# santiagolmedo/gnn_qot_estimation

Hardware: AMD Instinct MI355X
Metric: graphs/sec (train step) on 100-node/400-edge synthetic topologies, batch=1024 (higher is better)
Workload: dtype f32; 1 GPU; configs[1]: 2-layer TopologicalGNN (TransformerConv+NNConv) hidden=64, 100-node/400-directed-edge topologies, batch=1024 graphs per GPU, dropout 0.5, SGD momentum 0.9, SmoothL1; CSR build included in every step; graphs_per_gpu=1024, global_batch=1024, distinct_graphs_per_gpu=1024, launch=hip-graph replay, 4 whole steps (fwd+bwd+optimizer each) per graph, steps_per_graph=4, collective_in_graph=False, parallelism=dp1, prime_steps=45, collective_world_size=1, all_reduce_floats=68715

## Files before the change

### gnn_qot_estimation_amd/_lib.py

```python
from __future__ import annotations

import ctypes as C
import os
import subprocess

import torch

_HERE = os.path.dirname(os.path.abspath(__file__))
LIB_PATH = os.environ.get("QOT_LIB_PATH") or os.path.join(_HERE, "libqot_gnn.so")
CSRC_DIR = os.path.join(_HERE, "csrc")

_p = C.c_void_p
_i64 = C.c_int64
_int = C.c_int
_f = C.c_float
_u64 = C.c_uint64
_sz = C.c_size_t

ABI_VERSION = 13

_INFER_COMMON = ([_p] * 5 + [_i64] * 3 + [_int, _int, _p, _int, _p, _int, _p, _int] + [_p] * 9
                 + [_f, _f, _p, _int, _int, _int, _p])
_LP_COMMON = ([_p] * 6 + [_i64] * 4 + [_p] * 4 + [_f] + [_p] * 4 + [_f] + [_p] * 4 + [_f, _p, _p] + [_int] * 5 + [_p])

SIGNATURES = {
    "qot_abi_version": (_int, []),
    "qot_error_string": (C.c_char_p, [_int]),
    "qot_csr_workspace_bytes": (_sz, [_i64, _i64, _int]),
    "qot_csr_build": (_int, [_p, _i64, _i64, _int, _p, _p, _p, _p, _p, _p, _p, _p, _p, _p, _sz, _p]),
    "qot_csr_gat_by_graph_supported": (_int, [_i64, _i64]),
    "qot_csr_build_gat_by_graph": (_int, [_p, _i64, _i64, _p, _p, _i64, _i64, _i64, _p, _p, _p, _p, _p, _p, _p, _p, _p, _p, _p,
                                          _p]),
    "qot_csr_build_by_graph": (_int, [_p, _i64, _i64, _p, _p, _i64, _i64, _i64, _p, _p, _p, _p, _p, _p, _p, _p, _p,
                                      _p, _p, _p, _p, _p, _p, _p]),
    "qot_i32_gather": (_int, [_p, _p, _p, _i64, _p]),
    "qot_i64_to_i32": (_int, [_p, _p, _i64, _p]),
    "qot_batch_ptr": (_int, [_p, _i64, _i64, _p, _p]),
    "qot_embed_fwd": (_int, [_p, _p, _p, _i64, _int, _int, _p]),
    "qot_embed_bwd": (_int, [_p, _p, _p, _i64, _int, _int, _p]),
    "qot_tconv_fwd_scores": (_int, [_p, _p, _p, _int, _p, _int, _p, _p, _p, _p, _p, _p, _p, _p, _i64, _int, _int,
                                    _int, _f, _f, _u64, _p, _p]),
    "qot_tconv_rows_supported": (_int, [_int, _int, _int]),
    "qot_tconv_rows_npad": (_int, [_int]),
    "qot_tconv_rows_ld": (_int, [_int, _int, _int]),
    "qot_tconv_bwd_dst_rows": (_int, [_p, _p, _p, _int, _p, _p, _p, _p, _p, _p, _p, _int, _p, _p, _p, _p, _f, _f, _u64, _p,
                                      _int, _i64, _int, _p, _p, _int, _int, _p]),
    "qot_tconv_fwd_rows": (_int, [_p, _p, _p, _int, _p, _int, _p, _p, _p, _p, _p, _p, _p, _int, _i64, _int, _int, _int,
                                  _int, _f, _f, _u64, _p, _p]),
    "qot_tconv_bwd_src_rows": (_int, [_p, _p, _p, _p, _p, _int, _i64, _int, _p, _int, _p]),
    "qot_tconv_fwd": (_int, [_p, _p, _p, _p, _int, _p, _p, _p, _p, _p, _p, _p, _p, _i64, _int, _int,
                             _int, _f, _f, _u64, _p, _p]),
    "qot_tconv_fwd_tile": (_int, [_p, _p, _p, _p, _int, _p, _p, _p, _p, _p, _p, _p, _p, _i64, _int, _int, _int, _i64,
                                  _int, _f, _f, _u64, _p, _p]),
    "qot_tconv_bwd_dst_workspace_floats": (_sz, [_i64, _int, _int]),
    "qot_tconv_rows_per_block": (_int, [_int]),
    "qot_tconv_bwd_dst_blocks": (_i64, [_i64, _int, _int, _i64]),
    "qot_tconv_bwd_dst": (_int, [_p, _p, _p, _p, _int, _p, _p, _p, _p, _p, _p, _p, _p, _p, _int, _p, _p, _p, _p,
                                 _p, _f, _f, _u64, _p, _p, _p, _int, _i64, _p, _i64, _int, _int, _p]),
    "qot_tconv_bwd_src": (_int, [_p, _int, _p, _int, _p, _p, _p, _p, _p, _p, _p, _p, _int, _int, _i64, _p, _i64, _int,
                                 _p]),
    "qot_tconv_graph_supported": (_int, [_int, _int, _int, _int]),
    "qot_tconv_graph_ldm": (_int, [_int]),
    "qot_tconv_graph_row_floats": (_sz, [_int, _int, _int]),
    "qot_tconv_bwd_graph_blocks": (_int, [_i64]),
    "qot_table_scores": (_int, [_p, _p, _p, _p, _p, _p, _p, _p, _int, _int, _int, _p]),
    "qot_tconv_fwd_graph": (_int, [_p, _int, _p, _p, _p, _p, _p, _p, _p, _p, _p, _p, _p, _p, _int, _i64, _int, _int, _int,
                                   _int, _f, _f, _u64, _p, _p]),
    "qot_tconv_bwd_graph": (_int, [_p, _p, _f, _f, _u64, _p, _p, _int, _p, _p, _p, _p, _p, _p, _p, _p, _p, _p, _p, _int,
                                   _i64, _int, _int, _int, _p]),
    "qot_table_project_bwd_scores": (_int, [_p, _p, _p, _p, _p, _p, _p, _p, _p, _p, _p, _p, _int, _int, _int, _int, _p]),
    "qot_nnconv_agg": (_int, [_p, _int, _p, _p, _p, _p, _p, _p, _p, _p, _int, _p, _i64, _int, _int, _p]),
    "qot_nnconv_fused": (_int, [_p, _int, _p, _p, _p, _p, _p, _p, _p, _int, _p, _p, _p, _i64, _int, _int,
                                _int, _f, _f, _u64, _p, _p]),
    "qot_nnconv_fused_split": (_int, [_p, _int, _p, _p, _p, _p, _p, _p, _p, _p, _i64, _p, _p, _i64, _int, _int,
                                      _int, _f, _f, _u64, _p, _p]),
    "qot_nnconv_gradh_split": (_int, [_p, _int, _p, _int, _p, _p, _p, _p, _p, _p, _p, _p, _i64, _p, _p, _p, _i64, _int,
                                      _int, _p]),
    "qot_nnconv_bwd_finalize": (_int, [_p, _p, _p, _p, _p, _i64, _int, _int, _p]),
    "qot_nnconv_dw_workspace_floats": (_sz, [_i64, _int, _int]),
    "qot_nnconv_dw": (_int, [_p, _int, _p, _int, _p, _p, _p, _p, _p, _p, _p, _p, _p, _i64, _int, _int, _p]),
    "qot_gemm_tn_workspace_floats": (_sz, [_int]),
    "qot_gemm_tn": (_int, [_p, _int, _p, _int, _i64, _int, _p, _p, _p]),
    "qot_nnconv_adjoint_dw_workspace_floats": (_sz, [_int]),
    "qot_nnconv_adjoint_dw": (_int, [_p, _int, _p, _int, _p, _p, _p, _p, _p, _p, _p, _p, _p, _p, _int, _p, _i64,
                                     _int, _int, _p]),
    "qot_nnconv_gradh_workspace_floats": (_sz, [_int]),
    "qot_nnconv_gradh_fused": (_int, [_p, _int, _p, _int, _p, _p, _p, _p, _p, _p, _p, _p, _p, _p, _p, _i64, _int,
                                      _int, _p]),
    "qot_nnconv_bwd_edge": (_int, [_p, _int, _p, _int, _p, _p, _p, _p, _p, _p, _p, _p, _p, _i64, _int,
                                   _int, _p]),
    "qot_tconv_edge_attr_grad": (_int, [_p, _p, _f, _f, _u64, _p, _p, _int, _p, _p, _p, _p, _p, _p, _p, _i64, _int, _int,
                                        _p]),
    "qot_nnconv_edge_attr_grad": (_int, [_p, _int, _p, _int, _p, _p, _p, _p, _p, _p, _p, _p, _i64, _int, _int, _p]),
    "qot_tconv_attention": (_int, [_p, _int, _p, _p, _p, _p, _p, _p, _p, _i64, _int, _int, _p]),
    "qot_gat_attention": (_int, [_p, _p, _p, _p, _p, _p, _i64, _p, _i64, _int, _f, _p]),
    "qot_act_fwd": (_int, [_p, _p, _i64, _f, _f, _u64, _p, _p]),
    "qot_act_bwd": (_int, [_p, _p, _p, _i64, _f, _f, _u64, _p, _p]),
    "qot_pool_fwd": (_int, [_p, _p, _p, _i64, _int, _p]),
    "qot_pool_bwd": (_int, [_p, _p, _p, _p, _i64, _i64, _int, _p]),
    "qot_gat_blocks": (_int, [_i64, _int, _int]),
    "qot_gat_bn_partials_floats": (_sz, [_i64, _int, _int]),
    "qot_gat_logits": (_int, [_p, _p, _p, _p, _p, _i64, _int, _int, _p]),
    "qot_gat_fwd": (_int, [_p, _p, _p, _p, _p, _p, _p, _p, _i64, _int, _int, _f, _p, _p]),
    "qot_gat_att_grad": (_int, [_p, _p, _p, _p, _p, _p, _i64, _int, _int, _p]),
    "qot_gat_chunk_rows": (_i64, [_i64, _int, _int]),
    "qot_bn_stats_from_partials": (_int, [_p, _p, _int, _i64, _i64, _int, _f, _f, _p, _p, _p, _p, _p]),
    "qot_gat_thin_supported": (_int, [_int, _int, _int]),
    "qot_gat_fwd_thin": (_int, [_p, _int, _p, _p, _p, _p, _p, _p, _p, _p, _i64, _int, _int, _f, _p, _p]),
    "qot_gat_bwd_dst_thin": (_int, [_p, _p, _int, _p, _p, _p, _p, _p, _p, _p, _p, _p, _i64, _int, _int, _f, _p, _p, _p]),
    "qot_gat_bwd_dst": (_int, [_p, _p, _p, _p, _p, _p, _p, _p, _p, _p, _i64, _int, _int, _f, _p, _p, _p]),
    "qot_gat_bwd_src": (_int, [_p, _p, _p, _p, _p, _p, _p, _p, _p, _p, _i64, _int, _int, _f, _p, _p, _p, _p]),
    "qot_bn_partials_floats": (_sz, [_i64, _int]),
    "qot_bn_stats": (_int, [_p, _i64, _int, _f, _f, _p, _p, _p, _p, _p, _p]),
    "qot_bn_apply": (_int, [_p, _p, _p, _p, _p, _p, _i64, _int, _int, _p]),
    "qot_bn_bwd_reduce": (_int, [_p, _p, _p, _p, _p, _p, _p, _i64, _int, _int, _p, _p, _p, _p]),
    "qot_bn_bwd_apply": (_int, [_p, _p, _p, _p, _p, _p, _p, _p, _p, _i64, _int, _int, _int, _p, _p]),
    "qot_bn_apply_rows": (_int, [_p, _p, _i64, _p, _p, _p, _p, _p, _int, _int, _p]),
    "qot_bn_bwd_reduce_rows": (_int, [_p, _p, _i64, _p, _p, _p, _p, _p, _int, _int, _p, _p, _p, _p]),
    "qot_bn_bwd_apply_rows": (_int, [_p, _p, _i64, _p, _p, _p, _p, _p, _p, _p, _i64, _int, _int, _p, _p]),
    "qot_sgd_momentum": (_int, [_p, _p, _p, _i64, _f, _f, _int, _p]),
    "qot_sgd_momentum_multi": (_int, [_p, _p, _p, _int, _p, _p, _i64, _f, _p, _f, _int, _p]),
    "qot_sgd_momentum_dev": (_int, [_p, _p, _p, _i64, _p, _f, _int, _p]),
    "qot_small_gemm": (_int, [_p, _i64, _i64, _p, _i64, _i64, _p, _p, _int, _int, _int, _int, _int, _p]),
    "qot_colsum_workspace_floats": (_sz, [_int]),
    "qot_colsum": (_int, [_p, _int, _i64, _int, _p, _p, _p]),
    "qot_rowsum_wide_workspace_floats": (_sz, [_i64]),
    "qot_rowsum_wide": (_int, [_p, _i64, _i64, _p, _p, _p]),
    "qot_head_fwd": (_int, [_p, _p, _p, _p, _p, _p, _p, _p, _p, _i64, _int, _int, _f, _f, _u64, _p, _p]),
    "qot_head_fwd_loss": (_int, [_p, _p, _p, _p, _p, _p, _p, _p, _p, _i64, _int, _int, _f, _f, _u64, _p, _p, _f, _p, _p, _p]),
    "qot_head_train": (_int, [_p, _p, _p, _p, _p, _p, _p, _f, _p, _p, _p, _p, _p, _i64, _int, _int, _f, _f, _u64, _p, _int,
                              _f, _f, _u64, _p, _p]),
    "qot_head_train_blocks": (_int, [_i64, _int]),
    "qot_head_bwd_workspace_floats": (_sz, [_int, _int]),
    "qot_head_bwd_blocks": (_int, [_i64]),
    "qot_head_bwd": (_int, [_p, _p, _p, _p, _p, _p, _p, _p, _p, _i64, _int, _int, _f, _f, _u64, _p,
                            _p, _f, _f, _u64, _p, _p]),
    "qot_act_bwd_colsum": (_int, [_p, _p, _p, _i64, _int, _f, _f, _u64, _p, _p, _p, _p]),
    "qot_smooth_l1_workspace_floats": (_sz, []),
    "qot_smooth_l1": (_int, [_p, _p, _i64, _f, _p, _p, _p, _p]),
    "qot_table_project_fwd": (_int, [_p, _p, _p, _p, _p, _p, _p, _p, _p, _p, _int, _int, _p, _p, _p]),
    "qot_table_project_bwd": (_int, [_p, _p, _p, _p, _p, _p, _p, _p, _p, _int, _int, _p]),
    "qot_table_maps": (_int, [_p, _p, _p, _p, _p, _p, _i64, _i64, _p]),
    "qot_step_advance": (_int, [_p, _p, _p]),
    "qot_shard_stage": (_int, [_p, _i64, _p, _p, _p, _p, _i64, _i64, _i64, _p, _p, _int, _p, _p, _int, _p, _int, _i64, _i64,
                               _i64, _i64, _i64, _i64, _p, _p, _p, _p, _p, _p, _p, _p, _p]),
    "qot_shard_stage_padded": (_int, [_p, _i64, _p, _p, _p, _p, _i64, _i64, _i64, _p, _p, _int, _p, _p, _int, _p, _int, _i64,
                                      _i64, _i64, _i64, _i64, _i64, _p, _p, _p, _p, _p, _p, _p, _p, _p]),
    "qot_shard_stage_gather": (_int, [_p, _i64, _p, _p, _p, _p, _i64, _i64, _i64, _p, _p, _int, _p, _p, _int, _p, _int, _i64,
                                      _i64, _i64, _i64, _i64, _i64, _p, _p, _p, _p, _p, _p, _p, _p, _p]),
    "qot_gather3": (_int, [_p, _i64, _p, _i64, _p, _p, _p, _i64, _p]),
    "qot_gemm_nt": (_int, [_p, _i64, _p, _i64, _p, _i64, _i64, _int, _int, _p, _p, _p, _p]),
    "qot_gemm_nt_planes": (_int, [_p, _i64, _p, _i64, _p, _i64, _int, _int, _int, _p]),
    "qot_gemm_tn_splits": (_int, [_int, _int, _i64]),
    "qot_gemm256_takes": (_int, [_i64, _int]),
    "qot_gemm_tn_planes": (_int, [_p, _i64, _p, _i64, _p, _int, _int, _i64, _int, _p, _p, _p]),
    "qot_skinny_linear_fwd": (_int, [_p, _p, _p, _i64, _int, _int, _p]),
    "qot_skinny_linear_fwd_logits": (_int, [_p, _p, _p, _i64, _int, _int, _p, _p, _p, _p, _p]),
    "qot_gemm_nt_logits": (_int, [_p, _i64, _p, _i64, _p, _i64, _i64, _int, _int, _p, _p, _p, _p, _p, _p, _p, _p]),
    "qot_skinny_linear_dw_blocks": (_int, [_i64]),
    "qot_skinny_linear_dw": (_int, [_p, _p, _p, _i64, _int, _int, _p]),
    "qot_run_roles": (_int, [_p, _int, _p]),
    "qot_nnconv_gradh_host_roles": (_int, [_p, _int]),
    "qot_rows_gather": (_int, [_p, _p, _p, _i64, _int, _p]),
    "qot_rows_scatter": (_int, [_p, _p, _p, _i64, _int, _p]),
    **{f"qot_topological_infer{k}_supported": (_int, [_int] * 5) for k in ("", "_mc", "_grad", "_whatif")},
    **{f"qot_topological_infer{k}_max_edges": (_int, [_int] * 3) for k in ("", "_mc", "_grad", "_whatif")},
    "qot_topological_infer": (_int, _INFER_COMMON + [_p]),
    "qot_topological_infer_mc": (_int, _INFER_COMMON + [_int, _i64, _u64, _f, _f, _int, _p]),
    "qot_topological_infer_grad": (_int, _INFER_COMMON + [_p, _int, _p, _p, _p]),
    "qot_topological_infer_whatif": (_int, _INFER_COMMON + [_p, _p, _p, _i64, _p, _p, _i64, _p, _i64, _int, _p]),
    "qot_topological_infer_status": (_int, _INFER_COMMON + [_p, _p, _p, _i64, _int, _i64, _i64, _int, _int, _int, _p, _int,
                                                            _p]),
    "qot_topological_infer_place": (_int, _INFER_COMMON + [_p, _p, _p, _i64, _int, _i64, _i64, _int, _int, _int, _p, _int,
                                                           _p, _p, _p, _i64, _p]),
    "qot_lightpath_infer": (_int, _LP_COMMON + [_p]),
    "qot_lightpath_infer_grad": (_int, _LP_COMMON + [_p, _int, _p, _p, _p, _p, _p]),
    "qot_lightpath_infer_whatif": (_int, _LP_COMMON + [_p, _p, _p, _i64, _p, _p, _i64, _i64, _p]),
    "qot_lightpath_infer_status": (_int, _LP_COMMON + [_p, _p, _p, _i64, _int, _i64, _i64, _int, _int, _int, _int, _p, _int,
                                                       C.c_double, _p]),
    "qot_lightpath_infer_place": (_int, _LP_COMMON + [_p, _p, _p, _i64, _int, _i64, _i64, _int, _int, _int, _int, _p, _int,
                                                      C.c_double, _p, _p, _p, _i64, _p]),
    "qot_topological_infer_place_release": (_int, _INFER_COMMON + [_p, _p, _p, _i64, _int, _i64, _i64, _int, _int, _int, _p,
                                                                   _int, _p, _p, _p, _i64, _p, _p, _i64, _p]),
    "qot_lightpath_infer_place_release": (_int, _LP_COMMON + [_p, _p, _p, _i64, _int, _i64, _i64, _int, _int, _int, _int, _p,
                                                              _int, C.c_double, _p, _p, _p, _i64, _p, _p, _i64, _p]),
    "qot_lightpath_infer_place_impact": (_int, _LP_COMMON + [_p, _p, _p, _i64, _int, _i64, _i64, _int, _int, _int, _int, _p,
                                                             _int, C.c_double, _p, _p, _p, _i64, _p, _p, _p, _p, _int, _p]),
    "qot_status_graph_scratch_bytes": (_sz, [_i64, _i64, _i64, _int]),
    "qot_status_graph_count": (_int, [_p, _p, _p, _i64, _i64, _int, _i64, _i64, _int, _int, _int, C.c_double, _int, _p, _sz, _p,
                                      _p]),
    "qot_status_graph_fill": (_int, [_p, _p, _p, _i64, _i64, _int, _i64, _i64, _int, _int, _int, _int, _p, _int, _p, _int, _p,
                                     _p, _p, _p, _i64, _i64, _p, _p, _p, _p, _p]),
}

MAX_ROLES = 12
(ROLE_CSR_BY_GRAPH, ROLE_TABLE_PROJECT_FWD, ROLE_GATHER3, ROLE_SUM_ROWS, ROLE_NNCONV_FINALIZE64, ROLE_TABLE_PROJECT_BWD,
 ROLE_TABLE_SCORES, ROLE_TABLE_PROJECT_BWD_SCORES, ROLE_NNCONV_SLAB_SUM64, ROLE_NNCONV_GRADH_SUM64) = range(1, 11)
HOSTABLE_ROLES = (ROLE_SUM_ROWS, ROLE_NNCONV_SLAB_SUM64)


class Role(C.Structure):
    _fields_ = [("kind", C.c_int32), ("reserved", C.c_int32), ("p", C.c_void_p * 18), ("i", C.c_int64 * 8)]


def make_role(kind: int, ptrs, ints) -> Role:
    r = Role()
    r.kind = kind
    for k, t in enumerate(ptrs):
        r.p[k] = None if t is None else (t.data_ptr() if isinstance(t, torch.Tensor) else int(t))
    for k, v in enumerate(ints):
        r.i[k] = int(v)
    return r


def run_roles(roles, stream_handle=None):
    if not roles:
        return
    if len(roles) > MAX_ROLES:
        for k in range(0, len(roles), MAX_ROLES):
            run_roles(roles[k:k + MAX_ROLES], stream_handle)
        return
    arr = (Role * len(roles))(*roles)
    code = (_lib or load()).qot_run_roles(C.addressof(arr), len(roles), stream() if stream_handle is None else stream_handle)
    if code != 0:
        check(code, "qot_run_roles")


def host_roles(roles):
    arr = (Role * max(len(roles), 1))(*roles)
    code = (_lib or load()).qot_nnconv_gradh_host_roles(C.addressof(arr), len(roles))
    if code != 0:
        check(code, "qot_nnconv_gradh_host_roles")


_lib = None


class QotError(RuntimeError):
    """A libqot_gnn entry point returned a non-zero status."""


def build_library(verbose: bool = False) -> str:
    cmd = ["make", "-C", CSRC_DIR, "-j", str(min(8, os.cpu_count() or 1))]
    res = subprocess.run(cmd, capture_output=True, text=True)
    if res.returncode != 0:
        raise RuntimeError("building libqot_gnn.so failed:\n" + res.stdout[-4000:] + res.stderr[-8000:])
    if verbose:
        print(res.stdout[-2000:])
    return LIB_PATH


def load():
    global _lib
    if _lib is not None:
        return _lib
    if not os.path.exists(LIB_PATH):
        raise QotError(
            f"{LIB_PATH} not found: build it with `python -c 'import __graft_entry__ as g; g.build()'` "
            "or `make -C gnn_qot_estimation_amd/csrc` -- there is no CPU fallback for the HIP path"
        )
    lib = C.CDLL(LIB_PATH)
    for name, (res, args) in SIGNATURES.items():
        fn = getattr(lib, name)
        fn.restype = res
        fn.argtypes = args
    if lib.qot_abi_version() != ABI_VERSION:
        raise QotError(f"libqot_gnn ABI version {lib.qot_abi_version()} != {ABI_VERSION} expected by this package: "
                       "rebuild with `make -C gnn_qot_estimation_amd/csrc`")
    _lib = lib
    return lib


def ptr(t):
    return None if t is None else t.data_ptr()


_raw_stream = getattr(torch._C, "_cuda_getCurrentRawStream", None)
_raw_device = getattr(torch._C, "_cuda_getDevice", None)


def stream():
    if _pinned_stream is not None:
        return _pinned_stream
    if _raw_stream is not None and _raw_device is not None:
# ... 36 lines not shown
```

### gnn_qot_estimation_amd/csrc/head.hip

```cpp
#include "common.hpp"

namespace qot {

constexpr int kHeadBwdBlocks = 512;

template <int H>
__global__ __launch_bounds__(256) void head_fwd_kernel(
    const float* __restrict__ x, const int32_t* __restrict__ ptr, const float* __restrict__ w0,
    const float* __restrict__ b0, const float* __restrict__ w3, const float* __restrict__ b3,
    float* __restrict__ pooled, float* __restrict__ hidden, float* __restrict__ out, int O, ActParams act,
    const float* __restrict__ target, float beta, float inv_n, float* __restrict__ grad_out, float* __restrict__ loss_rows) {
    __shared__ float4 red[256];
    __shared__ float lrow[8];
    __shared__ float p[H];
    __shared__ float h[H];
    constexpr int TPR = H / 4, RPB = 256 / TPR;
    const int sub = threadIdx.x % TPR, slot = threadIdx.x / TPR;
    const int64_t b = blockIdx.x;
    const int beg = ptr[b], end = ptr[b + 1];
    float4 acc = f4zero();
    if (slot < RPB)
        for (int64_t r = beg + slot; r < end; r += RPB) acc = add4(acc, ld4(x + r * H + 4 * sub));
    red[threadIdx.x] = acc;
    __syncthreads();
    if (threadIdx.x < TPR) {
        float4 s = red[threadIdx.x];
        for (int k = 1; k < RPB; ++k) s = add4(s, red[k * TPR + threadIdx.x]);
        const int cnt = end - beg;
        s = scale4(1.0f / (float)(cnt > 1 ? cnt : 1), s);
        p[4 * threadIdx.x] = s.x; p[4 * threadIdx.x + 1] = s.y; p[4 * threadIdx.x + 2] = s.z; p[4 * threadIdx.x + 3] = s.w;
        st4(pooled + b * H + 4 * threadIdx.x, s);
    }
    __syncthreads();
    if (threadIdx.x < H) {
        const int o = threadIdx.x;
        float v = b0[o];
#pragma unroll 8
        for (int a = 0; a < H; ++a) v = fmaf(w0[o * H + a], p[a], v);
        v = act_apply1(v, act, (uint64_t)(b * H + o));
        h[o] = v;
        hidden[b * H + o] = v;
    }
    __syncthreads();
    if (threadIdx.x < O) {
        const int o = threadIdx.x;
        float v = b3[o];
        for (int a = 0; a < H; ++a) v = fmaf(w3[o * H + a], h[a], v);
        out[b * O + o] = v;
        if (target) {
            const float d = v - target[b * O + o];
            const float ad = fabsf(d);
            float l, g;
            if (ad < beta) { l = 0.5f * d * d / beta; g = d / beta; }
            else           { l = ad - 0.5f * beta;    g = d > 0.f ? 1.f : -1.f; }
            grad_out[b * O + o] = g * inv_n;
            lrow[o] = l * inv_n;
        }
    }
    if (target) {
        __syncthreads();
        if (threadIdx.x == 0) {
            float s = lrow[0];
            for (int o = 1; o < O; ++o) s += lrow[o];
            loss_rows[b] = s;
        }
    }
}

template <int H>
__global__ __launch_bounds__(256) void head_bwd_kernel(
    const float* __restrict__ gout, const float* __restrict__ pooled, const float* __restrict__ hidden,
    const int32_t* __restrict__ ptr, const float* __restrict__ w0, const float* __restrict__ w3,
    float* __restrict__ gx, float* __restrict__ partials, int64_t B, int O, ActParams act,
    const float* __restrict__ x_in, ActParams in_act) {
    constexpr int PER = H * H / 256;
    __shared__ float4 cred[256];
    float4 acs = f4zero();
    __shared__ float gh[H];
    __shared__ float gp[H];
    __shared__ float pp[H];
    __shared__ float go[8];
    float aw0[PER];
#pragma unroll
    for (int e = 0; e < PER; ++e) aw0[e] = 0.f;
    float ab0 = 0.f, aw3[8], ab3 = 0.f;
#pragma unroll
    for (int e = 0; e < 8; ++e) aw3[e] = 0.f;
    const int t = threadIdx.x;
    __shared__ float w0s[H * H];
    __shared__ float w3s[8 * H];
    {
        float wv[PER];
#pragma unroll
        for (int e = 0; e < PER; ++e) wv[e] = w0[t + 256 * e];
#pragma unroll
        for (int e = 0; e < PER; ++e) w0s[t + 256 * e] = wv[e];
    }
    for (int e = t; e < O * H; e += 256) w3s[e] = w3[e];
    for (int64_t b = blockIdx.x; b < B; b += gridDim.x) {
        if (t < O) go[t] = gout[b * O + t];
        if (t < H) pp[t] = pooled[b * H + t];
        const int beg = ptr[b], end = ptr[b + 1];
        const float hv_pre = (t < H) ? hidden[b * H + t] : 0.f;
        __syncthreads();
        if (t < H) {
            float v = 0.f;
            for (int o = 0; o < O; ++o) v = fmaf(w3s[o * H + t], go[o], v);
            const float hv = hv_pre;
            float d = 0.f;
            if (act.thr16) {
                const uint64_t z = act_hash64(act.seed, (uint64_t)act.step[0], (uint64_t)(b * H + t) >> 2);
                const bool keep = ((uint32_t)(z >> (16 * ((b * H + t) & 3))) & 0xFFFFu) >= act.thr16;
                d = keep ? act.keep_scale : 0.f;
            } else {
                d = 1.0f;
            }
            d *= (hv > 0.f) ? 1.0f : act.slope;
            gh[t] = v * d;
            ab0 += v * d;
#pragma unroll
            for (int o = 0; o < 8; ++o) if (o < O) aw3[o] = fmaf(go[o], hv, aw3[o]);
        }
        if (t < O) ab3 += go[t];
        __syncthreads();
        if (t < H) {
            float v = 0.f;
#pragma unroll 8
            for (int o = 0; o < H; ++o) v = fmaf(w0s[o * H + t], gh[o], v);
            gp[t] = v;
        }
#pragma unroll
        for (int e = 0; e < PER; ++e) {
            const int idx = t * PER + e;
            aw0[e] = fmaf(gh[idx / H], pp[idx % H], aw0[e]);
        }
        __syncthreads();
        const float inv = 1.0f / (float)((end - beg) > 1 ? (end - beg) : 1);
        constexpr int TPR = H / 4, RPB = 256 / TPR;
        const int sub = t % TPR, slot = t / TPR;
        float4 cs = f4zero();
        if (slot < RPB) {
            const float4 v = make_float4(gp[4 * sub] * inv, gp[4 * sub + 1] * inv, gp[4 * sub + 2] * inv, gp[4 * sub + 3] * inv);
            if (!x_in) {
                for (int64_t r = beg + slot; r < end; r += RPB) st4(gx + r * H + 4 * sub, v);
            } else {
                constexpr int UR = 4;
                for (int64_t r0 = beg + slot; r0 < end; r0 += (int64_t)UR * RPB) {
                    float4 yy[UR];
#pragma unroll
                    for (int u = 0; u < UR; ++u) {
                        const int64_t r = r0 + (int64_t)u * RPB;
                        yy[u] = ld4(x_in + (r < end ? r : r0) * H + 4 * sub);
                    }
// ... 126 lines not shown
                }
                if (t < O) ptgt = target[bn * O + t];
            }
        }
        float4 acc = f4zero();
        if (slot < RPB) {
#pragma unroll
            for (int u = 0; u < 8; ++u) {
                const int r = slot + u * RPB;
                if (r < cnt) {
                    if (in_lds) *reinterpret_cast<float4*>(&xs[r * H + 4 * sub]) = v0[u];
                    acc = add4(acc, v0[u]);
                }
            }
            for (int r0 = slot + 8 * RPB; r0 < cnt; r0 += 8 * RPB) {
                float4 v[8];
#pragma unroll
                for (int u = 0; u < 8; ++u) {
                    const int r = r0 + u * RPB;
                    v[u] = ld4(x + (int64_t)(beg + (r < cnt ? r : r0)) * H + 4 * sub);
                }
#pragma unroll
                for (int u = 0; u < 8; ++u) {
                    const int r = r0 + u * RPB;
                    if (r < cnt) {
                        if (in_lds) *reinterpret_cast<float4*>(&xs[r * H + 4 * sub]) = v[u];
                        acc = add4(acc, v[u]);
                    }
                }
            }
        }
        cred[t] = acc;
        __syncthreads();
        if (t < TPR) {
            float4 s4 = cred[t];
            for (int k2 = 1; k2 < RPB; ++k2) s4 = add4(s4, cred[k2 * TPR + t]);
            s4 = scale4(1.0f / (float)(cnt > 1 ? cnt : 1), s4);
            pp[4 * t] = s4.x; pp[4 * t + 1] = s4.y; pp[4 * t + 2] = s4.z; pp[4 * t + 3] = s4.w;
        }
        __syncthreads();
        float hv = 0.f, dact = 0.f;
        if (t < H) {
            float v = b0t;
#pragma unroll 8
            for (int a = 0; a < H; ++a) v = fmaf(w0s[t * HP + a], pp[a], v);
            float d = 1.0f;
            if (act.thr16) {
                const uint64_t flat = (uint64_t)(b * H + t);
                const uint64_t z = act_hash64(act.seed, stepv, flat >> 2);
                const bool keep = ((uint32_t)(z >> (16 * (flat & 3))) & 0xFFFFu) >= act.thr16;
                d = keep ? act.keep_scale : 0.f;
            }
            d *= (v > 0.f) ? 1.0f : act.slope;
            hv = v * d;
            dact = d;
            hh[t] = hv;
        }
        __syncthreads();
        if (t < O) {
            float v = b3t;
            for (int a = 0; a < H; ++a) v = fmaf(w3s[t * H + a], hh[a], v);
            out[b * O + t] = v;
            const float df = v - tgt;
            const float ad = fabsf(df);
            float l, g;
            if (ad < beta) { l = 0.5f * df * df / beta; g = df / beta; }
            else           { l = ad - 0.5f * beta;      g = df > 0.f ? 1.f : -1.f; }
            g *= inv_n;
            grad_out[b * O + t] = g;
            go[t] = g;
            lrow[t] = l * inv_n;
            ab3 += g;
        }
        __syncthreads();
        if (t == 0) {
            float sl = lrow[0];
            for (int o = 1; o < O; ++o) sl += lrow[o];
            loss_rows[b] = sl;
        }
        if (t < H) {
            float v = 0.f;
            for (int o = 0; o < O; ++o) v = fmaf(w3s[o * H + t], go[o], v);
            const float g1 = v * dact;
            gh[t] = g1;
            ab0 += g1;
#pragma unroll
            for (int o = 0; o < 8; ++o) if (o < O) aw3[o] = fmaf(go[o], hv, aw3[o]);
        }
        __syncthreads();
        if (t < H) {
            float v = 0.f;
#pragma unroll 8
            for (int o = 0; o < H; ++o) v = fmaf(w0s[o * HP + t], gh[o], v);
            gp[t] = v;
        }
#pragma unroll
        for (int e = 0; e < PER; ++e) {
            const int idx = t * PER + e;
            aw0[e] = fmaf(gh[idx / H], pp[idx % H], aw0[e]);
        }
        __syncthreads();
        const float inv = 1.0f / (float)(cnt > 1 ? cnt : 1);
        float4 cs = f4zero();
        if (slot < RPB) {
            const float4 v = make_float4(gp[4 * sub] * inv, gp[4 * sub + 1] * inv, gp[4 * sub + 2] * inv, gp[4 * sub + 3] * inv);
            if (!fold) {
                for (int r = slot; r < cnt; r += RPB) st4(gx + (int64_t)(beg + r) * H + 4 * sub, v);
            } else {
                for (int r = slot; r < cnt; r += RPB) {
                    const int64_t flat = (int64_t)(beg + r) * H + 4 * sub;
                    const float4 yy = in_lds ? *reinterpret_cast<const float4*>(&xs[r * H + 4 * sub]) : ld4(x + flat);
                    uint64_t z = 0;
                    if (in_act.thr16) z = act_hash64(in_act.seed, in_stepv, (uint64_t)flat >> 2);
                    float vi[4] = {v.x, v.y, v.z, v.w};
                    const float vr[4] = {yy.x, yy.y, yy.z, yy.w};
#pragma unroll
                    for (int c = 0; c < 4; ++c) {
                        const bool keep = in_act.thr16 ? (((uint32_t)(z >> (16 * c)) & 0xFFFFu) >= in_act.thr16) : true;
                        vi[c] = vi[c] * (keep ? in_act.keep_scale : 0.f) * (vr[c] > 0.f ? 1.0f : in_act.slope);
                    }
                    const float4 o4 = make_float4(vi[0], vi[1], vi[2], vi[3]);
                    st4(gx + flat, o4);
                    cs = add4(cs, o4);
                }
            }
        }
        if (fold) {
            cred[t] = cs;
            __syncthreads();
            if (t < TPR) {
                float4 s4 = cred[t];
                for (int k2 = 1; k2 < RPB; ++k2) s4 = add4(s4, cred[k2 * TPR + t]);
                acs = add4(acs, s4);
            }
        }
        __syncthreads();
    }
    float* part = partials + (int64_t)blockIdx.x * (H * H + H + O * H + O + (fold ? H : 0));
    if (fold && t < H / 4) st4(part + H * H + H + O * H + O + 4 * t, acs);
#pragma unroll
    for (int e = 0; e < PER; ++e) part[t * PER + e] = aw0[e];
    if (t < H) {
        part[H * H + t] = ab0;
        for (int o = 0; o < O; ++o) part[H * H + H + o * H + t] = aw3[o];
    }
    if (t < O) part[H * H + H + O * H + t] = ab3;
}

constexpr int kHeadKeep = 32;
#ifndef QOT_HEAD_THREADS
#define QOT_HEAD_THREADS 512
#endif
constexpr int kHeadThreads = QOT_HEAD_THREADS;

template <int H, int NT>
__global__ __launch_bounds__(NT) void head_train_batched_kernel(
    const float* __restrict__ x, const int32_t* __restrict__ ptr, const float* __restrict__ w0,
    const float* __restrict__ b0, const float* __restrict__ w3, const float* __restrict__ b3,
    const float* __restrict__ target, float beta, float inv_n, float* __restrict__ out, float* __restrict__ grad_out,
    float* __restrict__ loss_rows, float* __restrict__ gx, float* __restrict__ partials, int64_t B, int O, ActParams act,
    int fold, ActParams in_act) {
    constexpr int TPR = H / 4, RPB = NT / TPR;
    constexpr int GB = 256 / H;
    constexpr int SPG = RPB / GB;
    constexpr int KS = NT / 256;
    constexpr int KR = kHeadKeep * 4 / SPG;
    constexpr int PER = H * H / NT;
    constexpr int HP = H + 1;
    static_assert(KS == 1 || KS == 2 || KS == 4, "dense outputs are summed inside a quad");
    static_assert(H % (4 * KS) == 0 && PER >= 1, "width");
    extern __shared__ __attribute__((aligned(16))) float dyn[];
    float* w0s = dyn;
    float* w3s = w0s + H * HP;
    __shared__ float4 cred[NT > 640 ? NT : 640];
    __shared__ __attribute__((aligned(16))) float pp[GB][H];
    __shared__ __attribute__((aligned(16))) float hh[GB][H];
    __shared__ __attribute__((aligned(16))) float gh[GB][H];
    __shared__ __attribute__((aligned(16))) float gp[GB][H];
    __shared__ float go[GB][8];
    __shared__ float lrow[GB][8];
    __shared__ int pb[GB + 1];
    const int t = threadIdx.x;
    const int sub = t % TPR, slot = t / TPR;
    const int gs = slot / SPG, sr = slot % SPG;
    const int part = t % KS, od = t / KS;
    const int g = od / H, o = od % H;
    const int64_t npass = (B + GB - 1) / GB;
    int pb_first = 0;
    if (t <= GB && (int64_t)blockIdx.x < npass) {
        const int64_t bb = (int64_t)blockIdx.x * GB + t;
        pb_first = ptr[bb < B ? bb : B];
    }
    for (int e = t; e < H * H; e += NT) w0s[(e / H) * HP + e % H] = w0[e];
    for (int e = t; e < O * H; e += NT) w3s[e] = w3[e];
    const uint64_t stepv = act.thr16 ? (uint64_t)act.step[0] : 0;
    const uint64_t in_stepv = (fold && in_act.thr16) ? (uint64_t)in_act.step[0] : 0;
    const float b0o = b0[o];
    float aw0[PER];
#pragma unroll
    for (int e = 0; e < PER; ++e) aw0[e] = 0.f;
    float ab0p = 0.f, aw3p[8], ab3p = 0.f;
#pragma unroll
    for (int e = 0; e < 8; ++e) aw3p[e] = 0.f;
    float4 acs = f4zero();
    for (int64_t ps = blockIdx.x; ps < npass; ps += gridDim.x) {
        const int64_t b0g = ps * GB;
        __syncthreads();
        if (t <= GB) {
            const int64_t bb = b0g + t;
            pb[t] = ps == (int64_t)blockIdx.x ? pb_first : ptr[bb < B ? bb : B];
        }
        __syncthreads();
        const bool live = b0g + gs < B;
        const int beg = pb[gs], cnt = live ? pb[gs + 1] - beg : 0;
        float4 v[KR];
        float4 acc = f4zero();
#pragma unroll
        for (int k = 0; k < KR; ++k) {
            const int r = sr + SPG * k;
            v[k] = (r < cnt) ? ld4(x + (int64_t)(beg + r) * H + 4 * sub) : f4zero();
        }
#pragma unroll
        for (int k = 0; k < KR; ++k) acc = add4(acc, v[k]);
        for (int r = sr + SPG * KR; r < cnt; r += SPG) acc = add4(acc, ld4(x + (int64_t)(beg + r) * H + 4 * sub));
        cred[t] = acc;
        __syncthreads();
        if (t < GB * TPR) {
            const int gg = t / TPR, sb = t % TPR;
            float4 s4 = cred[(gg * SPG) * TPR + sb];
            for (int q = 1; q < SPG; ++q) s4 = add4(s4, cred[(gg * SPG + q) * TPR + sb]);
            const int c2 = pb[gg + 1] - pb[gg];
            s4 = scale4(1.0f / (float)(c2 > 1 ? c2 : 1), s4);
            pp[gg][4 * sb] = s4.x; pp[gg][4 * sb + 1] = s4.y; pp[gg][4 * sb + 2] = s4.z; pp[gg][4 * sb + 3] = s4.w;
        }
        __syncthreads();
        const int64_t bg = b0g + g;
        float hv = 0.f, dact = 0.f;
        {
            float a0 = 0.f;
#pragma unroll
            for (int a = part * (H / KS); a < (part + 1) * (H / KS); ++a) a0 = fmaf(w0s[o * HP + a], pp[g][a], a0);
            if (KS >= 2) a0 += dpp_move<0xB1>(a0);
            if (KS >= 4) a0 += dpp_move<0x4E>(a0);
            const float vv = a0 + b0o;
            float d = 1.0f;
            if (act.thr16) {
                const uint64_t flat = (uint64_t)(bg * H + o);
                const uint64_t z = act_hash64(act.seed, stepv, flat >> 2);
                const bool keep = ((uint32_t)(z >> (16 * (flat & 3))) & 0xFFFFu) >= act.thr16;
                d = keep ? act.keep_scale : 0.f;
            }
            d *= (vv > 0.f) ? 1.0f : act.slope;
            hv = vv * d;
            dact = d;
            if (part == 0) hh[g][o] = hv;
        }
        __syncthreads();
        for (int q = t / 16; q < GB * O; q += NT / 16) {
            const int gg = q / O, o3 = q % O, l16 = t % 16;
            const int64_t bb = b0g + gg;
            float pv = 0.f;
#pragma unroll
            for (int a = l16 * (H / 16); a < (l16 + 1) * (H / 16); ++a) pv = fmaf(w3s[o3 * H + a], hh[gg][a], pv);
            pv = group_sum<16>(pv);
            if (l16 == 0) {
                if (bb < B) {
                    const float vv = pv + b3[o3];
                    out[bb * O + o3] = vv;
                    const float df = vv - target[bb * O + o3];
                    const float ad = fabsf(df);
                    float l, gq;
                    if (ad < beta) { l = 0.5f * df * df / beta; gq = df / beta; }
                    else           { l = ad - 0.5f * beta;      gq = df > 0.f ? 1.f : -1.f; }
                    gq *= inv_n;
                    grad_out[bb * O + o3] = gq;
                    go[gg][o3] = gq;
                    lrow[gg][o3] = l * inv_n;
                } else {
                    go[gg][o3] = 0.f;
                    lrow[gg][o3] = 0.f;
                }
            }
        }
        __syncthreads();
        if (t < GB && b0g + t < B) {
            float sl = lrow[t][0];
            for (int o3 = 1; o3 < O; ++o3) sl += lrow[t][o3];
            loss_rows[b0g + t] = sl;
        }
        if (t < GB * O) ab3p += go[t / O][t % O];
        {
            float vv = 0.f;
            for (int o3 = 0; o3 < O; ++o3) vv = fmaf(w3s[o3 * H + o], go[g][o3], vv);
            const float g1 = bg < B ? vv * dact : 0.f;
            if (part == 0) {
                gh[g][o] = g1;
                ab0p += g1;
#pragma unroll
                for (int o3 = 0; o3 < 8; ++o3) if (o3 < O) aw3p[o3] = fmaf(go[g][o3], hv, aw3p[o3]);
            }
        }
        __syncthreads();
        {
            float a0 = 0.f;
#pragma unroll
            for (int oo = part * (H / KS); oo < (part + 1) * (H / KS); ++oo) a0 = fmaf(w0s[oo * HP + o], gh[g][oo], a0);
            if (KS >= 2) a0 += dpp_move<0xB1>(a0);
            if (KS >= 4) a0 += dpp_move<0x4E>(a0);
            if (part == 0) gp[g][o] = a0;
        }
#pragma unroll
        for (int gg = 0; gg < GB; ++gg)
#pragma unroll
            for (int e = 0; e < PER; ++e) {
                const int idx = t * PER + e;
                aw0[e] = fmaf(gh[gg][idx / H], pp[gg][idx % H], aw0[e]);
            }
        __syncthreads();
        if (cnt > 0) {
            const float inv = 1.0f / (float)(cnt > 1 ? cnt : 1);
            const float4 gv = make_float4(gp[gs][4 * sub] * inv, gp[gs][4 * sub + 1] * inv, gp[gs][4 * sub + 2] * inv,
                                          gp[gs][4 * sub + 3] * inv);
            auto back = [&](int r, float4 yy) {
                const int64_t flat = (int64_t)(beg + r) * H + 4 * sub;
                if (!fold) { st4(gx + flat, gv); return; }
                uint64_t z = 0;
                if (in_act.thr16) z = act_hash64(in_act.seed, in_stepv, (uint64_t)flat >> 2);
                float vi[4] = {gv.x, gv.y, gv.z, gv.w};
                const float vr[4] = {yy.x, yy.y, yy.z, yy.w};
#pragma unroll
                for (int c = 0; c < 4; ++c) {
                    const bool keep = in_act.thr16 ? (((uint32_t)(z >> (16 * c)) & 0xFFFFu) >= in_act.thr16) : true;
                    vi[c] = vi[c] * (keep ? in_act.keep_scale : 0.f) * (vr[c] > 0.f ? 1.0f : in_act.slope);
                }
                const float4 o4 = make_float4(vi[0], vi[1], vi[2], vi[3]);
                st4(gx + flat, o4);
                acs = add4(acs, o4);
            };
#pragma unroll
            for (int k = 0; k < KR; ++k) {
                const int r = sr + SPG * k;
                if (r < cnt) back(r, v[k]);
            }
            for (int r = sr + SPG * KR; r < cnt; r += SPG) back(r, fold ? ld4(x + (int64_t)(beg + r) * H + 4 * sub) : f4zero());
        }
    }
    float* part_row = partials + (int64_t)blockIdx.x * (H * H + H + O * H + O + (fold ? H : 0));
#pragma unroll
    for (int e = 0; e < PER; ++e) part_row[t * PER + e] = aw0[e];
    __syncthreads();
    float* red = reinterpret_cast<float*>(cred);
    if (part == 0) {
        red[od] = ab0p;
#pragma unroll
        for (int o3 = 0; o3 < 8; ++o3) if (o3 < O) red[(1 + o3) * 256 + od] = aw3p[o3];
    }
    if (t < GB * O) red[9 * 256 + t] = ab3p;
    __syncthreads();
    if (t < H) {
        float s2 = red[t];
#pragma unroll
        for (int gg = 1; gg < GB; ++gg) s2 += red[gg * H + t];
        part_row[H * H + t] = s2;
        for (int o3 = 0; o3 < O; ++o3) {
            float s3 = red[(1 + o3) * 256 + t];
#pragma unroll
            for (int gg = 1; gg < GB; ++gg) s3 += red[(1 + o3) * 256 + gg * H + t];
            part_row[H * H + H + o3 * H + t] = s3;
        }
    }
    if (t < O) {
        float s2 = red[9 * 256 + t];
        for (int gg = 1; gg < GB; ++gg) s2 += red[9 * 256 + gg * O + t];
        part_row[H * H + H + O * H + t] = s2;
    }
    if (fold) {
        __syncthreads();
        cred[t] = acs;
        __syncthreads();
        if (t < TPR) {
            float4 s4 = cred[t];
            for (int k2 = 1; k2 < RPB; ++k2) s4 = add4(s4, cred[k2 * TPR + t]);
            st4(part_row + H * H + H + O * H + O + 4 * t, s4);
        }
    }
}

__global__ __launch_bounds__(1024) void head_partial_sum_kernel(const float* __restrict__ partials, int nblk, int n,
                                                                float* __restrict__ out) {
    __shared__ float red[16][64];
    const int o = threadIdx.x & 63, sg = threadIdx.x >> 6;
    const int t = blockIdx.x * 64 + o;
    float acc = 0.f;
    if (t < n) {
        const int per = (nblk + 15) / 16;
        const int p0 = sg * per, p1 = (p0 + per < nblk) ? p0 + per : nblk;
        int p = p0;
        for (; p + 8 <= p1; p += 8) {
            float v[8];
#pragma unroll
            for (int u = 0; u < 8; ++u) v[u] = partials[(int64_t)(p + u) * n + t];
#pragma unroll
            for (int u = 0; u < 8; ++u) acc += v[u];
        }
        for (; p < p1; ++p) acc += partials[(int64_t)p * n + t];
    }
    red[sg][o] = acc;
    __syncthreads();
    if (sg == 0 && t < n) {
        float s = red[0][o];
#pragma unroll
        for (int q = 1; q < 16; ++q) s += red[q][o];
        out[t] = s;
    }
}

}

using namespace qot;

#define QOT_HEAD_H(H, ...)                                            \
    switch (H) {                                                      \
        case 16:  { constexpr int kH = 16;  __VA_ARGS__; } break;     \
        case 32:  { constexpr int kH = 32;  __VA_ARGS__; } break;     \
        case 64:  { constexpr int kH = 64;  __VA_ARGS__; } break;     \
        case 128: { constexpr int kH = 128; __VA_ARGS__; } break;     \
        default: return QOT_ERR_UNSUPPORTED;                          \
    }

extern "C" int qot_head_train(const float* x, const int32_t* ptr, const float* w0, const float* b0, const float* w3,
                              const float* b3, const float* target, float beta, float* out, float* grad_out,
                              float* loss_rows, float* grad_x, float* workspace, int64_t B, int H, int O, float slope,
                              float p, uint64_t seed, const int64_t* step_counter, int fold, float in_slope, float in_p,
                              uint64_t in_seed, const int64_t* in_step, qot_stream_t stream_) {
    hipStream_t stream = (hipStream_t)stream_;
    if (B <= 0 || O <= 0 || !(beta > 0.f)) return QOT_ERR_BADARG;
    if (O > 8) return QOT_ERR_UNSUPPORTED;
    if (!x || !ptr || !w0 || !b0 || !w3 || !b3 || !target || !out || !grad_out || !loss_rows || !grad_x || !workspace)
        return QOT_ERR_BADARG;
    const ActParams ap = make_act(1, slope, p, seed, step_counter);
    const ActParams in_ap = make_act(fold ? 1 : 0, in_slope, in_p, in_seed, in_step);
    int blocks = kHeadBwdBlocks;
    if (B < blocks) blocks = (int)B;
    const float inv_n = 1.0f / ((float)B * (float)O);
    if (H <= 64) {
        const int gbn = 256 / H;
        int64_t nb = (B + gbn - 1) / gbn;
        if (nb > kHeadBwdBlocks) nb = kHeadBwdBlocks;
        blocks = (int)nb;
        QOT_HEAD_H(H, {
            if constexpr (kH <= 64) {
                const size_t lds = (size_t)(kH * (kH + 1) + 8 * kH) * sizeof(float);
                constexpr int NT = kH * kH < kHeadThreads ? 256 : kHeadThreads;
                head_train_batched_kernel<kH, NT><<<blocks, NT, lds, stream>>>(
                    x, ptr, w0, b0, w3, b3, target, beta, inv_n, out, grad_out, loss_rows, grad_x, workspace, B, O, ap, fold,
                    in_ap);
            }
        });
        QOT_LAUNCH_CHECK();
        return QOT_OK;
    }
    QOT_HEAD_H(H, {
        const size_t lds = (size_t)(kHeadRowsCap * kH + kH * (kH + 1) + 8 * kH) * sizeof(float);
        static size_t allowed[kMaxDevices];
        const int lrc = ensure_dyn_lds(reinterpret_cast<const void*>(head_train_kernel<kH>), lds, allowed);
        if (lrc != QOT_OK) return lrc;
        head_train_kernel<kH><<<blocks, 256, lds, stream>>>(x, ptr, w0, b0, w3, b3, target, beta, inv_n, out, grad_out,
                                                            loss_rows, grad_x, workspace, B, O, ap, fold, in_ap);
    });
    QOT_LAUNCH_CHECK();
    return QOT_OK;
}

extern "C" int qot_head_train_blocks(int64_t B, int H) {
    if (B <= 0) return 0;
    if (H <= 64 && H >= 16) {
        const int gbn = 256 / H;
        const int64_t nb = (B + gbn - 1) / gbn;
        return nb > kHeadBwdBlocks ? kHeadBwdBlocks : (int)nb;
    }
    return B < kHeadBwdBlocks ? (int)B : kHeadBwdBlocks;
}


extern "C" int qot_head_fwd_loss(const float* x, const int32_t* ptr, const float* w0, const float* b0,
                                 const float* w3, const float* b3, float* pooled, float* hidden, float* out,
                                 int64_t B, int H, int O, float slope, float p, uint64_t seed,
                                 const int64_t* step_counter, const float* target, float beta, float* grad_out,
                                 float* loss_rows, qot_stream_t stream) {
    if (B < 0 || O <= 0 || O > 8) return (O > 8) ? QOT_ERR_UNSUPPORTED : QOT_ERR_BADARG;
    if (B == 0) return QOT_OK;
    if (!x || !ptr || !w0 || !b0 || !w3 || !b3 || !pooled || !hidden || !out) return QOT_ERR_BADARG;
    if (target && (!grad_out || !loss_rows || !(beta > 0.f))) return QOT_ERR_BADARG;
    const ActParams ap = make_act(1, slope, p, seed, step_counter);
    const float inv_n = 1.0f / ((float)B * (float)O);
    QOT_HEAD_H(H, head_fwd_kernel<kH><<<(int)B, 256, 0, (hipStream_t)stream>>>(x, ptr, w0, b0, w3, b3, pooled, hidden,
                                                                              out, O, ap, target, beta, inv_n, grad_out,
                                                                              loss_rows));
    QOT_LAUNCH_CHECK();
    return QOT_OK;
}

extern "C" int qot_head_fwd(const float* x, const int32_t* ptr, const float* w0, const float* b0,
                            const float* w3, const float* b3, float* pooled, float* hidden, float* out,
                            int64_t B, int H, int O, float slope, float p, uint64_t seed,
                            const int64_t* step_counter, qot_stream_t stream) {
    return qot_head_fwd_loss(x, ptr, w0, b0, w3, b3, pooled, hidden, out, B, H, O, slope, p, seed, step_counter, nullptr,
                             1.0f, nullptr, nullptr, stream);
}

extern "C" int qot_head_bwd_blocks(int64_t B) { return B < kHeadBwdBlocks ? (int)(B > 0 ? B : 0) : kHeadBwdBlocks; }

extern "C" size_t qot_head_bwd_workspace_floats(int H, int O) {
    return (size_t)kHeadBwdBlocks * (size_t)(H * H + 2 * H + O * H + O);
}

extern "C" int qot_head_bwd(const float* grad_out, const float* pooled, const float* hidden, const int32_t* ptr,
                            const float* w0, const float* w3, float* grad_x, float* grads, float* workspace,
                            int64_t B, int H, int O, float slope, float p, uint64_t seed,
                            const int64_t* step_counter, const float* x_in, float in_slope, float in_p,
                            uint64_t in_seed, const int64_t* in_step, qot_stream_t stream_) {
    hipStream_t stream = (hipStream_t)stream_;
    if (B <= 0 || O <= 0) return QOT_ERR_BADARG;
    if (O > 8) return QOT_ERR_UNSUPPORTED;
    if (!grad_out || !pooled || !hidden || !ptr || !w0 || !w3 || !grad_x || !workspace) return QOT_ERR_BADARG;
    const ActParams ap = make_act(1, slope, p, seed, step_counter);
    int blocks = kHeadBwdBlocks;
    if (B < blocks) blocks = (int)B;
    const ActParams in_ap = make_act(x_in ? 1 : 0, in_slope, in_p, in_seed, in_step);
    QOT_HEAD_H(H, head_bwd_kernel<kH><<<blocks, 256, 0, stream>>>(grad_out, pooled, hidden, ptr, w0, w3, grad_x,
                                                                  workspace, B, O, ap, x_in, in_ap));
    QOT_LAUNCH_CHECK();
    if (!grads) return QOT_OK;
    const int n = H * H + H + O * H + O + (x_in ? H : 0);
    head_partial_sum_kernel<<<grid_for(n, 64), 1024, 0, stream>>>(workspace, blocks, n, grads);
    QOT_LAUNCH_CHECK();
    return QOT_OK;
}
```

### gnn_qot_estimation_amd/csrc/mfma_tile.hpp

```cpp
#pragma once
#include "common.hpp"

namespace qot {

typedef float f32x16 __attribute__((ext_vector_type(16)));

__device__ __forceinline__ int at4_slot(int g, int hi, int i) { return (2 * g + hi) * 32 + (i ^ (g & 7)); }

__device__ __forceinline__ void store_fragment_grouped(float4* At4, int g, int i, float4 v0, float4 v1) {
    const float4 even = make_float4(v0.x, v0.z, v1.x, v1.z), odd = make_float4(v0.y, v0.w, v1.y, v1.w);
    At4[at4_slot(g, 0, i)] = even;
    At4[at4_slot(g, 1, i)] = odd;
}

__host__ __device__ constexpr int acc_row(int r, int hi) { return (r & 3) + 8 * (r >> 2) + 4 * hi; }

__device__ __forceinline__ f32x16 mfma4(float4 a, float4 b, f32x16 c) {
    c = __builtin_amdgcn_mfma_f32_32x32x2f32(a.x, b.x, c, 0, 0, 0);
    c = __builtin_amdgcn_mfma_f32_32x32x2f32(a.y, b.y, c, 0, 0, 0);
    c = __builtin_amdgcn_mfma_f32_32x32x2f32(a.z, b.z, c, 0, 0, 0);
    c = __builtin_amdgcn_mfma_f32_32x32x2f32(a.w, b.w, c, 0, 0, 0);
    return c;
}

__device__ __forceinline__ f32x16 mfma_group(const float4* __restrict__ At4, int g, int hi, int r31, float4 b,
                                             f32x16 c) {
    return mfma4(At4[at4_slot(g, hi, r31)], b, c);
}

template <int D>
__device__ __forceinline__ void edge_hidden(const float* __restrict__ w1, const float* __restrict__ b1,
                                            const float* __restrict__ ea, int64_t e, float scale, float* __restrict__ hid) {
    float ee[D];
#pragma unroll
    for (int d = 0; d < D; ++d) ee[d] = ea[e * D + d];
#pragma unroll
    for (int kk = 0; kk < 2 * D; ++kk) {
        float h = b1[kk];
#pragma unroll
        for (int d = 0; d < D; ++d) h = fmaf(w1[kk * D + d], ee[d], h);
        hid[kk] = fmaxf(h, 0.f) * scale;
    }
}

template <int S, int NH, int SS, int ST>
__device__ __forceinline__ void quad_share_from(const uint32_t (&mylo)[NH], const uint32_t (&myhi)[NH], uint32_t (&zlo)[4 * NH],
                                                uint32_t (&zhi)[4 * NH]) {
#pragma unroll
    for (int t = 0; t < NH; ++t) {
        zlo[S * SS + t * ST] = __builtin_amdgcn_update_dpp(0, mylo[t], S * 0x55, 0xF, 0xF, true);
        zhi[S * SS + t * ST] = __builtin_amdgcn_update_dpp(0, myhi[t], S * 0x55, 0xF, 0xF, true);
    }
}
template <int NH, int SS, int ST>
__device__ __forceinline__ void quad_share_draws(const uint32_t (&mylo)[NH], const uint32_t (&myhi)[NH], uint32_t (&zlo)[4 * NH],
                                                 uint32_t (&zhi)[4 * NH]) {
    quad_share_from<0, NH, SS, ST>(mylo, myhi, zlo, zhi);
    quad_share_from<1, NH, SS, ST>(mylo, myhi, zlo, zhi);
    quad_share_from<2, NH, SS, ST>(mylo, myhi, zlo, zhi);
    quad_share_from<3, NH, SS, ST>(mylo, myhi, zlo, zhi);
}

__device__ __forceinline__ void mfma_acc_in_agprs() {
#ifndef QOT_NO_AGPR_HINT
    float az = 0.f;
    asm volatile("; accumulators in AGPRs" : "+a"(az));
#endif
}

template <bool AFFINE>
__device__ __forceinline__ float4 affine_relu4(float4 v, float4 s, float4 t) {
    if (!AFFINE) return v;
    return make_float4(fmaxf(fmaf(v.x, s.x, t.x), 0.f), fmaxf(fmaf(v.y, s.y, t.y), 0.f),
                       fmaxf(fmaf(v.z, s.z, t.z), 0.f), fmaxf(fmaf(v.w, s.w, t.w), 0.f));
}

__device__ __forceinline__ void lds_barrier() {
    asm volatile("s_waitcnt lgkmcnt(0)" ::: "memory");
    __builtin_amdgcn_s_barrier();
    asm volatile("" ::: "memory");
}

__device__ __forceinline__ int64_t xcd_tile(int64_t it, int64_t ntiles, unsigned grid) {
    const int nx = 8;
    if ((int)grid % nx != 0) {
        const int64_t t = (int64_t)blockIdx.x + it * grid;
        return t < ntiles ? t : -1;
    }
    const int xcd = blockIdx.x % nx, slot = blockIdx.x / nx, per_x = grid / nx;
    const int64_t chunk = (ntiles + nx - 1) / nx;
    const int64_t local = slot + it * per_x;
    const int64_t t = xcd * chunk + local;
    return (local < chunk && t < ntiles) ? t : -1;
}
__device__ __forceinline__ int64_t xcd_tile(int64_t it, int64_t ntiles) {
    const int nx = 8;
    if ((int)gridDim.x % nx != 0) {
        const int64_t t = (int64_t)blockIdx.x + it * gridDim.x;
        return t < ntiles ? t : -1;
    }
    const int xcd = blockIdx.x % nx, slot = blockIdx.x / nx, per_x = gridDim.x / nx;
    const int64_t chunk = (ntiles + nx - 1) / nx;
    const int64_t local = slot + it * per_x;
    const int64_t t = xcd * chunk + local;
    return (local < chunk && t < ntiles) ? t : -1;
}

}

static inline int num_cus() {
    static int n = 0;
    if (!n) {
        int dev = 0;
        hipDeviceProp_t prop;
        if (hipGetDevice(&dev) == hipSuccess && hipGetDeviceProperties(&prop, dev) == hipSuccess) n = prop.multiProcessorCount;
        if (n <= 0) n = 256;
    }
    return n;
}
```

### gnn_qot_estimation_amd/csrc/nnconv_mfma.hip

```cpp
#include "common.hpp"
#include "mfma_tile.hpp"
#include "nnconv_finalize_dev.hpp"
#include "split_bf16.hpp"

namespace qot {

template <int D, bool TRANSPOSE, bool PRESPLIT = false>
__device__ __forceinline__ void nnconv_gather_tile(
    float* __restrict__ At, const float* __restrict__ x, int ldx, const float* __restrict__ ea,
    const float* __restrict__ w1, const float* __restrict__ b1, const int32_t* __restrict__ rowptr,
    const int32_t* __restrict__ col, const int32_t* __restrict__ eidx, const float* __restrict__ invdeg,
    int64_t tile0, int64_t N, float4& root0, float4& root1, float4* park0 = nullptr, float4* park1 = nullptr) {
    constexpr int K = 2 * D;
    const int sub = threadIdx.x & 7, il = threadIdx.x >> 3;
    const int c0 = 8 * sub;
    const int64_t i = tile0 + il;
    float4 acc0[K + 1], acc1[K + 1];
    root0 = f4zero(); root1 = f4zero();
    int beg = 0, end = 0;
    float srow = 0.f;
    if (i < N) {
        beg = rowptr[i]; end = rowptr[i + 1];
        if (!TRANSPOSE) srow = invdeg[i];
        root0 = ld4(x + i * ldx + c0);
        root1 = ld4(x + i * ldx + c0 + 4);
    }
    const int own = (i < N) ? (int)i : 0;
#define QOT_ACC(FIRSTSLOT, H, X, A) ((FIRSTSLOT) ? scale4((H), (X)) : fma4((H), (X), (A)))
#define QOT_EDGE4(U0, FIRST)                                                                            \
        {                                                                                               \
            float4 xa[4], xb[4];                                                                        \
            float sc[4];                                                                                \
            int jj[4];                                                                                  \
            jj[0] = group8_bcast<U0 + 0>(myj); jj[1] = group8_bcast<U0 + 1>(myj);                       \
            jj[2] = group8_bcast<U0 + 2>(myj); jj[3] = group8_bcast<U0 + 3>(myj);                       \
            sc[0] = group8_bcast<U0 + 0>(mysc); sc[1] = group8_bcast<U0 + 1>(mysc);                     \
            sc[2] = group8_bcast<U0 + 2>(mysc); sc[3] = group8_bcast<U0 + 3>(mysc);                     \
            _Pragma("unroll") for (int u = 0; u < 4; ++u) {                                             \
                const float* xr = x + (int64_t)jj[u] * ldx + c0;                                        \
                xa[u] = ld4(xr);                                                                        \
                xb[u] = ld4(xr + 4);                                                                    \
            }                                                                                           \
            _Pragma("unroll") for (int kk = 0; kk < K; ++kk) {                                          \
                const float h0 = group8_bcast<U0 + 0>(myh[kk]), h1 = group8_bcast<U0 + 1>(myh[kk]);     \
                acc0[kk] = QOT_ACC(FIRST, h0, xa[0], acc0[kk]); acc1[kk] = QOT_ACC(FIRST, h0, xb[0], acc1[kk]); \
                acc0[kk] = fma4(h1, xa[1], acc0[kk]); acc1[kk] = fma4(h1, xb[1], acc1[kk]);             \
            }                                                                                           \
            acc0[K] = QOT_ACC(FIRST, sc[0], xa[0], acc0[K]); acc1[K] = QOT_ACC(FIRST, sc[0], xb[0], acc1[K]); \
            acc0[K] = fma4(sc[1], xa[1], acc0[K]); acc1[K] = fma4(sc[1], xb[1], acc1[K]);               \
             \
             \
            if (cnt > U0 + 2) {                                                                         \
                _Pragma("unroll") for (int kk = 0; kk < K; ++kk) {                                      \
                    const float h2 = group8_bcast<U0 + 2>(myh[kk]), h3 = group8_bcast<U0 + 3>(myh[kk]); \
                    acc0[kk] = fma4(h2, xa[2], acc0[kk]); acc1[kk] = fma4(h2, xb[2], acc1[kk]);         \
                    acc0[kk] = fma4(h3, xa[3], acc0[kk]); acc1[kk] = fma4(h3, xb[3], acc1[kk]);         \
                }                                                                                       \
                _Pragma("unroll") for (int u = 2; u < 4; ++u) {                                         \
                    acc0[K] = fma4(sc[u], xa[u], acc0[K]);                                              \
                    acc1[K] = fma4(sc[u], xb[u], acc1[K]);                                              \
                }                                                                                       \
            }                                                                                           \
        }
#define QOT_FWD_BATCH(FIRST)                                                                            \
    {                                                                                                   \
        const int p = base + sub;                                                                       \
        int myj = own;                                                                                  \
        float myh[K], mysc = 0.f;                                                                       \
        _Pragma("unroll") for (int kk = 0; kk < K; ++kk) myh[kk] = 0.f;                                 \
        if (p < end) {                                                                                  \
            myj = col[p];                                                                               \
            mysc = TRANSPOSE ? invdeg[myj] : srow;                                                      \
            edge_hidden<D>(w1, b1, ea, (int64_t)eidx[p], mysc, myh);                                    \
        }                                                                                               \
        const int cnt = (end - base < 8) ? end - base : 8;                                              \
        QOT_EDGE4(0, FIRST)                                                                             \
        if (cnt > 4) QOT_EDGE4(4, false)                                                                \
    }
    int base = beg;
    QOT_FWD_BATCH(true)
    for (base = beg + 8; base < end; base += 8) QOT_FWD_BATCH(false)
#undef QOT_FWD_BATCH
#undef QOT_EDGE4
#undef QOT_ACC
    if constexpr (PRESPLIT) {
        constexpr int HB = (K + 2) / 2;
#pragma unroll
        for (int kk = 0; kk < HB; ++kk)
            store_split_planes(reinterpret_cast<u32x4*>(At) + kk * 3 * kGhPlLd, sub, il, acc0[kk], acc1[kk]);
#pragma unroll
        for (int kk = HB; kk <= K; ++kk) { park0[kk - HB] = acc0[kk]; park1[kk - HB] = acc1[kk]; }
    } else {
#pragma unroll
        for (int kk = 0; kk <= K; ++kk)
            store_fragment_grouped(reinterpret_cast<float4*>(At), kk * 8 + sub, il, acc0[kk], acc1[kk]);
    }
}

__device__ __forceinline__ void root_restage(float* At, float4 root0, float4 root1) {
    lds_barrier();
    store_fragment_grouped(reinterpret_cast<float4*>(At), threadIdx.x & 7, threadIdx.x >> 3, root0, root1);
    __syncthreads();
}

__host__ __device__ constexpr int fwd_plane_off(int p) { return (p / 4) * 3 * kGhPlLd + (p % 4) * kGhPlStep; }

template <int D, bool TRANSPOSE, bool SPLIT = false, bool PRESPLIT = false>
__global__ __launch_bounds__(256, 2) void nnconv_mfma64_kernel(
    const float* __restrict__ x, int ldx, const float* __restrict__ ea, const float* __restrict__ w1,
    const float* __restrict__ b1, const int32_t* __restrict__ rowptr, const int32_t* __restrict__ col,
    const int32_t* __restrict__ eidx, const float* __restrict__ invdeg, const float* __restrict__ Wp,
    const float* __restrict__ bias, float* __restrict__ out, int64_t N, ActParams act,
    const u32x4* __restrict__ Ws = nullptr, int64_t ws_planes = 0) {
    static_assert(!SPLIT || !TRANSPOSE, "split form: forward only");
    static_assert(!PRESPLIT || SPLIT, "the planes are the split form's");
    constexpr int K = 2 * D;
    constexpr int KM = (K + 1) * 64;
    constexpr int GM = KM / 16;
    constexpr int CH = 4;
    constexpr int HB = (K + 2) / 2;
    constexpr int PLF = HB * 3 * kGhPlLd * 4;
    __shared__ __attribute__((aligned(16))) float At[PRESPLIT ? PLF + 4 * 8 * 64 : KM * 32];
    const int64_t ntiles = (N + 31) / 32;
    const float bz = bias ? bias[((threadIdx.x >> 6) & 1) * 32 + (threadIdx.x & 31)] : 0.f;
    const uint64_t drop_step = (act.enabled && act.thr16) ? (uint64_t)act.step[0] : 0;
#pragma unroll 1
    for (int64_t it = 0;; ++it) {
    const int64_t tile = xcd_tile(it, ntiles);
    if (tile < 0) break;
    const int64_t tile0 = tile * 32;
    float4 root0, root1;
    float4 park0[PRESPLIT ? HB : 1], park1[PRESPLIT ? HB : 1];
    if constexpr (PRESPLIT) {
        nnconv_gather_tile<D, false, true>(At, x, ldx, ea, w1, b1, rowptr, col, eidx, invdeg, tile0, N, park0[HB - 1],
                                           park1[HB - 1], park0, park1);
    } else {
        nnconv_gather_tile<D, TRANSPOSE>(At, x, ldx, ea, w1, b1, rowptr, col, eidx, invdeg, tile0, N, root0, root1);
    }
    const float4* At4 = reinterpret_cast<const float4*>(At);
    const int lane = threadIdx.x & 63, wave = threadIdx.x >> 6;
    const int nh = wave & 1, kh = wave >> 1;
    const int r31 = lane & 31, hi = lane >> 5;
    f32x16 c;
#pragma unroll
    for (int r = 0; r < 16; ++r) c[r] = 0.f;
    if constexpr (PRESPLIT) {
        constexpr int SP = K + 2;
        constexpr int ST = 4 * SP;
        constexpr int SC = 2;
        constexpr int NCS = SP / SC;
        constexpr int NBS = 3;
        const int wv = __builtin_amdgcn_readfirstlane(wave);
        const u32x4* wsp = Ws + ((int64_t)(wv & 1) * ST + (wv >> 1) * SP) * 64;
        const unsigned lane_u = lane;
        const u32x4* plane = reinterpret_cast<const u32x4*>(At) + lane;
        const u32x4* pl_e = plane + kh * (fwd_plane_off(SP) - fwd_plane_off(0));
        const u32x4* pl_o = plane + kh * (fwd_plane_off(SP + 2) - fwd_plane_off(2));
        Bf3 sb[NBS][SC];
#define QOT_FWD_BLOAD(J)                                                                                \
        _Pragma("unroll") for (int u = 0; u < SC; ++u)                                                  \
            sb[(J) % NBS][u] = load_split_b(wsp + (((J) / NCS) * 2 * SP + ((J) % NCS) * SC + u) * 64, lane_u, ws_planes);
#define QOT_FWD_ALOAD(J)                                                                                \
        _Pragma("unroll") for (int u = 0; u < SC; ++u) {                                                \
            const int t = ((J) % NCS) * SC + u;                                                         \
            af[(J) & 1][u] = load_split_b(((t & 2) ? pl_o : pl_e) + fwd_plane_off(t), kGhPlLd);         \
        }
#define QOT_FWD_CHUNK(J)                                                                                \
        {                                                                                               \
            if ((J) + NBS - 1 < 2 * NCS) { QOT_FWD_BLOAD((J) + NBS - 1) }                               \
            if (((J) + 1) % NCS != 0) { QOT_FWD_ALOAD((J) + 1) }                                        \
            __builtin_amdgcn_sched_barrier(0);                                                          \
            _Pragma("unroll") for (int u = 0; u < SC; ++u) c = mfma_split6(af[(J) & 1][u], sb[(J) % NBS][u], c); \
            __builtin_amdgcn_sched_barrier(0);                                                          \
        }
        Bf3 af[2][SC];
#pragma unroll
        for (int j = 0; j < NBS - 1; ++j) QOT_FWD_BLOAD(j)
        lds_barrier();
        QOT_FWD_ALOAD(0)
#pragma unroll
        for (int j = 0; j < NCS; ++j) QOT_FWD_CHUNK(j)
        lds_barrier();
        {
            const int sub = threadIdx.x & 7, il = threadIdx.x >> 3;
#pragma unroll
            for (int kk = 0; kk < HB; ++kk)
                store_split_planes(reinterpret_cast<u32x4*>(At) + kk * 3 * kGhPlLd, sub, il, park0[kk], park1[kk]);
        }
        lds_barrier();
        QOT_FWD_ALOAD(NCS)
#pragma unroll
        for (int j = NCS; j < 2 * NCS; ++j) QOT_FWD_CHUNK(j)
#undef QOT_FWD_ALOAD
#undef QOT_FWD_CHUNK
#undef QOT_FWD_BLOAD
    } else if constexpr (SPLIT) {
        constexpr int ST = (K + 2) * 64 / 16;
        constexpr int SM = GM / 2;
        constexpr int SC = 2;
        constexpr int NCS = SM / SC;
        constexpr int NBS = 3;
        static_assert(GM % 4 == 0, "chunking");
        const u32x4* wsn = Ws + (int64_t)nh * ST * 64 + lane;
        const u32x4* wsp = wsn + (int64_t)kh * SM * 64;
        const u32x4* rsp = wsn + (int64_t)(2 * SM + 2 * kh) * 64;
        asm volatile("" : "+v"(rsp));
        Bf3 rbs[2];
#pragma unroll
        for (int u = 0; u < 2; ++u) rbs[u] = load_split_b(rsp + u * 64, ws_planes);
        Bf3 sb[NBS][SC];
#pragma unroll
        for (int q = 0; q < NBS - 1; ++q)
#pragma unroll
            for (int u = 0; u < SC; ++u) sb[q][u] = load_split_b(wsp + (q * SC + u) * 64, ws_planes);
        lds_barrier();
        int ch = 0;
#pragma unroll 1
        for (; ch + NBS <= NCS; ch += NBS) {
#pragma unroll
            for (int q = 0; q < NBS; ++q) {
                if (ch + q + NBS - 1 < NCS) {
#pragma unroll
                    for (int u = 0; u < SC; ++u)
                        sb[(q + NBS - 1) % NBS][u] = load_split_b(wsp + ((ch + q + NBS - 1) * SC + u) * 64, ws_planes);
                }
#pragma unroll
                for (int u = 0; u < SC; ++u) c = mfma_split_step(At4, kh * GM + 2 * ((ch + q) * SC + u), hi, r31, sb[q][u], c);
            }
        }
#pragma unroll
        for (int q = 0; q < NBS - 1; ++q) {
            if (ch + q < NCS) {
#pragma unroll
                for (int u = 0; u < SC; ++u) c = mfma_split_step(At4, kh * GM + 2 * ((ch + q) * SC + u), hi, r31, sb[q][u], c);
            }
        }
        root_restage(At, root0, root1);
#pragma unroll
        for (int u = 0; u < 2; ++u) c = mfma_split_step(At4, kh * 4 + 2 * u, hi, r31, rbs[u], c);
    } else {
    const float4* wpn = reinterpret_cast<const float4*>(Wp) + (int64_t)nh * (2 * GM + 8) * 64 + lane;
    const float4* wp = wpn + (int64_t)kh * GM * 64;
    const float4* rbp = wpn + (int64_t)(2 * GM + kh * 4) * 64;
    asm volatile("" : "+v"(rbp));
    float4 rb[4];
#pragma unroll
    for (int u = 0; u < 4; ++u) rb[u] = rbp[u * 64];
    constexpr int NCH = GM / CH;
    constexpr int NB = 4;
    float4 bb[NB][CH];
#pragma unroll
    for (int q = 0; q < NB - 1; ++q)
#pragma unroll
        for (int u = 0; u < CH; ++u) bb[q][u] = wp[(q * CH + u) * 64];
    lds_barrier();
    int ch = 0;
#pragma unroll 1
    for (; ch + NB <= NCH; ch += NB) {
#pragma unroll
        for (int q = 0; q < NB; ++q) {
            if (ch + q + NB - 1 < NCH) {
#pragma unroll
                for (int u = 0; u < CH; ++u) bb[(q + NB - 1) % NB][u] = wp[((ch + q + NB - 1) * CH + u) * 64];
            }
#pragma unroll
            for (int u = 0; u < CH; ++u) c = mfma_group(At4, kh * GM + (ch + q) * CH + u, hi, r31, bb[q][u], c);
        }
    }
#pragma unroll
    for (int q = 0; q < NB - 1; ++q) {
        if (ch + q < NCH) {
#pragma unroll
            for (int u = 0; u < CH; ++u) c = mfma_group(At4, kh * GM + (ch + q) * CH + u, hi, r31, bb[q][u], c);
        }
    }
    root_restage(At, root0, root1);
#pragma unroll
    for (int u = 0; u < 4; ++u) c = mfma_group(At4, kh * 4 + u, hi, r31, rb[u], c);
    }
    float* red = At + (PRESPLIT ? PLF : 64 * 32);
    if (kh) {
#pragma unroll
        for (int r = 0; r < 8; ++r) red[((2 + nh) * 8 + r) * 64 + lane] = c[r];
    } else {
#pragma unroll
        for (int r = 0; r < 8; ++r) red[(nh * 8 + r) * 64 + lane] = c[8 + r];
    }
    lds_barrier();
    {
        const int colg = nh * 32 + r31;
        float v[8];
        if (kh) {
#pragma unroll
            for (int r = 0; r < 8; ++r) v[r] = c[8 + r] + red[(nh * 8 + r) * 64 + lane] + bz;
        } else {
#pragma unroll
            for (int r = 0; r < 8; ++r) v[r] = c[r] + red[((2 + nh) * 8 + r) * 64 + lane] + bz;
        }
        uint32_t zlo[8], zhi[8];
        const bool drop = act.enabled && act.thr16;
        if (drop) {
            const int jq = r31 & 3;
            uint32_t mylo[2], myhi[2];
#pragma unroll
            for (int t = 0; t < 2; ++t) {
                const int rr = kh * 8 + 2 * jq + t;
                const int row = acc_row(rr, hi);
                const uint64_t flat = (uint64_t)((tile0 + row) * 64 + colg);
                const uint64_t z = act_hash64(act.seed, drop_step, flat >> 2);
                mylo[t] = (uint32_t)z; myhi[t] = (uint32_t)(z >> 32);
            }
            quad_share_draws<2, 2, 1>(mylo, myhi, zlo, zhi);
        }
#pragma unroll
        for (int r = 0; r < 8; ++r) {
            const int rr = kh * 8 + r;
            const int row = acc_row(rr, hi);
            const int64_t i = tile0 + row;
            float y = v[r];
            if (act.enabled) {
                y = y > 0.f ? y : act.slope * y;
                if (drop) {
                    const uint64_t z = ((uint64_t)zhi[r] << 32) | zlo[r];
                    const bool keep = ((uint32_t)(z >> (16 * (colg & 3))) & 0xFFFFu) >= act.thr16;
                    y = keep ? y * act.keep_scale : 0.f;
                }
            }
            if (i < N) out[i * 64 + colg] = y;
        }
    }
    if constexpr (!PRESPLIT) lds_barrier();
    }
}


template <int D, bool SPLIT>
__global__ __launch_bounds__(512, 2) void nnconv_adjoint_dw64_kernel(
    const float* __restrict__ g, int ldg, const float* __restrict__ xf, int ldx, const float* __restrict__ ea,
    const float* __restrict__ w1, const float* __restrict__ b1, const int32_t* __restrict__ rowptr_t,
    const int32_t* __restrict__ col_t, const int32_t* __restrict__ eid_t, const float* __restrict__ invdeg,
    const float* __restrict__ Wp, float* __restrict__ gx, float* __restrict__ slabs, int64_t N) {
    constexpr int K = 2 * D;
    constexpr int KT = (K + 2) * 64;
    constexpr int GQ = KT / 8 / 4;
    constexpr int MB = KT / 32;
    constexpr int TPW = MB * 2 / 8;
    static_assert(GQ % 4 == 0 || GQ % 5 == 0, "chunking");
    constexpr int CH = (GQ % 4 == 0) ? 4 : 5;
    __shared__ __attribute__((aligned(16))) float Ut[KT * 32];
    __shared__ __attribute__((aligned(16))) float red[8 * 3 * 4 * 64];
    __shared__ __attribute__((aligned(16))) float xs[32 * 64];
    float4* Ut4 = reinterpret_cast<float4*>(Ut);
    const int lane = threadIdx.x & 63, wave = threadIdx.x >> 6;
    const int r31 = lane & 31, hi = lane >> 5;
    const int nh = wave & 1, kq = wave >> 1;
    const int ah = wave & 1, mb0 = wave >> 1;
    const int64_t ntiles = (N + 31) / 32;

    f32x16 dw[TPW];
#pragma unroll
    for (int t = 0; t < TPW; ++t)
#pragma unroll
        for (int r = 0; r < 16; ++r) dw[t][r] = 0.f;
    int dwoff[4];
    {
        const int kcol = mb0 * 32 + r31;
        const int gg = kcol >> 3, within = kcol & 7;
        const int base0 = ((2 * gg + (within & 1)) * 32) * 4 + (within >> 1);
        const int m = gg & 7;
#pragma unroll
        for (int b = 0; b < 4; ++b) dwoff[b] = base0 + ((((b ^ (m >> 1)) << 1) | (hi ^ (m & 1))) << 2);
    }
    const float4* wp = reinterpret_cast<const float4*>(Wp) + ((int64_t)nh * (KT / 8) + kq * GQ) * 64 + lane;

#pragma unroll 1
    for (int64_t it = 0;; ++it) {
        const int64_t tile = xcd_tile(it, ntiles);
        if (tile < 0) break;
        const int64_t tile0 = tile * 32;
        float4 xown;
        {
            const int64_t j = tile0 + (threadIdx.x >> 4);
            xown = (j < N) ? ld4(xf + j * ldx + 4 * (threadIdx.x & 15)) : f4zero();
        }
        {
            const int sub = threadIdx.x & 15, il = threadIdx.x >> 4;
            const int c0 = 4 * sub;
            const int64_t j = tile0 + il;
            float4 acc[K + 2];
            acc[K + 1] = f4zero();
            int beg = 0, end = 0;
            if (j < N) { beg = rowptr_t[j]; end = rowptr_t[j + 1]; acc[K + 1] = ld4(g + j * ldg + c0); }
            const int own = (j < N) ? (int)j : 0;
#define QOT_ADJ_EDGE(U)                                                                                  \
                {                                                                                        \
                    const int64_t i = (int64_t)row16_bcast<U>(myi);                                      \
                    gr[(U) & 3] = ld4(g + i * ldg + c0);                                                 \
                    sc[(U) & 3] = row16_bcast<U>(mysc);                                                  \
                }
#define QOT_ADJ_FMA(U, FIRSTSLOT)                                                                        \
                {                                                                                        \
                    _Pragma("unroll") for (int kk = 0; kk < K; ++kk)                                     \
                        acc[kk] = (FIRSTSLOT) ? scale4(row16_bcast<U>(myh[kk]), gr[(U) & 3])             \
                                              : fma4(row16_bcast<U>(myh[kk]), gr[(U) & 3], acc[kk]);     \
                    acc[K] = (FIRSTSLOT) ? scale4(sc[(U) & 3], gr[(U) & 3]) : fma4(sc[(U) & 3], gr[(U) & 3], acc[K]); \
                }
#define QOT_ADJ_EDGE4(U0, FIRST)                                                                         \
                {                                                                                        \
                    float4 gr[4];                                                                        \
                    float sc[4];                                                                         \
                    QOT_ADJ_EDGE(U0) QOT_ADJ_EDGE(U0 + 1) QOT_ADJ_EDGE(U0 + 2) QOT_ADJ_EDGE(U0 + 3)      \
                    QOT_ADJ_FMA(U0, FIRST) QOT_ADJ_FMA(U0 + 1, false)                                    \
                     \
                     \
                    if (cnt > U0 + 2) { QOT_ADJ_FMA(U0 + 2, false) QOT_ADJ_FMA(U0 + 3, false) }          \
                }
#define QOT_ADJ_BATCH(FIRST)                                                                             \
            {                                                                                            \
                const int p = base + sub;                                                                \
                int myi = own;                                                                           \
                float myh[K], mysc = 0.f;                                                                \
                _Pragma("unroll") for (int kk = 0; kk < K; ++kk) myh[kk] = 0.f;                          \
                if (p < end) {                                                                           \
                    myi = col_t[p];                                                                      \
                    mysc = invdeg[myi];                                                                  \
                    edge_hidden<D>(w1, b1, ea, (int64_t)eid_t[p], mysc, myh);                            \
                }                                                                                        \
                const int cnt = (end - base < 16) ? end - base : 16;                                     \
                QOT_ADJ_EDGE4(0, FIRST)                                                                  \
                if (cnt > 4) QOT_ADJ_EDGE4(4, false)                                                     \
                if (cnt > 8) QOT_ADJ_EDGE4(8, false)                                                     \
                if (cnt > 12) QOT_ADJ_EDGE4(12, false)                                                   \
            }
            int base = beg;
            QOT_ADJ_BATCH(true)
            for (base = beg + 16; base < end; base += 16) QOT_ADJ_BATCH(false)
#undef QOT_ADJ_BATCH
#undef QOT_ADJ_EDGE4
#undef QOT_ADJ_FMA
#undef QOT_ADJ_EDGE
#pragma unroll
            for (int kk = 0; kk < K + 2; ++kk) {
                const int gg = kk * 8 + (sub >> 1);
                float2* s0 = reinterpret_cast<float2*>(&Ut4[at4_slot(gg, 0, il)]) + (sub & 1);
                float2* s1 = reinterpret_cast<float2*>(&Ut4[at4_slot(gg, 1, il)]) + (sub & 1);
                *s0 = make_float2(acc[kk].x, acc[kk].z);
                *s1 = make_float2(acc[kk].y, acc[kk].w);
            }
        }
        {
            const int sub = threadIdx.x & 15, il = threadIdx.x >> 4;
            *reinterpret_cast<float4*>(&xs[il * 64 + 4 * sub]) = xown;
        }
        constexpr int NCH = GQ / CH;
        float4 bc[CH], bn[CH];
#pragma unroll
        for (int u = 0; u < CH; ++u) bc[u] = wp[u * 64];
        lds_barrier();
        f32x16 c;
#pragma unroll
        for (int r = 0; r < 16; ++r) c[r] = 0.f;
        {
            int ch = 0;
#pragma unroll 1
            for (; ch + 1 < NCH; ch += 2) {
#pragma unroll
                for (int u = 0; u < CH; ++u) bn[u] = wp[((ch + 1) * CH + u) * 64];
#pragma unroll
                for (int u = 0; u < CH; ++u) c = mfma_group(Ut4, kq * GQ + ch * CH + u, hi, r31, bc[u], c);
                if (ch + 2 < NCH) {
#pragma unroll
                    for (int u = 0; u < CH; ++u) bc[u] = wp[((ch + 2) * CH + u) * 64];
                }
#pragma unroll
                for (int u = 0; u < CH; ++u) c = mfma_group(Ut4, kq * GQ + (ch + 1) * CH + u, hi, r31, bn[u], c);
            }
            if (NCH & 1) {
#pragma unroll
                for (int u = 0; u < CH; ++u) c = mfma_group(Ut4, kq * GQ + (NCH - 1) * CH + u, hi, r31, bc[u], c);
            }
        }
// ... 50 lines not shown
            float v[4];
            if (kq == 0) { v[0] = c[0]; v[1] = c[1]; v[2] = c[2]; v[3] = c[3]; }
            else if (kq == 1) { v[0] = c[4]; v[1] = c[5]; v[2] = c[6]; v[3] = c[7]; }
            else if (kq == 2) { v[0] = c[8]; v[1] = c[9]; v[2] = c[10]; v[3] = c[11]; }
            else { v[0] = c[12]; v[1] = c[13]; v[2] = c[14]; v[3] = c[15]; }
            const int colg = nh * 32 + r31;
#pragma unroll
            for (int rr = 0; rr < 4; ++rr) {
#pragma unroll
                for (int slot = 0; slot < 3; ++slot) v[rr] += red[(((kq * 2 + nh) * 3 + slot) * 4 + rr) * 64 + lane];
                const int reg = 4 * kq + rr;
                const int row = acc_row(reg, hi);
                const int64_t j = tile0 + row;
                if (j < N) gx[j * 64 + colg] = v[rr];
            }
        }
        lds_barrier();
    }
    float* slab = slabs + (int64_t)blockIdx.x * KT * 64;
#pragma unroll
    for (int t = 0; t < TPW; ++t)
#pragma unroll
        for (int r = 0; r < 16; ++r) {
            const int row = acc_row(r, hi);
            slab[((mb0 + 4 * t) * 32 + row) * 64 + ah * 32 + r31] = dw[t][r];
        }
}

__global__ void adj_slab_reduce_kernel(const float* __restrict__ slabs, int nslabs, int per_group, int64_t elems,
                                       int64_t slab_stride, float* __restrict__ dst, int64_t dst_stride) {
    int64_t t = blockIdx.x * (int64_t)blockDim.x + threadIdx.x;
    if (t * 4 >= elems) return;
    const int s0 = blockIdx.y * per_group;
    int s1 = s0 + per_group;
    if (s1 > nslabs) s1 = nslabs;
    float4 acc = f4zero();
    int sidx = s0;
    for (; sidx + 8 <= s1; sidx += 8) {
        float4 v[8];
#pragma unroll
        for (int u = 0; u < 8; ++u) v[u] = ld4(slabs + (int64_t)(sidx + u) * slab_stride + 4 * t);
#pragma unroll
        for (int u = 0; u < 8; ++u) acc = add4(acc, v[u]);
    }
    for (; sidx < s1; ++sidx) acc = add4(acc, ld4(slabs + (int64_t)sidx * slab_stride + 4 * t));
    st4(dst + blockIdx.y * dst_stride + 4 * t, acc);
}

__global__ void adj_slab_final_params_kernel(const float* __restrict__ slabs, int nslabs, int64_t elems,
                                             int64_t slab_stride, float* __restrict__ dst, int K) {
    int64_t t = blockIdx.x * (int64_t)blockDim.x + threadIdx.x;
    if (t * 4 >= elems) return;
    float4 acc = f4zero();
    for (int sidx = 0; sidx < nslabs; ++sidx) acc = add4(acc, ld4(slabs + (int64_t)sidx * slab_stride + 4 * t));
    const int64_t e = 4 * t;
    const int a0 = (int)(e & 63), o = (int)((e >> 6) & 63), kb = (int)(e >> 12);
    const float v[4] = {acc.x, acc.y, acc.z, acc.w};
#pragma unroll
    for (int c = 0; c < 4; ++c) {
        const int a = a0 + c;
        int64_t idx;
        if (kb < K) idx = ((int64_t)a * 64 + o) * K + kb;
        else if (kb == K) idx = (int64_t)4096 * K + a * 64 + o;
        else idx = (int64_t)4096 * (K + 1) + o * 64 + a;
        dst[idx] = v[c];
    }
}

__global__ void gradh_partial_sum_kernel(const float* __restrict__ partials, int nblk, int n, int KD,
                                         float* __restrict__ gw1, float* __restrict__ gb1) {
    const int t = blockIdx.x * (blockDim.x >> 6) + (threadIdx.x >> 6);
    if (t >= n) return;
    const float s = wave_sum_partials(partials, nblk, n, t);
    if ((threadIdx.x & 63) == 0) { if (t < KD) gw1[t] = s; else gb1[t - KD] = s; }
}

}

using namespace qot;

int qot_nnconv_gen_launch(const float* x, int ld_x, const float* edge_attr, const float* w1, const float* b1,
                          const int32_t* rowptr, const int32_t* col, const int32_t* edge_ids, const float* invdeg,
                          int transpose, const float* w_perm, const float* bias, float* out, int64_t N, int H, int D,
                          const ActParams& ap, hipStream_t stream);
int qot_nnconv_gradh_gen_launch(const float* grad_out, int ld_g, const float* x, int ld_x, const float* edge_attr,
                                const float* w1, const float* b1, const int32_t* rowptr, const int32_t* col,
                                const int32_t* eid, const float* invdeg, const float* b_perm, float* gw1, float* gb1,
                                float* workspace, int64_t N, int H, int D, hipStream_t stream);

extern "C" int qot_nnconv_fused(const float* x, int ld_x, const float* edge_attr, const float* w1,
                                const float* b1, const int32_t* rowptr, const int32_t* col,
                                const int32_t* edge_ids, const float* invdeg, int transpose,
                                const float* w_perm, const float* bias, float* out, int64_t N, int H, int D,
                                int act, float act_slope, float act_p, uint64_t act_seed,
                                const int64_t* act_step, qot_stream_t stream) {
    if (N < 0 || !rowptr) return QOT_ERR_BADARG;
    if (H != 16 && H != 32 && H != 64 && H != 128 && H != 256) return QOT_ERR_UNSUPPORTED;
    if (N == 0) return QOT_OK;
    if (!x || !w1 || !b1 || !invdeg || !w_perm || !out || (ld_x & 3)) return QOT_ERR_BADARG;
    if (H != 64 || transpose == 2 || transpose == 3) {
        if (D > 4) return QOT_ERR_UNSUPPORTED;
        return qot_nnconv_gen_launch(x, ld_x, edge_attr, w1, b1, rowptr, col, edge_ids, invdeg, transpose & 1, w_perm,
                                     bias, out, N, H, D, make_act(act, act_slope, act_p, act_seed, act_step),
                                     (hipStream_t)stream);
    }
    int grid = grid_for(N, 32);
    if (grid > 2 * num_cus()) grid = 2 * num_cus();
    const ActParams ap = make_act(act, act_slope, act_p, act_seed, act_step);
    QOT_DISPATCH_D(D, {
        if (transpose)
            nnconv_mfma64_kernel<kD, true><<<grid, 256, 0, (hipStream_t)stream>>>(
                x, ld_x, edge_attr, w1, b1, rowptr, col, edge_ids, invdeg, w_perm, bias, out, N, ap);
        else
            nnconv_mfma64_kernel<kD, false><<<grid, 256, 0, (hipStream_t)stream>>>(
                x, ld_x, edge_attr, w1, b1, rowptr, col, edge_ids, invdeg, w_perm, bias, out, N, ap);
    });
    QOT_LAUNCH_CHECK();
    return QOT_OK;
}

extern "C" int qot_nnconv_fused_split(const float* x, int ld_x, const float* edge_attr, const float* w1,
                                      const float* b1, const int32_t* rowptr, const int32_t* col,
                                      const int32_t* edge_ids, const float* invdeg, const void* w_split,
                                      int64_t split_stride, const float* bias, float* out, int64_t N, int H, int D,
                                      int act, float act_slope, float act_p, uint64_t act_seed,
                                      const int64_t* act_step, qot_stream_t stream) {
    if (N < 0 || !rowptr) return QOT_ERR_BADARG;
    if (H != 64 || D > 4) return QOT_ERR_UNSUPPORTED;
    if (N == 0) return QOT_OK;
    if (!x || !w1 || !b1 || !invdeg || !w_split || !out || (ld_x & 3) || ((uintptr_t)w_split & 15) || (split_stride & 7) ||
        split_stride < (int64_t)(2 * D + 2) * 4096)
        return QOT_ERR_BADARG;
    int grid = grid_for(N, 32);
    if (grid > 2 * num_cus()) grid = 2 * num_cus();
    const ActParams ap = make_act(act, act_slope, act_p, act_seed, act_step);
    const char* sar_env = getenv("QOT_NNCONV_FWD_SPLIT_AFTER_READ");
    const bool presplit = !(sar_env && sar_env[0] == '1' && sar_env[1] == '\0');
    QOT_DISPATCH_D(D, {
        if (kD <= 4) {
            if (presplit)
                nnconv_mfma64_kernel<(kD <= 4 ? kD : 4), false, true, true><<<grid, 256, 0, (hipStream_t)stream>>>(
                    x, ld_x, edge_attr, w1, b1, rowptr, col, edge_ids, invdeg, nullptr, bias, out, N, ap,
                    static_cast<const u32x4*>(w_split), split_stride / 8);
            else
                nnconv_mfma64_kernel<(kD <= 4 ? kD : 4), false, true><<<grid, 256, 0, (hipStream_t)stream>>>(
                    x, ld_x, edge_attr, w1, b1, rowptr, col, edge_ids, invdeg, nullptr, bias, out, N, ap,
                    static_cast<const u32x4*>(w_split), split_stride / 8);
        }
    });
    QOT_LAUNCH_CHECK();
    return QOT_OK;
}

int qot_nnconv_gradh64_launch(const float* grad_out, int ld_g, const float* x, int ld_x, const float* edge_attr, const float* w1,
                              const float* b1, const int32_t* rowptr, const int32_t* col, const int32_t* eid, const float* invdeg,
                              const float* b_perm, const void* b_split, int64_t split_stride, float* workspace, int64_t N, int D,
                              int grid, const qot::HostedTable& hosted, hipStream_t stream);
int qot_hosted_take(qot::HostedTable* t, qot_role_t* planned);
extern "C" size_t qot_nnconv_gradh_workspace_floats(int D) {
    return (size_t)2 * 256 * 2 * (size_t)(2 * D * (D + 1));
}

static int nnconv_gradh_impl(const float* grad_out, int ld_g, const float* x, int ld_x,
                             const float* edge_attr, const float* w1, const float* b1,
                             const int32_t* rowptr, const int32_t* col, const int32_t* eid,
                             const float* invdeg, const float* b_perm, const void* b_split, int64_t split_stride,
                             float* gw1, float* gb1,
                             float* workspace, int64_t N, int H, int D, qot_stream_t stream_) {
    hipStream_t stream = (hipStream_t)stream_;
    HostedTable hosted;
    qot_role_t hosted_roles[QOT_MAX_ROLES];
    const int n_hosted = qot_hosted_take(&hosted, hosted_roles);
    if (N < 0 || !rowptr) return QOT_ERR_BADARG;
    if ((H != 16 && H != 32 && H != 64 && H != 128 && H != 256) || D > 4) return QOT_ERR_UNSUPPORTED;
    if (!grad_out || !x || !w1 || !b1 || !invdeg || !(b_perm || b_split) || (!gw1 != !gb1) || !workspace || (ld_g & 3) ||
        (ld_x & 3) || ((uintptr_t)b_split & 15) || (b_split && ((split_stride & 7) || split_stride < (int64_t)2 * D * 64 * 64)))
        return QOT_ERR_BADARG;
    if (b_split && H != 64) return QOT_ERR_UNSUPPORTED;
    if (!gw1 && H != 64) return QOT_ERR_UNSUPPORTED;
    for (int r = 0; r < n_hosted; ++r) {
        const uintptr_t src = (uintptr_t)hosted.job[r].src, w0 = (uintptr_t)workspace;
        if (src >= w0 && src < w0 + qot_nnconv_gradh_workspace_floats(D) * sizeof(float)) return QOT_ERR_BADARG;
    }
    if (H != 64) {
        const int rc = qot_nnconv_gradh_gen_launch(grad_out, ld_g, x, ld_x, edge_attr, w1, b1, rowptr, col, eid, invdeg, b_perm,
                                                   gw1, gb1, workspace, N, H, D, stream);
        if (rc != QOT_OK || n_hosted == 0) return rc;
        return qot_run_roles(hosted_roles, n_hosted, stream_);
    }
    int grid = grid_for(N > 0 ? N : 1, 32);
    if (grid > 2 * num_cus()) grid = 2 * num_cus();
    const int K = 2 * D;
    const int rc = qot_nnconv_gradh64_launch(grad_out, ld_g, x, ld_x, edge_attr, w1, b1, rowptr, col, eid, invdeg, b_perm,
                                             b_split, split_stride, workspace, N, D, grid, hosted, stream);
    if (rc != QOT_OK) return rc;
    QOT_LAUNCH_CHECK();
    if (!gw1) return QOT_OK;
    const int n = K * (D + 1);
    gradh_partial_sum_kernel<<<grid_for(n, 4), 256, 0, stream>>>(workspace, grid, n, K * D, gw1, gb1);
    QOT_LAUNCH_CHECK();
    return QOT_OK;
}

extern "C" int qot_nnconv_gradh_fused(const float* grad_out, int ld_g, const float* x, int ld_x,
                                      const float* edge_attr, const float* w1, const float* b1,
                                      const int32_t* rowptr, const int32_t* col, const int32_t* eid,
                                      const float* invdeg, const float* b_perm, float* gw1, float* gb1,
                                      float* workspace, int64_t N, int H, int D, qot_stream_t stream) {
    return nnconv_gradh_impl(grad_out, ld_g, x, ld_x, edge_attr, w1, b1, rowptr, col, eid, invdeg, b_perm, nullptr, 0, gw1, gb1,
                             workspace, N, H, D, stream);
}

extern "C" int qot_nnconv_gradh_split(const float* grad_out, int ld_g, const float* x, int ld_x,
                                      const float* edge_attr, const float* w1, const float* b1,
                                      const int32_t* rowptr, const int32_t* col, const int32_t* eid,
                                      const float* invdeg, const void* b_split, int64_t split_stride, float* gw1, float* gb1,
                                      float* workspace, int64_t N, int H, int D, qot_stream_t stream) {
    if (!b_split) return QOT_ERR_BADARG;
    return nnconv_gradh_impl(grad_out, ld_g, x, ld_x, edge_attr, w1, b1, rowptr, col, eid, invdeg, nullptr, b_split, split_stride,
                             gw1, gb1,
                             workspace, N, H, D, stream);
}

extern "C" int qot_nnconv_bwd_finalize(const float* adj_workspace, const float* gradh_workspace, float* grad_params,
                                       float* gw1, float* gb1, int64_t N, int H, int D, qot_stream_t stream_) {
    if (N <= 0 || H != 64 || D < 1 || D > 4) return (H != 64 || D > 4) ? QOT_ERR_UNSUPPORTED : QOT_ERR_BADARG;
    qot_role_t r{};
    r.kind = QOT_ROLE_NNCONV_FINALIZE64;
    r.p[0] = adj_workspace; r.p[1] = gradh_workspace; r.p[2] = grad_params; r.p[3] = gw1; r.p[4] = gb1;
    r.i[0] = N; r.i[1] = D;
    return qot_run_roles(&r, 1, stream_);
}

extern "C" size_t qot_nnconv_adjoint_dw_workspace_floats(int D) {
    return (size_t)(num_cus() > 256 ? num_cus() : 256) * kAdjBlocksPerCu * (size_t)((2 * D + 2) * 64) * 64;
}

extern "C" int qot_nnconv_adjoint_dw(const float* grad_out, int ld_g, const float* x, int ld_x,
                                     const float* edge_attr, const float* w1, const float* b1,
                                     const int32_t* rowptr_t, const int32_t* col_t, const int32_t* eid_t,
                                     const float* invdeg, const float* w_perm, float* grad_x, float* gwcat_t,
                                     int param_layout, float* workspace, int64_t N, int H, int D,
                                     qot_stream_t stream_) {
    hipStream_t stream = (hipStream_t)stream_;
    if (N <= 0 || !rowptr_t) return QOT_ERR_BADARG;
    if (H != 64 || D > 4) return QOT_ERR_UNSUPPORTED;
    if (!grad_out || !x || !w1 || !b1 || !invdeg || !w_perm || !grad_x || !gwcat_t || !workspace || (ld_g & 3))
        return QOT_ERR_BADARG;
    int grid = grid_for(N, 32);
    const int cap = num_cus() * kAdjBlocksPerCu;
    if (grid > cap) grid = cap;
    const char* f32_env = getenv("QOT_NNCONV_F32_MFMA");
    const bool f32_mfma = f32_env && f32_env[0] == '1' && f32_env[1] == '\0';
    QOT_DISPATCH_D(D, {
        if (kD <= 4) {
            constexpr int kD4 = kD <= 4 ? kD : 4;
            if (f32_mfma)
                nnconv_adjoint_dw64_kernel<kD4, false><<<grid, 512, 0, stream>>>(
                    grad_out, ld_g, x, ld_x, edge_attr, w1, b1, rowptr_t, col_t, eid_t, invdeg, w_perm, grad_x,
                    workspace, N);
            else
                nnconv_adjoint_dw64_kernel<kD4, true><<<grid, 512, 0, stream>>>(
                    grad_out, ld_g, x, ld_x, edge_attr, w1, b1, rowptr_t, col_t, eid_t, invdeg, w_perm, grad_x,
                    workspace, N);
        }
    });
    QOT_LAUNCH_CHECK();
    if (param_layout == 2) return QOT_OK;
    const int64_t elems = (int64_t)(2 * D + 2) * 64 * 64;
    const int per_group = 16;
    const int groups = (grid + per_group - 1) / per_group;
    adj_slab_reduce_kernel<<<dim3(grid_for(elems / 4, 256), groups), 256, 0, stream>>>(
        workspace, grid, per_group, elems, elems, workspace, (int64_t)per_group * elems);
    QOT_LAUNCH_CHECK();
    if (param_layout)
        adj_slab_final_params_kernel<<<grid_for(elems / 4, 256), 256, 0, stream>>>(
            workspace, groups, elems, (int64_t)per_group * elems, gwcat_t, 2 * D);
    else
        adj_slab_reduce_kernel<<<dim3(grid_for(elems / 4, 256), 1), 256, 0, stream>>>(
            workspace, groups, groups, elems, (int64_t)per_group * elems, gwcat_t, 0);
    QOT_LAUNCH_CHECK();
    return QOT_OK;
}
```

### gnn_qot_estimation_amd/functional.py

```python
from __future__ import annotations

import os
from typing import Optional

import torch

from . import _lib, launch_group as LG
from .graph import GraphIndex, require_cuda

P = _lib.ptr


def _f32c(t: torch.Tensor) -> torch.Tensor:
    if t.dtype != torch.float32:
        raise TypeError("the HIP path computes in fp32; got %s" % t.dtype)
    return t.contiguous()


def _off(t: torch.Tensor, floats: int) -> int:
    return t.data_ptr() + 4 * floats


class EmbedFn(torch.autograd.Function):

# ... 532 lines not shown

class TConvGraphFn(torch.autograd.Function):

    @staticmethod
    def forward(ctx, table, wq, bq, wk, bk, wv, bv, ws, bs, w_edge, edge_attr, pre, graph: GraphIndex, maps, plan, act=None):
        t4, M, Pm = pre
        n, B, max_e = plan
        edge_attr, w_edge_c = _f32c(edge_attr), _f32c(w_edge.detach())
        require_cuda(edge_attr, t4, M, Pm)
        H, D = table.shape[1], w_edge.shape[1]
        N = graph.num_nodes
        if edge_attr.shape != (graph.num_edges_in, D):
            raise ValueError(f"edge_attr must be [{graph.num_edges_in}, {D}], got {tuple(edge_attr.shape)}")
        dev = t4.device
        out = torch.empty(N, H, dtype=torch.float32, device=dev)
        E = max(graph.num_edges_in, 1)
        alpha = torch.empty(E, dtype=torch.float32, device=dev)
        ea_csr = torch.empty(E, D, dtype=torch.float32, device=dev)
        aa = torch.empty(max(N, 1), D, dtype=torch.float32, device=dev)
        _lib.call("qot_tconv_fwd_graph", t4, 4 * H, M, Pm, w_edge_c, edge_attr, graph.rowptr, maps[1], graph.eid, graph.row,
                  out, alpha, ea_csr, aa, n, B, max_e, H, D, *_act_args(act))
        ctx.save_for_backward(table, wq, wk, wv, ws, w_edge_c, t4, alpha, ea_csr, aa, out if act is not None else None,
                              act[3] if act is not None else None, edge_attr if ctx.needs_input_grad[10] else None)
        ctx.graph, ctx.maps, ctx.plan = graph, maps, plan
        ctx.act = None if act is None else (act[0], act[1], act[2])
        return out

    @staticmethod
    def backward(ctx, g):
        table, wq, wk, wv, ws, w_edge, t4, alpha, ea_csr, aa, y, act_step, edge_attr = ctx.saved_tensors
        graph, maps = ctx.graph, ctx.maps
        n, B, max_e = ctx.plan
        g = _f32c(g)
        gea = tconv_edge_attr_grad(g, y, ctx.act, act_step, t4, edge_attr, w_edge, graph, maps) \
            if ctx.needs_input_grad[10] else None
        V, H = table.shape
        D = w_edge.shape[1]
        dev = g.device
        lib = _lib.load()
        blocks, rowlen = int(lib.qot_tconv_bwd_graph_blocks(B)), int(lib.qot_tconv_graph_row_floats(n, H, D))
        partials = torch.empty(blocks, rowlen, dtype=torch.float32, device=dev)
        if ctx.act is not None:
            slope, p, seed = ctx.act
            act_args = (y, float(slope), float(p if act_step is not None else 0.0), int(seed), act_step)
        else:
            act_args = (None, 0.0, 0.0, 0, None)
        _lib.call("qot_tconv_bwd_graph", g, *act_args, t4, 4 * H, w_edge, ea_csr, alpha, aa, graph.rowptr, maps[1],
                  graph.row, graph.rowptr_t, graph.col_t, graph.pos_t, partials, n, B, max_e, H, D)
        S = partials[0] if blocks == 1 else torch.empty(rowlen, dtype=torch.float32, device=dev)
        gt = torch.empty(V * H, dtype=torch.float32, device=dev)
        gw = torch.empty(4 * H * H, dtype=torch.float32, device=dev)
        gb = torch.empty(4 * H, dtype=torch.float32, device=dev)
        gwe = torch.empty(H, D, dtype=torch.float32, device=dev)
        wq_, wk_, wv_, ws_ = (_f32c(t.detach()) for t in (wq, wk, wv, ws))
        tab = _f32c(table.detach())
        if LG.enabled():
            if blocks > 1:
                LG.defer(_lib.ROLE_SUM_ROWS, (partials, S), (blocks, rowlen, 0), stage=1)
            LG.defer(_lib.ROLE_TABLE_PROJECT_BWD_SCORES, (S, t4, w_edge, tab, wq_, wk_, wv_, ws_, gt, gw, gb, gwe),
                     (V, n, H, D), stage=2)
            LG.flush()
        else:
            if blocks > 1:
                wsr = torch.empty(lib.qot_rowsum_wide_workspace_floats(rowlen), dtype=torch.float32, device=dev)
                _lib.call("qot_rowsum_wide", partials, blocks, rowlen, S, wsr)
            _lib.call("qot_table_project_bwd_scores", S, t4, w_edge, tab, wq_, wk_, wv_, ws_, gt, gw, gb, gwe, V, n, H, D)
        gw2 = gw.view(4 * H, H)
        return (gt.view(V, H), gw2[:H], gb[:H], gw2[H:2 * H], gb[H:2 * H], gw2[2 * H:3 * H], gb[2 * H:3 * H], gw2[3 * H:],
                gb[3 * H:], gwe, gea, None, None, None, None, None)


def nnconv_wcat(w2, b2, wroot, hin, hout, k):
    return torch.cat([
        w2.view(hin, hout, k).permute(2, 0, 1).reshape(k * hin, hout),
        b2.view(hin, hout),
        wroot.t(),
    ], dim=0)


def nnconv_wcat_t(w2, b2, wroot, hin, hout, k):
    return torch.cat([
        w2.view(hin, hout, k).permute(2, 1, 0).reshape(k * hout, hin),
        b2.view(hin, hout).t(),
        wroot,
    ], dim=0)


def gemm_tn(a: torch.Tensor, g: torch.Tensor) -> torch.Tensor:
    n, kt = a.shape
    if g.shape[1] != 64 or kt % 128 != 0 or kt > 1280 or n == 0 or os.environ.get("QOT_DISABLE_GEMM_TN"):
        return a.t() @ g
    a, g = a.contiguous(), g.contiguous()
    out = torch.empty(kt, 64, dtype=torch.float32, device=a.device)
    ws = torch.empty(_lib.load().qot_gemm_tn_workspace_floats(kt), dtype=torch.float32, device=a.device)
    _lib.call("qot_gemm_tn", P(a), kt, P(g), 64, n, kt, P(out), P(ws))
    return out


_PERM_CACHE = {}


def nnconv_perm_index(kt: int, device) -> torch.Tensor:
    key = (kt, str(device))
    if key not in _PERM_CACHE:
        nh, g, l, r = torch.meshgrid(torch.arange(2), torch.arange(kt // 8), torch.arange(64), torch.arange(4),
                                     indexing="ij")
        k = 8 * g + 2 * r + (l >> 5)
        n = nh * 32 + (l & 31)
        _PERM_CACHE[key] = (k * 64 + n).reshape(-1).to(device)
    return _PERM_CACHE[key]


def nnconv_gradh_perm_index(k: int, device) -> torch.Tensor:
    key = ("gradh", k, str(device))
    if key not in _PERM_CACHE:
        nb, gq, l, r = torch.meshgrid(torch.arange(2 * k), torch.arange(8), torch.arange(64), torch.arange(4),
                                      indexing="ij")
        o = 8 * gq + 2 * r + (l >> 5)
        n = nb * 32 + (l & 31)
        _PERM_CACHE[key] = (n * 64 + o).reshape(-1).to(device)
    return _PERM_CACHE[key]


def nnconv_fused_indices(k: int, device):
    key = ("fusedidx", k, str(device))
    if key not in _PERM_CACHE:
        h = 64
        kk, a, o = torch.meshgrid(torch.arange(k), torch.arange(h), torch.arange(h), indexing="ij")
        w2_off = (a * h + o) * k + kk
        a2, o2 = torch.meshgrid(torch.arange(h), torch.arange(h), indexing="ij")
        b2_off = h * h * k + a2 * h + o2
        root_off = h * h * k + h * h + o2 * h + a2
        wcat_idx = torch.cat([w2_off.reshape(k * h, h), b2_off, root_off], 0)
        wcat_t_idx = wcat_idx.view(k + 2, h, h).transpose(1, 2).reshape((k + 2) * h, h)
        fwd = wcat_idx.reshape(-1)[nnconv_perm_index((k + 2) * h, "cpu")]
        adj = wcat_t_idx.reshape(-1)[nnconv_perm_index((k + 2) * h, "cpu")]
        gh = wcat_idx[:k * h].reshape(-1)[nnconv_gradh_perm_index(k, "cpu")]
        allidx = torch.cat([fwd, adj, gh]).to(torch.int32).contiguous().to(device)
        _PERM_CACHE[key] = (allidx, fwd.numel(), adj.numel(), gh.numel())
    return _PERM_CACHE[key]


def nnconv_pack_operands(w2, b2, wroot, k: int):
    allidx, n_f, n_a, n_g = nnconv_fused_indices(k, w2.device)
    packed = torch.empty(allidx.numel(), dtype=torch.float32, device=w2.device)
    _lib.call("qot_gather3", P(w2), w2.numel(), P(b2), b2.numel(), P(wroot), P(allidx), P(packed), allidx.numel())
    return packed[:n_f], packed[n_f:n_f + n_a], packed[n_f + n_a:]


def nnconv_split_bf16() -> bool:
    return os.environ.get("QOT_NNCONV_F32_MFMA", "0") != "1"


def nnconv_split_index(k: int, device) -> torch.Tensor:
    key = ("splitidx", k, str(device))
    if key not in _PERM_CACHE:
        allidx, n_f, n_a, n_g = nnconv_fused_indices(k, "cpu")
        fwd = allidx[:n_f].view(2, -1, 2, 64, 4).permute(0, 1, 3, 2, 4)
        gh = allidx[n_f + n_a:].view(2 * k, 4, 2, 64, 4).permute(0, 1, 3, 2, 4)
        _PERM_CACHE[key] = torch.cat([fwd.reshape(-1), gh.reshape(-1)]).contiguous().to(device)
    return _PERM_CACHE[key]


def nnconv_pack(w2, b2, wroot, h: int, k: int, group=None):
    allidx, n_f, n_a, n_g = nnconv_fused_indices(k, w2.device) if h == 64 else nnconv_gen_indices(h, k, w2.device)
    packed = torch.empty(allidx.numel(), dtype=torch.float32, device=w2.device)
    ptrs, ints = [w2, b2, wroot, allidx, packed], [w2.numel(), b2.numel(), allidx.numel()]
    split = None
    if h == 64 and nnconv_split_bf16():
        sidx = nnconv_split_index(k, w2.device)
        split = torch.empty(3 * sidx.numel(), dtype=torch.int16, device=w2.device)
        ptrs, ints = ptrs + [sidx, split], ints + [sidx.numel()]
    if group is not None:
        group.add(_lib.ROLE_GATHER3, tuple(ptrs), tuple(ints))
    else:
        _lib.run_roles([_lib.make_role(_lib.ROLE_GATHER3, ptrs, ints)])
    return packed[:n_f], packed[n_f:n_f + n_a], packed[n_f + n_a:], split


GEN_WIDTHS = (16, 32, 128, 256)


def nnconv_gen_indices(h: int, k: int, device, cw: int = 0):
    key = ("genidx", h, k, str(device), cw)
    if key not in _PERM_CACHE:
        cw = cw or min(h, 64)
        n_pass, ncb, gall = h // cw, (h + 31) // 32, (k + 2) * cw // 8
        P_, CB, G_, L_, R_ = torch.meshgrid(torch.arange(n_pass), torch.arange(ncb), torch.arange(gall), torch.arange(64),
                                            torch.arange(4), indexing="ij")
        kl = 8 * G_ + 2 * R_ + (L_ >> 5)
        kk, a = kl // cw, P_ * cw + kl % cw
        col = CB * 32 + (L_ & 31)

        def wcat_off(kk, a, o):
            return torch.where(kk < k, (a * h + o) * k + kk,
                               torch.where(kk == k, h * h * k + a * h + o, h * h * (k + 1) + o * h + a))
        pad = col >= h
        colc = col.clamp(max=h - 1)
        fwd = torch.where(pad, torch.full_like(col, -1), wcat_off(kk, a, colc))
        adj = torch.where(pad, torch.full_like(col, -1), wcat_off(kk, colc, a))
        cwg = min(h, 32)
        npg, nbg, gh_ = h // cwg, k * cwg // 32, h // 8
        P2, NB, GQ, L2, R2 = torch.meshgrid(torch.arange(npg), torch.arange(nbg), torch.arange(gh_), torch.arange(64),
                                            torch.arange(4), indexing="ij")
        o = 8 * GQ + 2 * R2 + (L2 >> 5)
        n = NB * 32 + (L2 & 31)
        kq, al = n // cwg, n % cwg
        gh = ((P2 * cwg + al) * h + o) * k + kq
        allidx = torch.cat([fwd.reshape(-1), adj.reshape(-1), gh.reshape(-1)]).to(torch.int32).contiguous().to(device)
        _PERM_CACHE[key] = (allidx, fwd.numel(), adj.numel(), gh.numel())
    return _PERM_CACHE[key]


def nnconv_pack_operands_gen(w2, b2, wroot, h: int, k: int):
    allidx, n_f, n_a, n_g = nnconv_gen_indices(h, k, w2.device)
    packed = torch.empty(allidx.numel(), dtype=torch.float32, device=w2.device)
    _lib.call("qot_gather3", P(w2), w2.numel(), P(b2), b2.numel(), P(wroot), P(allidx), P(packed), allidx.numel())
    return packed[:n_f], packed[n_f:n_f + n_a], packed[n_f + n_a:]


def nnconv_edge_attr_grad(GA, x, edge_attr, w1, b1, graph: GraphIndex):
    N, hin = x.shape
    E, D = edge_attr.shape
    GA = GA.contiguous()
    gea = torch.empty(E, D, dtype=torch.float32, device=x.device)
    _lib.call("qot_nnconv_edge_attr_grad", GA, GA.shape[1], x, hin, edge_attr, w1, b1, graph.rowptr, graph.col, graph.eid,
              graph.invdeg, gea, N, hin, D)
    return gea


class NNConvFn(torch.autograd.Function):

    @staticmethod
    def forward(ctx, x, edge_attr, w1, b1, w2, b2, wroot, bias, graph: GraphIndex, act=None, side=None, packed=None):
        require_cuda(x, edge_attr, w1, b1, w2, b2, wroot, bias)
        ctx.receivers = (w1, b1, w2, b2, wroot)
        if side is not None and act is not None:
            side["bias_param"] = bias
        x, edge_attr = _f32c(x), _f32c(edge_attr)
        w1, b1, w2, b2, wroot, bias = (_f32c(t) for t in (w1, b1, w2, b2, wroot, bias))
        N, hin = x.shape
        hout = wroot.shape[0]
        K, D = w1.shape
        if K != 2 * D:
            raise _lib.QotError("NNConv edge MLP must be Linear(D, 2D) -> ReLU -> Linear(2D, Hin*Hout)")
        if edge_attr.shape != (graph.num_edges_in, D):
            raise ValueError(f"edge_attr must be [{graph.num_edges_in}, {D}], got {tuple(edge_attr.shape)}")
        if hin != hout:
            raise _lib.QotError("NNConv HIP path needs in_channels == out_channels")
        if hin != 64 and hin not in GEN_WIDTHS:
            raise _lib.QotError(f"NNConv HIP path: hidden width {hin} not in (16, 32, 64, 128, 256)")
        if D > 8:
            raise _lib.QotError("NNConv HIP path: edge_dim <= 8 (include/qot_gnn.h)")
        if D > 4:
            return NNConvFn._forward_wide_edge(ctx, x, edge_attr, w1, b1, w2, b2, wroot, bias, graph, act, side)
        wp, wp_adj, bp, split = packed if packed is not None else nnconv_pack(w2, b2, wroot, hin, K)
        out = torch.empty(N, hout, dtype=torch.float32, device=x.device)
        if split is not None:
            _lib.call("qot_nnconv_fused_split", P(x), hin, P(edge_attr), P(w1), P(b1), P(graph.rowptr), P(graph.col),
                      P(graph.eid), P(graph.invdeg), P(split), split.numel() // 3, P(bias), P(out), N, hin, D,
                      *_act_args(act))
        else:
            _lib.call("qot_nnconv_fused", P(x), hin, P(edge_attr), P(w1), P(b1), P(graph.rowptr), P(graph.col),
                      P(graph.eid), P(graph.invdeg), 0, P(wp), P(bias), P(out), N, hin, D, *_act_args(act))
        ctx.save_for_backward(x, edge_attr, w1, b1, w2, b2, wroot, None, wp_adj, bp, out if act is not None else None,
                              act[3] if act is not None else None, split)
        ctx.n_wcat = wp.numel()
        ctx.graph = graph
        ctx.act = None if act is None else (act[0], act[1], act[2])
        ctx.side = side if act is not None else None
        return out

    @staticmethod
    def _forward_wide_edge(ctx, x, edge_attr, w1, b1, w2, b2, wroot, bias, graph, act, side):
        N, hin = x.shape
        hout = wroot.shape[0]
        K, D = w1.shape
        A = torch.empty(N, (K + 2) * hin, dtype=torch.float32, device=x.device)
        _lib.call("qot_nnconv_agg", P(x), hin, P(edge_attr), P(w1), P(b1), P(graph.rowptr), P(graph.col),
                  P(graph.eid), None, P(graph.invdeg), 0, P(A), N, hin, D)
        out = torch.addmm(bias, A, nnconv_wcat(w2, b2, wroot, hin, hout, K))
        if act is not None:
            pre = out
            out = torch.empty_like(pre)
            _lib.call("qot_act_fwd", P(pre), P(out), pre.numel(), *_act_args(act)[1:])
        ctx.save_for_backward(x, edge_attr, w1, b1, w2, b2, wroot, A, None, None, out if act is not None else None,
                              act[3] if act is not None else None, None)
        ctx.graph = graph
        ctx.act = None if act is None else (act[0], act[1], act[2])
        ctx.side = side if act is not None else None
        return out

    @staticmethod
    def _backward_wide_edge(ctx, g, gbias):
        x, edge_attr, w1, b1, w2, b2, wroot, A, _, _, _, _, _ = ctx.saved_tensors
        graph = ctx.graph
        N, hin = x.shape
        hout = wroot.shape[0]
        K, D = w1.shape
        dev = x.device
        gwcat = gemm_tn(A, g)
        gx = None
        if ctx.needs_input_grad[0]:
            U = torch.empty(N, (K + 2) * hout, dtype=torch.float32, device=dev)
            _lib.call("qot_nnconv_agg", P(g), hout, P(edge_attr), P(w1), P(b1), P(graph.rowptr_t), P(graph.col_t),
                      P(graph.pos_t), P(graph.eid), P(graph.invdeg), 1, P(U), N, hout, D)
            gx = U @ nnconv_wcat_t(w2, b2, wroot, hin, hout, K)
        gw2 = gwcat[:K * hin].view(K, hin, hout).permute(1, 2, 0).reshape(hin * hout, K)
        gb2 = gwcat[K * hin:(K + 1) * hin].reshape(hin * hout)
        gwroot = gwcat[(K + 1) * hin:].t()
        wk = w2.view(hin, hout, K).permute(2, 0, 1).reshape(K * hin, hout)
        GA = (g @ wk.t()).contiguous()
        gw1 = torch.zeros(K, D, dtype=torch.float32, device=dev)
        gb1 = torch.zeros(K, dtype=torch.float32, device=dev)
        _lib.call("qot_nnconv_bwd_edge", P(GA), K * hin, P(x), hin, P(edge_attr), P(w1), P(b1),
                  P(graph.rowptr), P(graph.col), P(graph.eid), P(graph.invdeg), P(gw1), P(gb1), N, hin, D)
        gea = nnconv_edge_attr_grad(GA, x, edge_attr, w1, b1, graph) if ctx.needs_input_grad[1] else None
        return gx, gea, gw1, gb1, gw2, gb2, gwroot, gbias, None, None, None, None

    @staticmethod
    def backward(ctx, g):
        x, edge_attr, w1, b1, w2, b2, wroot, A, wp_adj, bp, y, act_step, split = ctx.saved_tensors
        graph = ctx.graph
        g = _f32c(g)
        if ctx.side is not None:
            if "gbias" not in ctx.side:
                raise RuntimeError("NNConv output was folded into the fused read-out, but the read-out's backward "
                                   "has not run: the conv output must feed only the read-out head "
                                   "(set model._qot_fold_head = False for other graphs)")
            gbias = ctx.side.pop("gbias")
        elif ctx.act is not None:
            g, gbias = act_backward_colsum(g, y, ctx.act + (act_step,))
        else:
            gbias = colsum(g)
        if A is not None:
            return NNConvFn._backward_wide_edge(ctx, g, gbias)
        N, hin = x.shape
        hout = wroot.shape[0]
        K, D = w1.shape
        dev = x.device
        hh = hin * hout
        gea = None
        if ctx.needs_input_grad[1]:
            wk = w2.view(hin, hout, K).permute(2, 0, 1).reshape(K * hin, hout)
            gea = nnconv_edge_attr_grad(g @ wk.t(), x, edge_attr, w1, b1, graph)
        gw1f = torch.empty(K * D, dtype=torch.float32, device=dev)
        gb1f = torch.empty(K, dtype=torch.float32, device=dev)
        gw1, gb1 = gw1f.view(K, D), gb1f.view(K)
        wsh = torch.empty(_lib.load().qot_nnconv_gradh_workspace_floats(D), dtype=torch.float32, device=dev)
        gpar = torch.empty((K + 2) * hh, dtype=torch.float32, device=dev)
        gradh_args = (P(g), hout, P(x), hin, P(edge_attr), P(w1), P(b1), P(graph.rowptr), P(graph.col), P(graph.eid),
                      P(graph.invdeg))
        if split is not None:
            gradh_fn, gradh_args = "qot_nnconv_gradh_split", gradh_args + (P(split[ctx.n_wcat:]), split.numel() // 3)
        else:
            gradh_fn, gradh_args = "qot_nnconv_gradh_fused", gradh_args + (P(bp),)
        if hin == 64 and not os.environ.get("QOT_SPLIT_NNCONV_BWD"):
            gx = torch.empty(N, hin, dtype=torch.float32, device=dev)
            ws = torch.empty(_lib.load().qot_nnconv_adjoint_dw_workspace_floats(D), dtype=torch.float32, device=dev)
            deferred = LG.can_defer(*ctx.receivers)
            _lib.call("qot_nnconv_adjoint_dw", P(g), hout, P(x), hin, P(edge_attr), P(w1), P(b1), P(graph.rowptr_t),
                      P(graph.col_t), P(graph.eid_t), P(graph.invdeg), P(wp_adj), P(gx), P(gpar), 2, P(ws), N, hin, D)
            if deferred and LG.hosted_sums():
                LG.defer(_lib.ROLE_NNCONV_SLAB_SUM64, (ws, None, gpar), (N, D), stage=1)
                LG.defer_gradh(gradh_fn, gradh_args + (None, None, P(wsh), N, hin, D),
                               (_lib.ROLE_NNCONV_GRADH_SUM64, (None, wsh, None, gw1f, gb1f), (N, D)),
                               keep=(g, x, edge_attr, w1, b1, graph, split, bp))
            else:
                _lib.call(gradh_fn, *gradh_args, None, None, P(wsh), N, hin, D)
                if deferred:
                    LG.defer(_lib.ROLE_NNCONV_FINALIZE64, (ws, wsh, gpar, gw1f, gb1f), (N, D), stage=1)
                else:
                    _lib.call("qot_nnconv_bwd_finalize", P(ws), P(wsh), P(gpar), P(gw1f), P(gb1f), N, hin, D)
        else:
            gx = None
            if ctx.needs_input_grad[0]:
                gx = torch.empty(N, hin, dtype=torch.float32, device=dev)
                _lib.call("qot_nnconv_fused", P(g), hout, P(edge_attr), P(w1), P(b1), P(graph.rowptr_t),
                          P(graph.col_t), P(graph.eid_t), P(graph.invdeg), 1, P(wp_adj), None, P(gx), N, hout, D,
                          0, 0.0, 0.0, 0, None)
            ws = torch.empty(_lib.load().qot_nnconv_dw_workspace_floats(N, hin, D), dtype=torch.float32, device=dev)
            _lib.call("qot_nnconv_dw", P(x), hin, P(g), hout, P(edge_attr), P(w1), P(b1), P(graph.rowptr), P(graph.col),
                      P(graph.eid), P(graph.invdeg), P(gpar), P(ws), N, hin, D)
            _lib.call(gradh_fn, *gradh_args, P(gw1), P(gb1), P(wsh), N, hin, D)
        gw2, gb2, gwroot = gpar[:hh * K].view(hh, K), gpar[hh * K:hh * (K + 1)], gpar[hh * (K + 1):].view(hout, hin)
        return gx, gea, gw1, gb1, gw2, gb2, gwroot, gbias, None, None, None, None


class ActFn(torch.autograd.Function):

    @staticmethod
    def forward(ctx, x, slope, p, seed, step_counter):
        require_cuda(x)
        x = _f32c(x)
        y = torch.empty_like(x)
        _lib.call("qot_act_fwd", P(x), P(y), x.numel(), float(slope), float(p), int(seed), P(step_counter))
        ctx.save_for_backward(y, step_counter if step_counter is not None else torch.empty(0))
        ctx.cfg = (float(slope), float(p), int(seed), step_counter is not None)
        return y

    @staticmethod
    def backward(ctx, g):
        y, counter = ctx.saved_tensors
        slope, p, seed, has_counter = ctx.cfg
        g = _f32c(g)
        gx = torch.empty_like(g)
        _lib.call("qot_act_bwd", P(g), P(y), P(gx), g.numel(), slope, p, seed, P(counter) if has_counter else None)
        return gx, None, None, None, None


class PoolFn(torch.autograd.Function):
    @staticmethod
    def forward(ctx, x, batch32, ptr32, B):
        require_cuda(x)
        x = _f32c(x)
        N, H = x.shape
        out = torch.empty(B, H, dtype=torch.float32, device=x.device)
        _lib.call("qot_pool_fwd", P(x), P(ptr32), P(out), B, H)
        ctx.save_for_backward(batch32, ptr32)
        ctx.dims = (N, H, B)
        return out

    @staticmethod
    def backward(ctx, g):
        batch32, ptr32 = ctx.saved_tensors
        N, H, B = ctx.dims
        g = _f32c(g)
        gx = torch.empty(N, H, dtype=torch.float32, device=g.device)
        _lib.call("qot_pool_bwd", P(g), P(ptr32), P(batch32), P(gx), N, B, H)
        return gx, None, None, None


class HeadFn(torch.autograd.Function):

    @staticmethod
    def forward(ctx, x, ptr32, w0, b0, w3, b3, B, act, in_act=None, side=None, loss=None):
        require_cuda(x, w0, b0, w3, b3)
        ctx.receivers = (w0, b0, w3, b3)
        x, w0, b0, w3, b3 = (_f32c(t) for t in (x, w0, b0, w3, b3))
        N, H = x.shape
        O = w3.shape[0]
        slope, p, seed, step = act
        dev = x.device
        pooled = torch.empty(B, H, dtype=torch.float32, device=dev)
        hidden = torch.empty(B, H, dtype=torch.float32, device=dev)
        out = torch.empty(B, O, dtype=torch.float32, device=dev)
        gout = loss_rows = None
        fold = in_act is not None and side is not None
        ctx.train_fused = None
        if loss is not None:
            target, beta, loss_out = loss[:3]
            target = _f32c(target.detach())
            if target.shape != (B, O):
                raise ValueError(f"target must be [{B}, {O}], got {tuple(target.shape)}")
            gout = torch.empty(B, O, dtype=torch.float32, device=dev)
            loss_rows = torch.empty(B, dtype=torch.float32, device=dev)
            ctx.loss = (loss_rows, loss_out)
            if len(loss) > 3 and loss[3] and not os.environ.get("QOT_NO_HEAD_TRAIN"):
                nb = H * H + H + O * H + O
                gx = torch.empty(N, H, dtype=torch.float32, device=dev)
                ws = torch.empty(_lib.load().qot_head_bwd_workspace_floats(H, O), dtype=torch.float32, device=dev)
                fa = (1, float(in_act[0]), float(in_act[1] if in_act[3] is not None else 0.0), int(in_act[2]), P(in_act[3])) \
                    if fold else (0, 0.0, 0.0, 0, None)
                _lib.call("qot_head_train", P(x), P(ptr32), P(w0), P(b0), P(w3), P(b3), P(target), float(beta), P(out), P(gout),
                          P(loss_rows), P(gx), P(ws), B, H, O, float(slope), float(p if step is not None else 0.0), int(seed),
                          P(step), *fa)
                ctx.train_fused = (gx, ws, gout, nb + (H if fold else 0))
                ctx.cfg = (N, H, O, B, float(slope), float(p if step is not None else 0.0), int(seed))
                ctx.fold = fold
                ctx.side = side if fold else None
                ctx.mark_non_differentiable(gout)
                ctx.set_materialize_grads(False)
                return out, gout
            _lib.call("qot_head_fwd_loss", P(x), P(ptr32), P(w0), P(b0), P(w3), P(b3), P(pooled), P(hidden), P(out), B, H,
                      O, float(slope), float(p if step is not None else 0.0), int(seed), P(step), P(target), float(beta),
                      P(gout), P(loss_rows))
        else:
            _lib.call("qot_head_fwd", P(x), P(ptr32), P(w0), P(b0), P(w3), P(b3), P(pooled), P(hidden), P(out), B, H, O,
                      float(slope), float(p if step is not None else 0.0), int(seed), P(step))
            ctx.loss = None
        ctx.save_for_backward(ptr32, w0, w3, pooled, hidden, step, x if fold else None,
                              in_act[3] if fold else None)
        ctx.cfg = (N, H, O, B, float(slope), float(p if step is not None else 0.0), int(seed))
        ctx.fold = (float(in_act[0]), float(in_act[1] if in_act[3] is not None else 0.0), int(in_act[2])) if fold else None
        ctx.side = side if fold else None
        if loss is not None:
            ctx.mark_non_differentiable(gout)
            ctx.set_materialize_grads(False)
            return out, gout
        return out

    @staticmethod
    def _backward_train_fused(ctx, g):
        gx, ws, gout, ntot = ctx.train_fused
        N, H, O, B, slope, p, seed = ctx.cfg
        if g is None or g.data_ptr() != gout.data_ptr() or g.shape != gout.shape:
            raise RuntimeError("the read-out ran its backward inside forward_loss with the criterion's own gradient: call "
                               "out.backward(g) with the g forward_loss returned (or use forward() + a criterion)")
        nb = H * H + H + O * H + O
        grads = torch.empty(ntot, dtype=torch.float32, device=gx.device)
        loss_rows, loss_out = ctx.loss
        roles = [(_lib.ROLE_SUM_ROWS, (ws, grads), (_lib.load().qot_head_train_blocks(B, H), ntot, 0)),
                 (_lib.ROLE_SUM_ROWS, (loss_rows, loss_out), (B, 1, 0))]
        if LG.can_defer(*ctx.receivers, ctx.side.get("bias_param") if ctx.fold else None):
            for r in roles:
                LG.defer(*r, stage=1)
        else:
            _lib.run_roles([_lib.make_role(*r) for r in roles])
        if ctx.fold:
            ctx.side["gbias"] = grads[nb:]
        gw0 = grads[:H * H].view(H, H)
        gb0 = grads[H * H:H * H + H]
        gw3 = grads[H * H + H:H * H + H + O * H].view(O, H)
        gb3 = grads[H * H + H + O * H:H * H + H + O * H + O]
        return gx, None, gw0, gb0, gw3, gb3, None, None, None, None, None

    @staticmethod
    def backward(ctx, g, _g_gout=None):
        if ctx.train_fused is not None:
            return HeadFn._backward_train_fused(ctx, g)
        ptr32, w0, w3, pooled, hidden, step, x_in, in_step = ctx.saved_tensors
        N, H, O, B, slope, p, seed = ctx.cfg
        if g is None:
            g = torch.zeros(B, O, dtype=torch.float32, device=pooled.device)
        g = _f32c(g)
        dev = g.device
        gx = torch.empty(N, H, dtype=torch.float32, device=dev)
        nb = H * H + H + O * H + O
        ntot = nb + (H if ctx.fold else 0)
        grads = torch.empty(ntot, dtype=torch.float32, device=dev)
        ws = torch.empty(_lib.load().qot_head_bwd_workspace_floats(H, O), dtype=torch.float32, device=dev)
        fold_args = (P(x_in), ctx.fold[0], ctx.fold[1], ctx.fold[2], P(in_step)) if ctx.fold else (None, 0.0, 0.0, 0, None)
        grouped = LG.can_defer(*ctx.receivers, ctx.side.get("bias_param") if ctx.fold else None)
        _lib.call("qot_head_bwd", P(g), P(pooled), P(hidden), P(ptr32), P(w0), P(w3), P(gx), None if grouped else P(grads),
                  P(ws), B, H, O, slope, p, seed, P(step), *fold_args)
        if grouped:
            LG.defer(_lib.ROLE_SUM_ROWS, (ws, grads), (_lib.load().qot_head_bwd_blocks(B), ntot, 0), stage=1)
        if ctx.loss is not None:
            loss_rows, loss_out = ctx.loss
            role = (_lib.ROLE_SUM_ROWS, (loss_rows, loss_out), (B, 1, 0))
            if LG.enabled():
                LG.defer(*role, stage=1)
            else:
                _lib.run_roles([_lib.make_role(*role)])
        if ctx.fold:
            ctx.side["gbias"] = grads[nb:]
        gw0 = grads[:H * H].view(H, H)
        gb0 = grads[H * H:H * H + H]
        gw3 = grads[H * H + H:H * H + H + O * H].view(O, H)
        gb3 = grads[H * H + H + O * H:H * H + H + O * H + O]
        return gx, None, gw0, gb0, gw3, gb3, None, None, None, None, None


class GatFn(torch.autograd.Function):

    @staticmethod
    def forward(ctx, z, att_src, att_dst, bias, graph: GraphIndex, neg_slope: float, bn_stats: bool = False,
                a_src=None, a_dst=None, logits_sink=None):
        require_cuda(z, att_src, att_dst, bias)
        z, bias = _f32c(z), _f32c(bias)
        heads, C = att_src.shape[-2], att_src.shape[-1]
        att_s, att_d = _f32c(att_src).reshape(-1), _f32c(att_dst).reshape(-1)
        N, HC = z.shape
        dev = z.device
        if a_src is None or a_dst is None:
            a_src = torch.empty(N, heads, dtype=torch.float32, device=dev)
            a_dst = torch.empty(N, heads, dtype=torch.float32, device=dev)
            _lib.call("qot_gat_logits", P(z), P(att_s), P(att_d), P(a_src), P(a_dst), N, heads, C)
        else:
            a_src, a_dst = _f32c(a_src), _f32c(a_dst)
        if logits_sink is not None:
            logits_sink.append((a_src, a_dst))
        out = torch.empty(N, HC, dtype=torch.float32, device=dev)
        stats = torch.empty(N, heads, 2, dtype=torch.float32, device=dev)
        partials = None
        if bn_stats and N > 0:
            partials = torch.empty(_lib.load().qot_gat_bn_partials_floats(N, heads, C), dtype=torch.float32, device=dev)
        _lib.call("qot_gat_fwd", P(z), P(a_src), P(a_dst), P(bias), P(graph.rowptr), P(graph.col), P(out),
                  P(stats), N, heads, C, float(neg_slope), P(partials))
        ctx.save_for_backward(z, a_src, a_dst, stats, att_s, att_d)
        ctx.graph, ctx.ns, ctx.att_shape = graph, float(neg_slope), tuple(att_src.shape)
        if bn_stats:
            if partials is None:
                partials = torch.empty(0, dtype=torch.float32, device=dev)
            ctx.mark_non_differentiable(partials)
            return out, partials
        return out

    @staticmethod
    def backward(ctx, g, _gp=None):
        z, a_src, a_dst, stats, att_s, att_d = ctx.saved_tensors
        graph, ns = ctx.graph, ctx.ns
        g = _f32c(g)
        N, HC = z.shape
        heads = a_src.shape[1]
        C = HC // heads
        dev = z.device
        gad = torch.empty(N, heads, dtype=torch.float32, device=dev)
        gas = torch.empty(N, heads, dtype=torch.float32, device=dev)
        gz = torch.empty(N, HC, dtype=torch.float32, device=dev)
        escr = torch.empty(max(graph.cap, 1), heads, 2, dtype=torch.float32, device=dev)
        delta = torch.empty(N, heads, dtype=torch.float32, device=dev)
        g_bias = torch.empty(HC, dtype=torch.float32, device=dev)
        ws = torch.empty(_lib.load().qot_gat_bn_partials_floats(N, heads, C), dtype=torch.float32, device=dev)
        _lib.call("qot_gat_bwd_dst", P(g), P(z), P(a_src), P(a_dst), P(stats), P(graph.rowptr), P(graph.col),
                  P(gad), P(escr), P(delta), N, heads, C, ns, P(g_bias), P(ws))
        _lib.call("qot_gat_bwd_src", P(g), P(a_src), P(a_dst), P(escr), P(delta), P(graph.rowptr_t),
                  P(graph.col_t), P(graph.pos_t), P(gz), P(gas), N, heads, C, ns, P(att_s), P(att_d), P(gad))
        g_att = torch.empty(2, HC, dtype=torch.float32, device=dev)
        _lib.call("qot_gat_att_grad", P(z), P(gas), P(gad), _off(g_att, 0), _off(g_att, HC), P(ws), N, heads, C)
        return gz, g_att[0].view(ctx.att_shape), g_att[1].view(ctx.att_shape), g_bias, None, None, None, None, None, None


def gat_thin_ok(x: torch.Tensor, heads: int, C: int) -> bool:
    if os.environ.get("QOT_NO_GAT_THIN", "0") == "1" or not x.is_cuda or x.dtype != torch.float32 or x.requires_grad:
        return False
    if x.dim() != 2 or x.shape[0] < int(os.environ.get("QOT_GAT_THIN_MIN_ROWS", "32768")) or not skinny_ok(x.shape[1], 4):
        return False
    return bool(_lib.load().qot_gat_thin_supported(heads, C, x.shape[1]))
# ... 403 lines not shown
```

### gnn_qot_estimation_amd/graph.py

```python
from __future__ import annotations

from dataclasses import dataclass
from typing import Optional

import os

import torch

from . import _lib


@dataclass
class GraphIndex:
    num_nodes: int
    num_edges_in: int
    cap: int
    rowptr: torch.Tensor
    col: torch.Tensor
    eid: torch.Tensor
    row: torch.Tensor
    rowptr_t: torch.Tensor
    col_t: torch.Tensor
    pos_t: torch.Tensor
    eid_t: torch.Tensor
# ... 69 lines not shown
        pos_t=torch.empty(max(cap, 1), **i32), eid_t=torch.empty(max(cap, 1), **i32),
        invdeg=torch.empty(max(N, 1), dtype=torch.float32, device=dev),
        gat_self_loops=gat_self_loops,
    )
    lib = _lib.load()
    if slices is not None and not gat_self_loops:
        node_ptr, edge_ptr, max_n, max_m = slices
        B = node_ptr.numel() - 1
        if (B >= 1 and edge_ptr.numel() == B + 1 and node_ptr.is_cuda and edge_ptr.is_cuda
                and node_ptr.dtype == torch.long and edge_ptr.dtype == torch.long
                and int(max_n) <= 65535 and (5 * int(max_n) + 2 + 6 * int(max_m)) * 4 <= 144 * 1024):
            g.ptr32 = torch.empty(B + 1, **i32)
            ids = None
            if node_ids is not None and node_ids.is_cuda and node_ids.dtype == torch.long and node_ids.numel() == N:
                ids = node_ids.contiguous()
                g.ids32 = torch.empty(N, **i32)
                g.colf, g.colf_t = torch.empty(max(E, 1), **i32), torch.empty(max(E, 1), **i32)
            np_c, ep_c = node_ptr.contiguous(), edge_ptr.contiguous()
            status = _index_status(dev)
            g.sizes = (int(max_n), int(max_m))
            if group is not None and B >= 1:
                group.add(_lib.ROLE_CSR_BY_GRAPH, (ei, np_c, ep_c, g.rowptr, g.col, g.eid, g.row, g.rowptr_t, g.col_t,
                                                   g.pos_t, g.eid_t, g.invdeg, status, ids, g.ids32, g.colf, g.colf_t,
                                                   g.ptr32), (E, N, B, int(max_n), int(max_m)))
                if CHECK_INDEX_STATUS:
                    group.post.append(lambda: check_index_status(dev))
                return g
            _lib.call("qot_csr_build_by_graph", ei, E, N, np_c, ep_c, B, int(max_n), int(max_m), g.rowptr, g.col,
                      g.eid, g.row, g.rowptr_t, g.col_t, g.pos_t, g.eid_t, g.invdeg, status, ids, g.ids32, g.colf,
                      g.colf_t, g.ptr32)
            if CHECK_INDEX_STATUS:
                check_index_status(dev)
            return g
    if slices is not None and gat_self_loops:
        node_ptr, edge_ptr, max_n, max_m = slices
        B = node_ptr.numel() - 1
        if (B >= 1 and edge_ptr.numel() == B + 1 and node_ptr.is_cuda and edge_ptr.is_cuda and node_ptr.dtype == torch.long
                and edge_ptr.dtype == torch.long and lib.qot_csr_gat_by_graph_supported(int(max_n), int(max_m))):
            g.ptr32 = torch.empty(B + 1, **i32)
            np_c, ep_c = node_ptr.contiguous(), edge_ptr.contiguous()
            status = _index_status(dev)
            _lib.call("qot_csr_build_gat_by_graph", ei, E, N, np_c, ep_c, B, int(max_n), int(max_m), g.rowptr, g.col, g.eid,
                      g.row, g.rowptr_t, g.col_t, g.pos_t, g.eid_t, g.invdeg, status, g.ptr32)
            if CHECK_INDEX_STATUS and check:
                check_index_status(dev)
            else:
                g.status_pending = CHECK_INDEX_STATUS
            return g
    ws_bytes = lib.qot_csr_workspace_bytes(E, N, int(gat_self_loops))
    if ws_bytes == 0:
        raise _lib.QotError("qot_csr_workspace_bytes failed")
    ws = torch.empty(ws_bytes, dtype=torch.uint8, device=dev)
    _lib.call("qot_csr_build", _lib.ptr(ei), E, N, int(gat_self_loops), _lib.ptr(g.rowptr), _lib.ptr(g.col),
              _lib.ptr(g.eid), _lib.ptr(g.row), _lib.ptr(g.rowptr_t), _lib.ptr(g.col_t), _lib.ptr(g.pos_t),
              _lib.ptr(g.eid_t), _lib.ptr(g.invdeg), _lib.ptr(ws), ws_bytes)
    return g


def _cache(data) -> Optional[dict]:
    c = getattr(data, "_qot_cache", None)
    if c is None:
        c = {}
        try:
            setattr(data, "_qot_cache", c)
        except Exception:
            return None
    return c


def graph_index_for(data, num_nodes: int, gat_self_loops: bool = False, group=None, check: bool = True) -> GraphIndex:
    ei = data.edge_index
    key = ("graph", bool(gat_self_loops))
    tag = (ei.data_ptr(), ei._version, tuple(ei.shape), int(num_nodes))
    c = _cache(data)
    if c is not None and key in c and c[key][0] == tag:
        return c[key][1]
    slices = None
    ptr, eptr, sizes = getattr(data, "ptr", None), getattr(data, "edge_ptr", None), getattr(data, "graph_sizes", None)
    if eptr is None and not gat_self_loops and ptr is not None:
        sd = getattr(data, "_slice_dict", None)
        es = sd.get("edge_index") if isinstance(sd, dict) else None
        if isinstance(es, torch.Tensor) and es.dim() == 1 and es.numel() == ptr.numel() and es.numel() >= 2:
            es = es.to(torch.long).cpu()
            pc = ptr.detach().to("cpu", torch.long) if c is None or "ptr_host" not in c else c["ptr_host"]
            eptr = es.to(ei.device)
            sizes = (int((pc[1:] - pc[:-1]).max()), int((es[1:] - es[:-1]).max()))
            if c is not None:
                c["ptr_host"] = pc
    if (ptr is not None and eptr is not None and sizes is not None and ptr.numel() == eptr.numel() and ptr.is_cuda
            and eptr.is_cuda and (not gat_self_loops or (getattr(data, "has_self_loops", None) is False
                                                         and os.environ.get("QOT_NO_GAT_BY_GRAPH", "0") != "1"))):
        slices = (ptr, eptr, sizes[0], sizes[1])
    ids = getattr(data, "node_ids", None) if (slices is not None and getattr(data, "uniform_node_ids", None)) else None
    g = build_graph_index(ei, num_nodes, gat_self_loops, slices, ids, group=group, check=check)
    if c is not None:
        def remember():
            c[key] = (tag, g)
            if g.ptr32 is not None:
                c["ptr32"] = ((ptr.data_ptr(), ptr._version, tuple(ptr.shape)), (g.ptr32, ptr.numel() - 1))
        if group is not None and group.roles:
            group.on_success.append(remember)
        else:
            remember()
    return g


def to_i32(t: torch.Tensor) -> torch.Tensor:
    require_cuda(t)
    t = t.contiguous()
    if t.dtype == torch.int32:
        return t
    if t.dtype != torch.long:
        raise ValueError("expected an int64 index tensor")
    out = torch.empty(t.shape, dtype=torch.int32, device=t.device)
    _lib.call("qot_i64_to_i32", _lib.ptr(t), _lib.ptr(out), t.numel())
    return out


def batch_index_for(data, num_nodes: int):
    batch = data.batch
    tag = (batch.data_ptr(), batch._version, tuple(batch.shape))
    c = _cache(data)
    if c is not None and "batch" in c and c["batch"][0] == tag:
        return c["batch"][1]
    B = getattr(data, "num_graphs", None)
    if B is None:
        B = int(batch.max().item()) + 1 if batch.numel() else 0
    B = int(B)
    b32 = to_i32(batch)
    ptr = torch.empty(B + 1, dtype=torch.int32, device=batch.device)
    _lib.call("qot_batch_ptr", _lib.ptr(b32), int(num_nodes), B, _lib.ptr(ptr))
    res = (b32, ptr, B)
    if c is not None:
        c["batch"] = (tag, res)
    return res


def batch_ptr_for(data, num_nodes: int):
    ptr = getattr(data, "ptr", None)
    B = getattr(data, "num_graphs", None)
    if ptr is None or B is None or ptr.numel() != int(B) + 1 or not ptr.is_cuda:
        _, p32, B = batch_index_for(data, num_nodes)
        return p32, B
    tag = (ptr.data_ptr(), ptr._version, tuple(ptr.shape))
    c = _cache(data)
    if c is not None and "ptr32" in c and c["ptr32"][0] == tag:
        return c["ptr32"][1]
    res = (to_i32(ptr), int(B))
    if c is not None:
        c["ptr32"] = (tag, res)
    return res


def cached_i32(data, name: str) -> torch.Tensor:
    t = getattr(data, name)
    tag = (t.data_ptr(), t._version, tuple(t.shape))
    c = _cache(data)
    key = ("i32", name)
    if c is not None and key in c and c[key][0] == tag:
        return c[key][1]
    out = to_i32(t)
    if c is not None:
        c[key] = (tag, out)
    return out


def _detect_uniform_node_ids(data, N: int) -> None:
    ids, ptr, B = getattr(data, "node_ids", None), getattr(data, "ptr", None), getattr(data, "num_graphs", None)
    found = None
    try:
        capturing = torch.cuda.is_current_stream_capturing()
    except Exception:
        capturing = False
    if (not capturing and ids is not None and ptr is not None and B and ids.is_cuda and ptr.is_cuda
            and ids.numel() == N and N % int(B) == 0 and ptr.numel() == int(B) + 1):
        n = N // int(B)
        ar = torch.arange(n, device=ids.device, dtype=ids.dtype)
        ok = (ids.view(int(B), n) == ar).all() & (ptr == torch.arange(int(B) + 1, device=ptr.device, dtype=ptr.dtype) * n).all()
        if bool(ok.item()):
            found = n
    if capturing:
        return
    try:
        data.uniform_node_ids = found
    except Exception:
        pass


def table_maps_for(data, graph: GraphIndex, group=None):
    if not hasattr(data, "uniform_node_ids"):
        _detect_uniform_node_ids(data, graph.num_nodes)
    n = getattr(data, "uniform_node_ids", None)
    if not n:
        return None
    N = graph.num_nodes
    if N % n != 0:
        return None
    ids = data.node_ids
    tag = (ids.data_ptr(), ids._version, graph.col.data_ptr())
    c = _cache(data)
    if c is not None and "tmaps" in c and c["tmaps"][0] == tag:
        return c["tmaps"][1]
    if graph.colf is not None and graph.ids32 is not None:
        res = (graph.ids32, graph.colf, graph.colf_t, (N // n, int(n)))
        if c is not None:
            if group is not None and group.roles:
                group.on_success.append(lambda: c.__setitem__("tmaps", (tag, res)))
            else:
                c["tmaps"] = (tag, res)
        return res
    require_cuda(ids)
    if group is not None and group.roles:
        group.run()
    if ids.dtype != torch.int64:
        ids = ids.long()
    ids = ids.contiguous()
    E = graph.num_edges_in
    dev = ids.device
    ids32 = torch.empty(N, dtype=torch.int32, device=dev)
    colf = torch.empty(max(E, 1), dtype=torch.int32, device=dev)
    colf_t = torch.empty(max(E, 1), dtype=torch.int32, device=dev)
    _lib.call("qot_table_maps", _lib.ptr(ids), _lib.ptr(graph.col), _lib.ptr(graph.col_t), _lib.ptr(ids32),
              _lib.ptr(colf), _lib.ptr(colf_t), N, E)
    res = (ids32, colf, colf_t, (N // n, int(n)))
    if c is not None:
        c["tmaps"] = (tag, res)
    return res
```

### gnn_qot_estimation_amd/topological.py

```python
from __future__ import annotations

import torch
from torch import nn

from . import _lib, functional as QF, launch_group as LG
from .graph import batch_index_for, batch_ptr_for, cached_i32, graph_index_for, table_maps_for
from .nn import NNConv, TransformerConv


class TopologicalGNN(nn.Module):
    def __init__(self, num_nodes, hidden_channels, out_channels, edge_dim, dropout_p=0.5, num_layers=2):
        super().__init__()
        if num_layers < 2:
            raise ValueError("num_layers >= 2 (TransformerConv + NNConv is the reference model)")
        self.node_embeddings = nn.Embedding(num_nodes, hidden_channels)
        self.conv1 = TransformerConv(hidden_channels, hidden_channels, edge_dim=edge_dim)
        for layer in range(2, num_layers + 1):
            edge_nn = nn.Sequential(
                nn.Linear(edge_dim, edge_dim * 2),
                nn.ReLU(),
                nn.Linear(edge_dim * 2, hidden_channels * hidden_channels),
            )
            setattr(self, f"conv{layer}", NNConv(hidden_channels, hidden_channels, nn=edge_nn, aggr="mean"))
        self.mlp = nn.Sequential(
            nn.Linear(hidden_channels, hidden_channels),
            nn.LeakyReLU(),
            nn.Dropout(p=dropout_p),
            nn.Linear(hidden_channels, out_channels),
        )
        self.dropout = nn.Dropout(p=dropout_p)
        self.num_layers = num_layers
        from .padded import WIDTHS, padded_width
        self._qot_hp = None if hidden_channels in WIDTHS else padded_width(hidden_channels)
        self._qot_shadow = None
        self.register_buffer("_qot_step", torch.zeros((), dtype=torch.long), persistent=False)
        self._qot_seed = None

    def _act(self, site: int, step):
        p = self.dropout.p if self.training else 0.0
        seed = (self._seed() + 0x9E3779B97F4A7C15 * (site + 1)) & 0xFFFFFFFFFFFFFFFF
        return (0.01, p, seed, step if p > 0.0 else None)

    def _seed(self) -> int:
        if self._qot_seed is None:
            import torch.distributed as dist
            rank = dist.get_rank() if (dist.is_available() and dist.is_initialized()) else 0
            self._qot_seed = (int(torch.initial_seed()) + 0xD1B54A32D192ED03 * rank) & 0x7FFFFFFFFFFFFFFF
        return self._qot_seed

    def _check_node_ids(self, data, maps):
        V = self.node_embeddings.num_embeddings
        if maps is not None:
            if int(maps[3][1]) > V:
                raise IndexError("index out of range in self")
            return
        ids = data.node_ids
        c = getattr(data, "_qot_cache", None)
        tag = (ids.data_ptr(), ids._version, tuple(ids.shape), V)
        if isinstance(c, dict) and c.get("ids_ok") == tag:
            return
        if ids.numel():
            if torch.cuda.is_current_stream_capturing():
                return
            lo, hi = torch.aminmax(ids)
            if int(lo) < 0 or int(hi) >= V:
                raise IndexError("index out of range in self")
        if isinstance(c, dict):
            c["ids_ok"] = tag

    def _forward_padded(self, data, attention: bool = False):
        from . import padded
        if data.x is not None and data.x.numel():
            raise NotImplementedError("explicit node features with a padded hidden width")
        if self._qot_shadow is None or self._qot_shadow[0].node_embeddings.weight.device != self.node_embeddings.weight.device:
            shadow = TopologicalGNN(self.node_embeddings.num_embeddings, self._qot_hp, self.mlp[3].out_features,
                                    self.conv1.edge_dim, dropout_p=self.dropout.p, num_layers=self.num_layers)
            shadow.to(self.node_embeddings.weight.device)
            for p in shadow.parameters():
                p.requires_grad_(False)
            self._qot_shadow = (shadow,)
        shadow = self._qot_shadow[0]
        shadow.train(self.training)
        shadow.dropout.p = shadow.mlp[2].p = self.dropout.p
        shadow._qot_seed = self._seed()
        state = padded.topological_params(self, self._qot_hp)
        state["_qot_step"] = self._qot_step
        kwargs = {"return_attention_weights": True} if attention else {}
        return torch.func.functional_call(shadow, state, (data,), kwargs)

    def forward_loss(self, data, target, beta: float = 1.0, loss_out=None):
        res = self._forward(data, (target, float(beta), loss_out))
        if isinstance(res, tuple):
            out, gout, loss = res
            return out, loss, gout
        loss, gout = QF.smooth_l1_loss_and_grad(res, target, beta, loss_out=loss_out)
        return res, loss, gout

    def forward(self, data, return_attention_weights=False):
        if return_attention_weights:
            return self._forward(data, None, attention=True)
        return self._forward(data, None)

    def _forward(self, data, loss_spec, attention: bool = False):
        if not self.node_embeddings.weight.is_cuda:
            from . import auto_device
            if auto_device.enabled():
                return auto_device.forward(self, data, return_attention_weights=attention)
            raise auto_device.cpu_model_error()
        if self._qot_hp is not None:
            return self._forward_padded(data, attention)
        x, edge_index, edge_attr = data.x, data.edge_index, data.edge_attr
        LG.drop_stale()
        grp = LG.LaunchGroup() if LG.enabled() else None
        maps = None
        if x is None or x.numel() == 0:
            n = data.node_ids.shape[0]
            graph = graph_index_for(data, n, group=grp)
            maps = table_maps_for(data, graph, group=grp)
            self._check_node_ids(data, maps)
            if maps is None:
                if grp is not None:
                    grp.run()
                x = QF.EmbedFn.apply(self.node_embeddings.weight, cached_i32(data, "node_ids"))
        else:
            n = x.shape[0]
            graph = graph_index_for(data, n, group=grp)
        step, step_pair = None, None
        if self.training and self.dropout.p > 0.0:
            step = torch.empty_like(self._qot_step)
            if maps is not None:
                step_pair = (self._qot_step, step)
            else:
                _lib.call("qot_step_advance", _lib.ptr(self._qot_step), _lib.ptr(step))
        plan = self.conv1.graph_form(self.node_embeddings.weight, graph, maps) if maps is not None else None
        t4 = pre = None
        if plan is not None:
            pre = self.conv1.prepare_graph_form(self.node_embeddings.weight, plan, step_pair, grp)
        elif maps is not None:
            t4 = self.conv1.project_table(self.node_embeddings.weight, step_pair, grp)
        packed = {layer: getattr(self, f"conv{layer}").prepack(grp) for layer in range(2, self.num_layers + 1)}
        if grp is not None:
            grp.run()
        attn = None
        if plan is not None:
            x = self.conv1.forward_table_graph(self.node_embeddings.weight, edge_attr, graph, maps, plan, pre,
                                               act=self._act(0, step))
            if attention:
                c1 = self.conv1
                attn = (edge_index, c1.attention_weights(pre[0], edge_attr, graph, maps,
                                                         (self.node_embeddings.weight, c1.lin_query.weight,
                                                          c1.lin_key.weight)))
        elif maps is not None:
            x = self.conv1.forward_table(self.node_embeddings.weight, edge_attr, graph, maps, act=self._act(0, step),
                                         step_pair=step_pair, t4=t4)
            if attention:
                attn = (edge_index, self.conv1.attention_weights(t4, edge_attr, graph, maps))
        elif attention:
            x, attn = self.conv1(x, edge_index, edge_attr, graph=graph, act=self._act(0, step), return_attention_weights=True)
        else:
            x = self.conv1(x, edge_index, edge_attr, graph=graph, act=self._act(0, step))
        l0, l3 = self.mlp[0], self.mlp[3]
        width = self.node_embeddings.embedding_dim
        fused_head = width in (16, 32, 64, 128) and l3.out_features <= 8 and l0.out_features == width
        side = {} if (fused_head and torch.is_grad_enabled() and getattr(self, "_qot_fold_head", True)) else None
        last_act = None
        for layer in range(2, self.num_layers + 1):
            act_l = self._act(layer - 1, step)
            last = layer == self.num_layers
            if last:
                last_act = act_l
            x = getattr(self, f"conv{layer}")(x, edge_index, edge_attr, graph=graph, act=act_l,
                                              side=side if last else None, packed=packed[layer])
        if fused_head:
            p = self.mlp[2].p if self.training else 0.0
            seed = (self._seed() + 0x9E3779B97F4A7C15 * 97) & 0xFFFFFFFFFFFFFFFF
            act = (self.mlp[1].negative_slope, p, seed, step if p > 0.0 else None)
            ptr, B = batch_ptr_for(data, n)
            if loss_spec is not None and torch.is_grad_enabled():
                target, beta, loss_out = loss_spec
                if loss_out is None:
                    loss_out = torch.full((), float("nan"), dtype=torch.float32, device=x.device)
                out, gout = QF.HeadFn.apply(x, ptr, l0.weight, l0.bias, l3.weight, l3.bias, B, act,
                                            last_act if side is not None else None, side, (target, beta, loss_out, True))
                return out, gout, loss_out
            out = QF.HeadFn.apply(x, ptr, l0.weight, l0.bias, l3.weight, l3.bias, B, act,
                                  last_act if side is not None else None, side)
        else:
            b32, ptr, B = batch_index_for(data, n)
            x = QF.PoolFn.apply(x, b32, ptr, B)
            out = self._head(x)
        return out if attn is None else (out, attn)

    def _head(self, x):
        l0, act, drop, l3 = self.mlp[0], self.mlp[1], self.mlp[2], self.mlp[3]
        h = QF.SmallLinearFn.apply(x, l0.weight, l0.bias)
        return QF.SmallLinearFn.apply(drop(act(h)), l3.weight, l3.bias)
```

### include/qot_gnn.h

```cpp
#ifndef QOT_GNN_H
#define QOT_GNN_H

#include <stddef.h>
#include <stdint.h>

#ifdef __cplusplus
extern "C" {
#endif

typedef void* qot_stream_t;

#define QOT_ABI_VERSION 13
#define QOT_OK 0
#define QOT_ERR_UNSUPPORTED (-1)
#define QOT_ERR_BADARG (-2)

int qot_abi_version(void);
const char* qot_error_string(int code);

size_t qot_csr_workspace_bytes(int64_t E, int64_t N, int gat_self_loops);
int qot_csr_build(const int64_t* edge_index, int64_t E, int64_t N, int gat_self_loops,
                  int32_t* rowptr, int32_t* col, int32_t* eid, int32_t* row,
                  int32_t* rowptr_t, int32_t* col_t, int32_t* pos_t, int32_t* eid_t, float* invdeg,
                  void* workspace, size_t workspace_bytes, qot_stream_t stream);
int qot_csr_build_by_graph(const int64_t* edge_index, int64_t E, int64_t N, const int64_t* node_ptr,
                           const int64_t* edge_ptr, int64_t B, int64_t max_nodes, int64_t max_edges,
                           int32_t* rowptr, int32_t* col, int32_t* eid, int32_t* row, int32_t* rowptr_t,
                           int32_t* col_t, int32_t* pos_t, int32_t* eid_t, float* invdeg, int32_t* status,
                           const int64_t* node_ids, int32_t* ids32, int32_t* colf, int32_t* colf_t, int32_t* ptr32,
                           qot_stream_t stream);
int qot_csr_gat_by_graph_supported(int64_t max_nodes, int64_t max_edges);
int qot_csr_build_gat_by_graph(const int64_t* edge_index, int64_t E, int64_t N, const int64_t* node_ptr,
                               const int64_t* edge_ptr, int64_t B, int64_t max_nodes, int64_t max_edges, int32_t* rowptr,
                               int32_t* col, int32_t* eid, int32_t* row, int32_t* rowptr_t, int32_t* col_t, int32_t* pos_t,
                               int32_t* eid_t, float* invdeg, int32_t* status, int32_t* ptr32, qot_stream_t stream);
int qot_i32_gather(const int32_t* map, const int32_t* idx, int32_t* out, int64_t n, qot_stream_t stream);
int qot_i64_to_i32(const int64_t* in, int32_t* out, int64_t n, qot_stream_t stream);
int qot_batch_ptr(const int32_t* batch, int64_t N, int64_t B, int32_t* ptr, qot_stream_t stream);

int qot_embed_fwd(const float* table, const int32_t* ids, float* out, int64_t N, int V, int H,
                  qot_stream_t stream);
int qot_embed_bwd(const float* grad_out, const int32_t* ids, float* grad_table, int64_t N, int V,
                  int H, qot_stream_t stream);

int qot_tconv_fwd_scores(const float* q, const float* v, const float* skip, int ld, const float* scores, int ld_scores,
                         const float* edge_attr, const float* w_edge, const int32_t* rowptr, const int32_t* col,
                         const int32_t* eid, const int32_t* rowmap, float* out, float* stats, int64_t N, int H, int D,
                         int act, float act_slope, float act_p, uint64_t act_seed, const int64_t* act_step,
                         qot_stream_t stream);
int qot_tconv_rows_supported(int n, int H, int D);
int qot_tconv_rows_npad(int n);
int qot_tconv_rows_ld(int n, int H, int D);
int qot_tconv_bwd_dst_rows(const float* grad_out, const float* q, const float* v, int ld, const float* edge_attr,
                           const float* w_edge, const float* stats, const int32_t* rowptr, const int32_t* colf,
                           const int32_t* eid, const float* scores, int ld_scores, float* grad_skip, float* escr, float* delta,
                           const float* y_act, float act_slope, float act_p, uint64_t act_seed, const int64_t* act_step, int n,
                           int64_t B, int parts, float* part_rows, float* wedge_partials, int H, int D, qot_stream_t stream);
int qot_tconv_fwd_rows(const float* q, const float* v, const float* skip, int ld, const float* scores, int ld_scores,
                       const float* edge_attr, const float* w_edge, const int32_t* rowptr, const int32_t* colf, const int32_t* eid,
                       float* out, float* stats, int n, int64_t B, int parts, int H, int D, int act, float act_slope, float act_p,
                       uint64_t act_seed, const int64_t* act_step, qot_stream_t stream);
int qot_tconv_bwd_src_rows(const float* grad_skip, const float* escr, const int32_t* rowptr_t, const int32_t* col_t,
                           const int32_t* pos_t, int n, int64_t B, int parts, float* part_rows, int H, qot_stream_t stream);
int qot_tconv_fwd(const float* q, const float* k, const float* v, const float* skip, int ld,
                  const float* edge_attr, const float* w_edge, const int32_t* rowptr,
                  const int32_t* col, const int32_t* eid, const int32_t* rowmap, float* out,
                  float* stats, int64_t N, int H, int D, int act, float act_slope, float act_p,
                  uint64_t act_seed, const int64_t* act_step, qot_stream_t stream);
int qot_tconv_fwd_tile(const float* q, const float* k, const float* v, const float* skip, int ld,
                       const float* edge_attr, const float* w_edge, const int32_t* rowptr, const int32_t* col,
                       const int32_t* eid, const int32_t* rowmap, float* out, float* stats, int64_t N, int H, int D,
                       int tile_n, int64_t tile_B, int act, float act_slope, float act_p, uint64_t act_seed,
                       const int64_t* act_step, qot_stream_t stream);
int qot_tconv_rows_per_block(int H);
int64_t qot_tconv_bwd_dst_blocks(int64_t N, int H, int tile_n, int64_t tile_B);
size_t qot_tconv_bwd_dst_workspace_floats(int64_t N, int H, int D);
int qot_tconv_bwd_dst(const float* grad_out, const float* q, const float* k, const float* v, int ld,
                      const float* edge_attr, const float* w_edge, const float* stats,
                      const int32_t* rowptr, const int32_t* col, const int32_t* eid,
                      const int32_t* rowmap, float* grad_q, float* grad_skip, int ld_g, float* escr,
                      float* delta, float* pds, float* pal, const float* y_act, float act_slope, float act_p,
                      uint64_t act_seed, const int64_t* act_step, float* grad_w_edge, float* workspace,
                      int tile_n, int64_t tile_B, float* grad_part, int64_t N, int H, int D, qot_stream_t stream);
int qot_tconv_bwd_src(const float* grad_out, int ld_go, const float* q, int ld, const float* escr,
                      const float* delta, const int32_t* rowptr_t, const int32_t* col_t,
                      const int32_t* pos_t, const int32_t* qmap_t, float* grad_k, float* grad_v,
                      int ld_g, int tile_n, int64_t tile_B, float* grad_part, int64_t N, int H,
                      qot_stream_t stream);

int qot_tconv_graph_supported(int n, int max_e, int H, int D);
int qot_tconv_graph_ldm(int n);
size_t qot_tconv_graph_row_floats(int n, int H, int D);
int qot_tconv_bwd_graph_blocks(int64_t B);
int qot_table_scores(const float* table, const float* wq, const float* bq, const float* wk, const float* bk,
                     const float* w_edge, float* M, float* P, int n, int H, int D, qot_stream_t stream);
int qot_tconv_fwd_graph(const float* t4, int ld, const float* M, const float* P, const float* w_edge,
                        const float* edge_attr, const int32_t* rowptr, const int32_t* colf, const int32_t* eid,
                        const int32_t* row, float* out, float* alpha, float* ea_csr, float* aa, int n, int64_t B, int max_e,
                        int H, int D, int act, float act_slope, float act_p, uint64_t act_seed, const int64_t* act_step,
                        qot_stream_t stream);
int qot_tconv_bwd_graph(const float* grad_out, const float* y_act, float act_slope, float act_p, uint64_t act_seed,
                        const int64_t* act_step, const float* t4, int ld, const float* w_edge, const float* ea_csr,
                        const float* alpha, const float* aa, const int32_t* rowptr, const int32_t* colf,
                        const int32_t* row, const int32_t* rowptr_t, const int32_t* col_t, const int32_t* pos_t,
                        float* partials, int n, int64_t B, int max_e, int H, int D, qot_stream_t stream);
int qot_table_project_bwd_scores(const float* S, const float* t4, const float* w_edge, const float* table,
                                 const float* wq, const float* wk, const float* wv, const float* ws, float* grad_table,
                                 float* grad_w, float* grad_b, float* grad_w_edge, int V, int n, int H, int D,
                                 qot_stream_t stream);

int qot_nnconv_agg(const float* x, int ld_x, const float* edge_attr, const float* w1,
                   const float* b1, const int32_t* rowptr, const int32_t* col,
                   const int32_t* eid_or_pos, const int32_t* eid_of_pos, const float* invdeg,
                   int transpose, float* A, int64_t N, int H, int D, qot_stream_t stream);
int qot_nnconv_fused(const float* x, int ld_x, const float* edge_attr, const float* w1,
                     const float* b1, const int32_t* rowptr, const int32_t* col,
                     const int32_t* edge_ids, const float* invdeg, int transpose,
                     const float* w_perm, const float* bias, float* out, int64_t N, int H, int D,
                     int act, float act_slope, float act_p, uint64_t act_seed, const int64_t* act_step,
                     qot_stream_t stream);
int qot_nnconv_fused_split(const float* x, int ld_x, const float* edge_attr, const float* w1,
                           const float* b1, const int32_t* rowptr, const int32_t* col,
                           const int32_t* edge_ids, const float* invdeg, const void* w_split,
                           int64_t split_stride, const float* bias, float* out, int64_t N, int H, int D,
                           int act, float act_slope, float act_p, uint64_t act_seed, const int64_t* act_step,
                           qot_stream_t stream);
size_t qot_gemm_tn_workspace_floats(int KT);
int qot_gemm_tn(const float* A, int lda, const float* G, int ldg, int64_t N, int KT, float* C,
                float* workspace, qot_stream_t stream);
size_t qot_nnconv_adjoint_dw_workspace_floats(int D);
int qot_nnconv_adjoint_dw(const float* grad_out, int ld_g, const float* x, int ld_x,
                          const float* edge_attr, const float* w1, const float* b1,
                          const int32_t* rowptr_t, const int32_t* col_t, const int32_t* eid_t,
                          const float* invdeg, const float* w_perm, float* grad_x, float* gwcat_t, int param_layout,
                          float* workspace, int64_t N, int H, int D, qot_stream_t stream);
size_t qot_nnconv_gradh_workspace_floats(int D);
int qot_nnconv_gradh_fused(const float* grad_out, int ld_g, const float* x, int ld_x,
                           const float* edge_attr, const float* w1, const float* b1,
                           const int32_t* rowptr, const int32_t* col, const int32_t* eid,
                           const float* invdeg, const float* b_perm, float* gw1, float* gb1,
                           float* workspace, int64_t N, int H, int D, qot_stream_t stream);
int qot_nnconv_gradh_split(const float* grad_out, int ld_g, const float* x, int ld_x,
                           const float* edge_attr, const float* w1, const float* b1,
                           const int32_t* rowptr, const int32_t* col, const int32_t* eid,
                           const float* invdeg, const void* b_split, int64_t split_stride, float* gw1, float* gb1,
                           float* workspace, int64_t N, int H, int D, qot_stream_t stream);
size_t qot_nnconv_dw_workspace_floats(int64_t N, int H, int D);
int qot_nnconv_dw(const float* x, int ld_x, const float* grad_out, int ld_g, const float* edge_attr,
                  const float* w1, const float* b1, const int32_t* rowptr, const int32_t* col,
                  const int32_t* eid, const float* invdeg, float* grad_params, float* workspace, int64_t N,
                  int H, int D, qot_stream_t stream);
int qot_nnconv_bwd_finalize(const float* adj_workspace, const float* gradh_workspace, float* grad_params,
                            float* gw1, float* gb1, int64_t N, int H, int D, qot_stream_t stream);
int qot_nnconv_bwd_edge(const float* GA, int ld_ga, const float* x, int ld_x,
                        const float* edge_attr, const float* w1, const float* b1,
                        const int32_t* rowptr, const int32_t* col, const int32_t* eid,
                        const float* invdeg, float* gw1, float* gb1, int64_t N, int H, int D,
                        qot_stream_t stream);

int qot_tconv_edge_attr_grad(const float* grad_out, const float* y_act, float act_slope, float act_p, uint64_t act_seed,
                             const int64_t* act_step, const float* qkvs, int ld, const int32_t* rowmap, const int32_t* col,
                             const int32_t* rowptr, const int32_t* eid, const float* edge_attr, const float* w_edge,
                             float* grad_edge_attr, int64_t N, int H, int D, qot_stream_t stream);
int qot_nnconv_edge_attr_grad(const float* GA, int ld_ga, const float* x, int ld_x, const float* edge_attr,
                              const float* w1, const float* b1, const int32_t* rowptr, const int32_t* col,
                              const int32_t* eid, const float* invdeg, float* grad_edge_attr, int64_t N, int H, int D,
                              qot_stream_t stream);

int qot_tconv_attention(const float* qkvs, int ld, const int32_t* rowmap, const int32_t* col, const int32_t* rowptr,
                        const int32_t* eid, const float* edge_attr, const float* w_edge, float* alpha, int64_t N, int H,
                        int D, qot_stream_t stream);
int qot_gat_attention(const float* a_src, const float* a_dst, const int32_t* rowptr, const int32_t* col,
                      const int32_t* eid, const int32_t* edge_pos, int64_t num_kept, float* alpha, int64_t N, int heads,
                      float neg_slope, qot_stream_t stream);

int qot_act_fwd(const float* x, float* y, int64_t n, float slope, float p, uint64_t seed,
                const int64_t* step_counter, qot_stream_t stream);
int qot_act_bwd(const float* grad_y, const float* y_or_x, float* grad_x, int64_t n, float slope,
                float p, uint64_t seed, const int64_t* step_counter, qot_stream_t stream);

int qot_pool_fwd(const float* x, const int32_t* ptr, float* out, int64_t B, int H,
                 qot_stream_t stream);
int qot_pool_bwd(const float* grad_out, const int32_t* ptr, const int32_t* batch, float* grad_x,
                 int64_t N, int64_t B, int H, qot_stream_t stream);

int qot_gat_blocks(int64_t N, int heads, int C);
size_t qot_gat_bn_partials_floats(int64_t N, int heads, int C);
int qot_gat_logits(const float* z, const float* att_src, const float* att_dst, float* a_src, float* a_dst,
                   int64_t N, int heads, int C, qot_stream_t stream);
int qot_gat_fwd(const float* z, const float* a_src, const float* a_dst, const float* bias,
                const int32_t* rowptr, const int32_t* col, float* out, float* stats, int64_t N,
                int heads, int C, float neg_slope, float* bn_partials, qot_stream_t stream);
int qot_gat_thin_supported(int heads, int C, int K);
int qot_gat_fwd_thin(const float* x, int K, const float* w, const float* a_src, const float* a_dst, const float* bias,
                     const int32_t* rowptr, const int32_t* col, float* out, float* stats, int64_t N, int heads, int C,
                     float neg_slope, float* bn_partials, qot_stream_t stream);
int qot_gat_bwd_dst_thin(const float* grad_out, const float* x, int K, const float* w, const float* a_src,
                         const float* a_dst, const float* stats, const int32_t* rowptr, const int32_t* col,
                         float* grad_a_dst, float* escr, float* delta, int64_t N, int heads, int C, float neg_slope,
                         float* grad_bias, float* workspace, qot_stream_t stream);
int qot_gat_bwd_dst(const float* grad_out, const float* z, const float* a_src, const float* a_dst,
                    const float* stats, const int32_t* rowptr, const int32_t* col, float* grad_a_dst,
                    float* escr, float* delta, int64_t N, int heads, int C, float neg_slope,
                    float* grad_bias, float* workspace, qot_stream_t stream);
int qot_gat_bwd_src(const float* grad_out, const float* a_src, const float* a_dst, const float* escr,
                    const float* delta, const int32_t* rowptr_t, const int32_t* col_t,
                    const int32_t* pos_t, float* grad_z, float* grad_a_src, int64_t N, int heads,
                    int C, float neg_slope, const float* att_src, const float* att_dst,
                    const float* grad_a_dst, qot_stream_t stream);
int qot_gat_att_grad(const float* z, const float* grad_a_src, const float* grad_a_dst, float* grad_att_src,
                     float* grad_att_dst, float* workspace, int64_t N, int heads, int C, qot_stream_t stream);

size_t qot_bn_partials_floats(int64_t N, int C);
int qot_bn_stats(const float* x, int64_t N, int C, float eps, float momentum, float* mean,
                 float* rstd, float* running_mean, float* running_var, float* partials,
                 qot_stream_t stream);
int64_t qot_gat_chunk_rows(int64_t N, int heads, int C);
int qot_bn_stats_from_partials(const float* shift, const float* partials, int nblk, int64_t chunk_rows, int64_t N, int C,
                               float eps, float momentum, float* mean, float* rstd, float* running_mean,
                               float* running_var, qot_stream_t stream);
int qot_bn_apply(const float* x, const float* mean, const float* rstd, const float* w,
                 const float* b, float* y, int64_t N, int C, int relu, qot_stream_t stream);
int qot_bn_bwd_reduce(const float* grad_y, const float* y, const float* x, const float* mean,
                      const float* rstd, float* gw, float* gb, int64_t N, int C, int relu,
                      float* partials, const float* w, const float* b, qot_stream_t stream);
int qot_bn_bwd_apply(const float* grad_y, const float* y, const float* x, const float* mean,
                     const float* rstd, const float* w, const float* gw, const float* gb,
                     float* grad_x, int64_t N, int C, int relu, int batch_stats, const float* b,
                     qot_stream_t stream);
int qot_bn_apply_rows(const float* x, const int32_t* idx, int64_t n, const float* mean, const float* rstd, const float* w,
                      const float* b, float* y_rows, int C, int relu, qot_stream_t stream);
int qot_bn_bwd_reduce_rows(const float* grad_rows, const int32_t* idx, int64_t n, const float* x, const float* mean,
                           const float* rstd, float* gw, float* gb, int C, int relu, float* partials, const float* w,
                           const float* b, qot_stream_t stream);
int qot_bn_bwd_apply_rows(const float* grad_rows, const int32_t* idx, int64_t n, const float* x, const float* mean,
                          const float* rstd, const float* w, const float* gw, const float* gb, float* grad_x, int64_t N,
                          int C, int relu, const float* b, qot_stream_t stream);

int qot_sgd_momentum(float* param, const float* grad, float* momentum_buf, int64_t n, float lr,
                     float momentum, int first_step, qot_stream_t stream);
int qot_sgd_momentum_multi(float* param, const float* const* grads, const int64_t* offsets, int count,
                           float* grad_flat, float* momentum_buf, int64_t n, float lr, const float* lr_dev,
                           float momentum, int first_step, qot_stream_t stream);
int qot_sgd_momentum_dev(float* param, const float* grad, float* momentum_buf, int64_t n, const float* lr_dev,
                         float momentum, int first_step, qot_stream_t stream);
int qot_small_gemm(const float* A, int64_t stride_am, int64_t stride_ak, const float* B, int64_t stride_bk,
                   int64_t stride_bn, const float* bias, float* C, int ldc, int M, int N, int K,
                   int split_k, qot_stream_t stream);
size_t qot_colsum_workspace_floats(int C);
size_t qot_rowsum_wide_workspace_floats(int64_t C);
int qot_rowsum_wide(const float* x, int64_t B, int64_t C, float* out, float* workspace, qot_stream_t stream);
int qot_colsum(const float* x, int ld, int64_t N, int C, float* out, float* workspace, qot_stream_t stream);
int qot_act_bwd_colsum(const float* grad_y, const float* y, float* grad_x, int64_t N, int C, float slope, float p,
                       uint64_t seed, const int64_t* step_counter, float* colsum_out, float* workspace,
                       qot_stream_t stream);

int qot_head_fwd(const float* x, const int32_t* ptr, const float* w0, const float* b0, const float* w3,
                 const float* b3, float* pooled, float* hidden, float* out, int64_t B, int H, int O,
                 float slope, float p, uint64_t seed, const int64_t* step_counter, qot_stream_t stream);
int qot_head_fwd_loss(const float* x, const int32_t* ptr, const float* w0, const float* b0, const float* w3,
                      const float* b3, float* pooled, float* hidden, float* out, int64_t B, int H, int O,
                      float slope, float p, uint64_t seed, const int64_t* step_counter, const float* target,
                      float beta, float* grad_out, float* loss_rows, qot_stream_t stream);
int qot_head_train_blocks(int64_t B, int H);
int qot_head_train(const float* x, const int32_t* ptr, const float* w0, const float* b0, const float* w3, const float* b3,
                   const float* target, float beta, float* out, float* grad_out, float* loss_rows, float* grad_x,
                   float* workspace, int64_t B, int H, int O, float slope, float p, uint64_t seed,
                   const int64_t* step_counter, int fold, float in_slope, float in_p, uint64_t in_seed,
                   const int64_t* in_step, qot_stream_t stream);
size_t qot_head_bwd_workspace_floats(int H, int O);
int qot_head_bwd_blocks(int64_t B);
int qot_head_bwd(const float* grad_out, const float* pooled, const float* hidden, const int32_t* ptr,
                 const float* w0, const float* w3, float* grad_x, float* grads, float* workspace, int64_t B,
                 int H, int O, float slope, float p, uint64_t seed, const int64_t* step_counter,
                 const float* x_in, float in_slope, float in_p, uint64_t in_seed, const int64_t* in_step,
                 qot_stream_t stream);

size_t qot_smooth_l1_workspace_floats(void);
int qot_smooth_l1(const float* pred, const float* target, int64_t n, float beta, float* loss, float* grad,
                  float* workspace, qot_stream_t stream);

int qot_table_project_fwd(const float* table, const float* wq, const float* bq, const float* wk, const float* bk,
                          const float* wv, const float* bv, const float* ws, const float* bs, float* out, int V,
                          int H, int64_t* step_counter, int64_t* step_snapshot, qot_stream_t stream);
int qot_table_project_bwd(const float* grad_out, const float* table, const float* wq, const float* wk,
                          const float* wv, const float* ws, float* grad_table, float* grad_w, float* grad_b, int V,
                          int H, qot_stream_t stream);

int qot_table_maps(const int64_t* node_ids, const int32_t* col, const int32_t* col_t, int32_t* ids32,
                   int32_t* colf, int32_t* colf_t, int64_t N, int64_t E, qot_stream_t stream);
int qot_step_advance(int64_t* counter, int64_t* snapshot, qot_stream_t stream);

#define QOT_STAGE_BAD_SHAPE 1
#define QOT_STAGE_BAD_RANGE 2
#define QOT_STAGE_BAD_NODE_ID 4
int qot_shard_stage(int64_t* ctl, int64_t sched_cap, int32_t* status, const int64_t* node_ptr, const int64_t* edge_ptr,
                    const int64_t* graph_of_node, int64_t G, int64_t N_total, int64_t E_total, const int64_t* edge_index,
                    const void* edge_attr, int D, const int64_t* node_ids, const void* x, int F, const void* y, int Y,
                    int64_t B, int64_t N, int64_t E, int64_t max_nodes, int64_t max_edges, int64_t V,
                    int64_t* dst_edge_index, void* dst_edge_attr, int64_t* dst_node_ids, void* dst_x, void* dst_y,
                    int64_t* dst_ptr, int64_t* dst_edge_ptr, int64_t* dst_batch, qot_stream_t stream);
int qot_shard_stage_padded(int64_t* ctl, int64_t sched_cap, int32_t* status, const int64_t* node_ptr,
                           const int64_t* edge_ptr, const int64_t* graph_of_node, int64_t G, int64_t N_total,
                           int64_t E_total, const int64_t* edge_index, const void* edge_attr, int D,
                           const int64_t* node_ids, const void* x, int F, const void* y, int Y, int64_t B, int64_t n,
                           int64_t E_cap, int64_t P, int64_t max_edges, int64_t V, int64_t* dst_edge_index,
                           void* dst_edge_attr, int64_t* dst_node_ids, void* dst_x, void* dst_y, int64_t* dst_ptr,
                           int64_t* dst_edge_ptr, int64_t* dst_batch, qot_stream_t stream);
int qot_shard_stage_gather(int64_t* ctl, int64_t sched_cap, int32_t* status, int64_t* offs, const int64_t* node_ptr,
                           const int64_t* edge_ptr, int64_t G, int64_t N_total, int64_t E_total, const int64_t* edge_index,
                           const void* edge_attr, int D, const int64_t* node_ids, const void* x, int F, const void* y, int Y,
                           int64_t B, int64_t n, int64_t E_cap, int64_t P, int64_t max_edges, int64_t V,
                           int64_t* dst_edge_index, void* dst_edge_attr, int64_t* dst_node_ids, void* dst_x, void* dst_y,
                           int64_t* dst_ptr, int64_t* dst_edge_ptr, int64_t* dst_batch, qot_stream_t stream);

int qot_gather3(const float* s0, int64_t n0, const float* s1, int64_t n1, const float* s2, const int32_t* idx,
                float* out, int64_t n, qot_stream_t stream);

int qot_gemm_nt(const float* A, int64_t lda, const float* B, int64_t ldb, float* C, int64_t ldc, int64_t M, int N, int K,
                const float* scale, const float* shift, const float* bias, qot_stream_t stream);
int qot_gemm_nt_logits(const float* A, int64_t lda, const float* B, int64_t ldb, float* C, int64_t ldc, int64_t M, int N, int K,
                       const float* scale, const float* shift, const float* bias, const float* att_src,
                       const float* att_dst, float* a_src, float* a_dst, qot_stream_t stream);
int qot_gemm_nt_planes(const float* A, int64_t lda, const float* B, int64_t ldb, float* Cpart, int64_t M, int N, int K,
                       int kslices, qot_stream_t stream);
int qot_gemm_tn_splits(int M, int N, int64_t K);
int qot_gemm256_takes(int64_t M, int N);
int qot_gemm_tn_planes(const float* A, int64_t lda, const float* B, int64_t ldb, float* Cpart, int M, int N, int64_t K,
                       int splits, const float* scale, const float* shift, qot_stream_t stream);

int qot_skinny_linear_fwd(const float* x, const float* w, float* out, int64_t N, int F, int C, qot_stream_t stream);
int qot_skinny_linear_fwd_logits(const float* x, const float* w, float* out, int64_t N, int F, int C, const float* att_src,
                                 const float* att_dst, float* a_src, float* a_dst, qot_stream_t stream);
int qot_skinny_linear_dw_blocks(int64_t N);
int qot_skinny_linear_dw(const float* g, const float* x, float* partials, int64_t N, int F, int C, qot_stream_t stream);

#define QOT_MAX_ROLES 12
enum {
    QOT_ROLE_CSR_BY_GRAPH = 1,
    QOT_ROLE_TABLE_PROJECT_FWD = 2,
    QOT_ROLE_GATHER3 = 3,
    QOT_ROLE_SUM_ROWS = 4,
    QOT_ROLE_NNCONV_FINALIZE64 = 5,
    QOT_ROLE_TABLE_PROJECT_BWD = 6,
    QOT_ROLE_TABLE_SCORES = 7,
    QOT_ROLE_TABLE_PROJECT_BWD_SCORES = 8,
    QOT_ROLE_NNCONV_SLAB_SUM64 = 9,
    QOT_ROLE_NNCONV_GRADH_SUM64 = 10
};
typedef struct qot_role {
    int32_t kind;
    int32_t reserved;
    const void* p[18];
    int64_t i[8];
} qot_role_t;
int qot_run_roles(const qot_role_t* roles, int n_roles, qot_stream_t stream);

int qot_nnconv_gradh_host_roles(const qot_role_t* roles, int n_roles);

int qot_rows_gather(const float* x, const int32_t* idx, float* out, int64_t n_idx, int C,
                    qot_stream_t stream);
int qot_rows_scatter(const float* grad_out, const int32_t* idx, float* grad_x, int64_t n_idx, int C,
                     qot_stream_t stream);

int qot_topological_infer_supported(int n_max, int max_e, int H, int D, int O);
int qot_topological_infer_max_edges(int n_max, int H, int D);
int qot_topological_infer(const int64_t* node_ids, const int64_t* edge_index, const float* edge_attr,
                          const int64_t* node_ptr, const int64_t* edge_ptr, int64_t N, int64_t E, int64_t B, int n_max,
                          int max_e, const float* t4, int ld4, const float* M, int ldm, const float* P, int V,
                          const float* w_edge, const float* w1, const float* b1, const float* wcat, const float* bias2,
                          const float* w0, const float* b0, const float* w3, const float* b3, float slope_conv,
                          float slope_head, float* out, int H, int D, int O, int32_t* status, qot_stream_t stream);

int qot_topological_infer_mc_supported(int n_max, int max_e, int H, int D, int O);
int qot_topological_infer_mc_max_edges(int n_max, int H, int D);
int qot_topological_infer_mc(const int64_t* node_ids, const int64_t* edge_index, const float* edge_attr,
                             const int64_t* node_ptr, const int64_t* edge_ptr, int64_t N, int64_t E, int64_t B, int n_max,
                             int max_e, const float* t4, int ld4, const float* M, int ldm, const float* P, int V,
                             const float* w_edge, const float* w1, const float* b1, const float* wcat, const float* bias2,
                             const float* w0, const float* b0, const float* w3, const float* b3, float slope_conv,
                             float slope_head, float* samples, int H, int D, int O, int32_t* status, int T,
                             int64_t first_step, uint64_t base_seed, float p_conv, float p_head, int chunk,
                             qot_stream_t stream);

int qot_topological_infer_grad_supported(int n_max, int max_e, int H, int D, int O);
int qot_topological_infer_grad_max_edges(int n_max, int H, int D);
int qot_topological_infer_grad(const int64_t* node_ids, const int64_t* edge_index, const float* edge_attr,
                               const int64_t* node_ptr, const int64_t* edge_ptr, int64_t N, int64_t E, int64_t B, int n_max,
                               int max_e, const float* t4, int ld4, const float* M, int ldm, const float* P, int V,
                               const float* w_edge, const float* w1, const float* b1, const float* wcat, const float* bias2,
                               const float* w0, const float* b0, const float* w3, const float* b3, float slope_conv,
                               float slope_head, float* out, int H, int D, int O, int32_t* status, const int32_t* outputs,
                               int Q, float* jac, float* alpha, qot_stream_t stream);

int qot_topological_infer_whatif_supported(int n_max, int max_e, int H, int D, int O);
int qot_topological_infer_whatif_max_edges(int n_max, int H, int D);
int qot_topological_infer_whatif(const int64_t* node_ids, const int64_t* edge_index, const float* edge_attr,
                                 const int64_t* node_ptr, const int64_t* edge_ptr, int64_t N, int64_t E, int64_t B, int n_max,
                                 int max_e, const float* t4, int ld4, const float* M, int ldm, const float* P, int V,
                                 const float* w_edge, const float* w1, const float* b1, const float* wcat, const float* bias2,
                                 const float* w0, const float* b0, const float* w3, const float* b3, float slope_conv,
                                 float slope_head, float* out, int H, int D, int O, int32_t* status,
                                 const int64_t* add_edge_index, const float* add_edge_attr, const int64_t* add_ptr, int64_t A,
                                 const int64_t* drop, const int64_t* drop_ptr, int64_t R, const int64_t* graph, int64_t K,
                                 int max_add, qot_stream_t stream);

int qot_lightpath_infer(const float* x, const int64_t* edge_index, const int64_t* batch, const int64_t* node_ptr,
                        const int64_t* edge_ptr, const int64_t* lut_idx, int64_t L, int64_t N, int64_t E, int64_t B,
                        const float* w, const float* att_src, const float* att_dst, const float* conv_bias, float slope_att,
                        const float* bn_weight, const float* bn_bias, const float* bn_mean, const float* bn_var,
                        float bn_eps, const float* w0, const float* b0, const float* w3, const float* b3, float slope_head,
                        float* out, int32_t* count, int F, int C, int O, int heads, int lut_col, int32_t* status,
                        qot_stream_t stream);

int qot_lightpath_infer_grad(const float* x, const int64_t* edge_index, const int64_t* batch, const int64_t* node_ptr,
                             const int64_t* edge_ptr, const int64_t* lut_idx, int64_t L, int64_t N, int64_t E, int64_t B,
                             const float* w, const float* att_src, const float* att_dst, const float* conv_bias,
                             float slope_att, const float* bn_weight, const float* bn_bias, const float* bn_mean,
                             const float* bn_var, float bn_eps, const float* w0, const float* b0, const float* w3,
                             const float* b3, float slope_head, float* out, int32_t* count, int F, int C, int O, int heads,
                             int lut_col, int32_t* status, const int32_t* outputs, int Q, float* jac_self, float* jac_edge,
                             float* alpha_self, float* alpha_edge, qot_stream_t stream);
// ... 132 lines not shown
```

Measured before the change: 2.580 million graphs/s.

## Have last NNConv emit 4-row partial sums and activation codes for fused head

Result: no change. 2.606 million graphs/s (median of 6 runs) (+1.0%).

```diff
diff --git a/gnn_qot_estimation_amd/_lib.py b/gnn_qot_estimation_amd/_lib.py
--- a/gnn_qot_estimation_amd/_lib.py
+++ b/gnn_qot_estimation_amd/_lib.py
@@ -74,6 +74,8 @@
                                 _int, _f, _f, _u64, _p, _p]),
     "qot_nnconv_fused_split": (_int, [_p, _int, _p, _p, _p, _p, _p, _p, _p, _p, _i64, _p, _p, _i64, _int, _int,
                                       _int, _f, _f, _u64, _p, _p]),
+    "qot_nnconv_fused_split_rowsum": (_int, [_p, _int, _p, _p, _p, _p, _p, _p, _p, _p, _i64, _p, _p, _p, _i64, _int, _int,
+                                             _f, _f, _u64, _p, _p]),
     "qot_nnconv_gradh_split": (_int, [_p, _int, _p, _int, _p, _p, _p, _p, _p, _p, _p, _p, _i64, _p, _p, _p, _i64, _int,
                                       _int, _p]),
     "qot_nnconv_bwd_finalize": (_int, [_p, _p, _p, _p, _p, _i64, _int, _int, _p]),
@@ -130,6 +132,8 @@
     "qot_head_fwd_loss": (_int, [_p, _p, _p, _p, _p, _p, _p, _p, _p, _i64, _int, _int, _f, _f, _u64, _p, _p, _f, _p, _p, _p]),
     "qot_head_train": (_int, [_p, _p, _p, _p, _p, _p, _p, _f, _p, _p, _p, _p, _p, _i64, _int, _int, _f, _f, _u64, _p, _int,
                               _f, _f, _u64, _p, _p]),
+    "qot_head_train_rowsum": (_int, [_p, _p, _p, _p, _p, _p, _p, _p, _f, _p, _p, _p, _p, _p, _i64, _int, _int, _f, _f, _u64, _p,
+                                     _f, _f, _u64, _p, _p]),
     "qot_head_train_blocks": (_int, [_i64, _int]),
     "qot_head_bwd_workspace_floats": (_sz, [_int, _int]),
     "qot_head_bwd_blocks": (_int, [_i64]),
diff --git a/gnn_qot_estimation_amd/csrc/head.hip b/gnn_qot_estimation_amd/csrc/head.hip
--- a/gnn_qot_estimation_amd/csrc/head.hip
+++ b/gnn_qot_estimation_amd/csrc/head.hip
@@ -1,4 +1,5 @@
 #include "common.hpp"
+#include "mfma_tile.hpp"
 
 namespace qot {
 
@@ -431,14 +432,16 @@
 #define QOT_HEAD_THREADS 512
 #endif
 constexpr int kHeadThreads = QOT_HEAD_THREADS;
-
-template <int H, int NT>
+constexpr int kHeadKeepCodes = 4;
+
+template <int H, int NT, bool ROWSUM = false>
 __global__ __launch_bounds__(NT) void head_train_batched_kernel(
     const float* __restrict__ x, const int32_t* __restrict__ ptr, const float* __restrict__ w0,
     const float* __restrict__ b0, const float* __restrict__ w3, const float* __restrict__ b3,
     const float* __restrict__ target, float beta, float inv_n, float* __restrict__ out, float* __restrict__ grad_out,
     float* __restrict__ loss_rows, float* __restrict__ gx, float* __restrict__ partials, int64_t B, int O, ActParams act,
-    int fold, ActParams in_act) {
+    int fold, ActParams in_act, const uint16_t* __restrict__ codes = nullptr) {
+    static_assert(!ROWSUM || H == 64, "the code words are laid out for the 64-wide forward tile");
     constexpr int TPR = H / 4, RPB = NT / TPR;
     constexpr int GB = 256 / H;
     constexpr int SPG = RPB / GB;
@@ -474,6 +477,10 @@
     for (int e = t; e < O * H; e += NT) w3s[e] = w3[e];
     const uint64_t stepv = act.thr16 ? (uint64_t)act.step[0] : 0;
     const uint64_t in_stepv = (fold && in_act.thr16) ? (uint64_t)in_act.step[0] : 0;
+    const uint16_t* cds = codes;
+    if constexpr (ROWSUM) {
+        if (!codes) cds = reinterpret_cast<const uint16_t*>(x + (int64_t)((ptr[B] + 3) >> 2) * H);
+    }
     const float b0o = b0[o];
     float aw0[PER];
 #pragma unroll
@@ -492,8 +499,28 @@
         __syncthreads();
         const bool live = b0g + gs < B;
         const int beg = pb[gs], cnt = live ? pb[gs + 1] - beg : 0;
-        float4 v[KR];
+        float4 v[ROWSUM ? 1 : KR];
+        uint2 cw[ROWSUM ? kHeadKeepCodes : 1];
         float4 acc = f4zero();
+        auto code_words = [&](int64_t g4) {
+            const int row = 4 * (int)(g4 & 7);
+            return *reinterpret_cast<const uint2*>(
+                cds + ((g4 >> 3) * 4 + rowsum_code_wave(row, 4 * sub)) * 64 + rowsum_code_lane(row, 4 * sub));
+        };
+        if constexpr (ROWSUM) {
+            const int64_t beg4 = beg >> 2;
+            const int cnt4 = cnt >> 2;
+            float4 pv[kHeadKeepCodes];
+#pragma unroll
+            for (int k = 0; k < kHeadKeepCodes; ++k) {
+                const int r = sr + SPG * k;
+                pv[k] = (r < cnt4) ? ld4(x + (beg4 + r) * H + 4 * sub) : f4zero();
+                cw[k] = (r < cnt4) ? code_words(beg4 + r) : make_uint2(0u, 0u);
+            }
+#pragma unroll
+            for (int k = 0; k < kHeadKeepCodes; ++k) acc = add4(acc, pv[k]);
+            for (int r = sr + SPG * kHeadKeepCodes; r < cnt4; r += SPG) acc = add4(acc, ld4(x + (beg4 + r) * H + 4 * sub));
+        } else {
 #pragma unroll
         for (int k = 0; k < KR; ++k) {
             const int r = sr + SPG * k;
@@ -502,6 +529,7 @@
 #pragma unroll
         for (int k = 0; k < KR; ++k) acc = add4(acc, v[k]);
         for (int r = sr + SPG * KR; r < cnt; r += SPG) acc = add4(acc, ld4(x + (int64_t)(beg + r) * H + 4 * sub));
+        }
         cred[t] = acc;
         __syncthreads();
         if (t < GB * TPR) {
@@ -616,12 +644,39 @@
                 st4(gx + flat, o4);
                 acs = add4(acs, o4);
             };
+            auto back4 = [&](int r, uint2 w) {
+                const int64_t g4 = (beg >> 2) + r;
+                const uint32_t wc[4] = {w.x & 0xFFFFu, w.x >> 16, w.y & 0xFFFFu, w.y >> 16};
+                const int s0 = rowsum_code_slot(4 * (int)(g4 & 7));
+#pragma unroll
+                for (int j = 0; j < 4; ++j) {
+                    float vi[4] = {gv.x, gv.y, gv.z, gv.w};
+#pragma unroll
+                    for (int c = 0; c < 4; ++c) {
+                        const uint32_t bits = wc[c] >> (2 * (s0 + j));
+                        vi[c] = vi[c] * ((bits & 1u) ? in_act.keep_scale : 0.f) * ((bits & 2u) ? 1.0f : in_act.slope);
+                    }
+                    const float4 o4 = make_float4(vi[0], vi[1], vi[2], vi[3]);
+                    st4(gx + (4 * g4 + j) * H + 4 * sub, o4);
+                    acs = add4(acs, o4);
+                }
+            };
+            if constexpr (ROWSUM) {
+                const int cnt4 = cnt >> 2;
+#pragma unroll
+                for (int k = 0; k < kHeadKeepCodes; ++k) {
+                    const int r = sr + SPG * k;
+                    if (r < cnt4) back4(r, cw[k]);
+                }
+                for (int r = sr + SPG * kHeadKeepCodes; r < cnt4; r += SPG) back4(r, code_words((beg >> 2) + r));
+            } else {
 #pragma unroll
             for (int k = 0; k < KR; ++k) {
                 const int r = sr + SPG * k;
                 if (r < cnt) back(r, v[k]);
             }
             for (int r = sr + SPG * KR; r < cnt; r += SPG) back(r, fold ? ld4(x + (int64_t)(beg + r) * H + 4 * sub) : f4zero());
+            }
         }
     }
     float* part_row = partials + (int64_t)blockIdx.x * (H * H + H + O * H + O + (fold ? H : 0));
@@ -717,6 +772,9 @@
     if (O > 8) return QOT_ERR_UNSUPPORTED;
     if (!x || !ptr || !w0 || !b0 || !w3 || !b3 || !target || !out || !grad_out || !loss_rows || !grad_x || !workspace)
         return QOT_ERR_BADARG;
+    if (fold == 2)
+        return qot_head_train_rowsum(x, nullptr, ptr, w0, b0, w3, b3, target, beta, out, grad_out, loss_rows, grad_x, workspace,
+                                     B, H, O, slope, p, seed, step_counter, in_slope, in_p, in_seed, in_step, stream_);
     const ActParams ap = make_act(1, slope, p, seed, step_counter);
     const ActParams in_ap = make_act(fold ? 1 : 0, in_slope, in_p, in_seed, in_step);
     int blocks = kHeadBwdBlocks;
@@ -747,6 +805,31 @@
         head_train_kernel<kH><<<blocks, 256, lds, stream>>>(x, ptr, w0, b0, w3, b3, target, beta, inv_n, out, grad_out,
                                                             loss_rows, grad_x, workspace, B, O, ap, fold, in_ap);
     });
+    QOT_LAUNCH_CHECK();
+    return QOT_OK;
+}
+
+extern "C" int qot_head_train_rowsum(const float* rowsum4, const uint16_t* codes, const int32_t* ptr, const float* w0,
+                                     const float* b0, const float* w3, const float* b3, const float* target, float beta,
+                                     float* out, float* grad_out, float* loss_rows, float* grad_x, float* workspace,
+                                     int64_t B, int H, int O, float slope, float p, uint64_t seed,
+                                     const int64_t* step_counter, float in_slope, float in_p, uint64_t in_seed,
+                                     const int64_t* in_step, qot_stream_t stream_) {
+    hipStream_t stream = (hipStream_t)stream_;
+    if (B <= 0 || O <= 0 || !(beta > 0.f)) return QOT_ERR_BADARG;
+    if (O > 8 || H != 64) return QOT_ERR_UNSUPPORTED;
+    if (!rowsum4 || ((uintptr_t)codes & 7) || ((uintptr_t)rowsum4 & 15) || !ptr || !w0 || !b0 || !w3 || !b3 || !target || !out || !grad_out ||
+        !loss_rows || !grad_x || !workspace)
+        return QOT_ERR_BADARG;
+    const ActParams ap = make_act(1, slope, p, seed, step_counter);
+    const ActParams in_ap = make_act(1, in_slope, in_p, in_seed, in_step);
+    const int blocks = qot_head_train_blocks(B, H);
+    const float inv_n = 1.0f / ((float)B * (float)O);
+    constexpr int kH = 64;
+    const size_t lds = (size_t)(kH * (kH + 1) + 8 * kH) * sizeof(float);
+    head_train_batched_kernel<kH, kHeadThreads, true><<<blocks, kHeadThreads, lds, stream>>>(
+        rowsum4, ptr, w0, b0, w3, b3, target, beta, inv_n, out, grad_out, loss_rows, grad_x, workspace, B, O, ap, 1, in_ap,
+        codes);
     QOT_LAUNCH_CHECK();
     return QOT_OK;
 }
diff --git a/gnn_qot_estimation_amd/csrc/mfma_tile.hpp b/gnn_qot_estimation_amd/csrc/mfma_tile.hpp
--- a/gnn_qot_estimation_amd/csrc/mfma_tile.hpp
+++ b/gnn_qot_estimation_amd/csrc/mfma_tile.hpp
@@ -14,6 +14,11 @@
 }
 
 __host__ __device__ constexpr int acc_row(int r, int hi) { return (r & 3) + 8 * (r >> 2) + 4 * hi; }
+
+__host__ __device__ constexpr uint32_t rowsum_code_bits(bool kept, bool pos) { return (kept ? 1u : 0u) | (pos ? 2u : 0u); }
+__host__ __device__ constexpr int rowsum_code_wave(int row, int c) { return (c >> 5) + 2 * (row >> 4); }
+__host__ __device__ constexpr int rowsum_code_lane(int row, int c) { return 32 * ((row >> 2) & 1) + (c & 31); }
+__host__ __device__ constexpr int rowsum_code_slot(int row) { return 4 * ((row >> 3) & 1) + (row & 3); }
 
 __device__ __forceinline__ f32x16 mfma4(float4 a, float4 b, f32x16 c) {
     c = __builtin_amdgcn_mfma_f32_32x32x2f32(a.x, b.x, c, 0, 0, 0);
diff --git a/gnn_qot_estimation_amd/csrc/nnconv_mfma.hip b/gnn_qot_estimation_amd/csrc/nnconv_mfma.hip
--- a/gnn_qot_estimation_amd/csrc/nnconv_mfma.hip
+++ b/gnn_qot_estimation_amd/csrc/nnconv_mfma.hip
@@ -105,15 +105,16 @@
 
 __host__ __device__ constexpr int fwd_plane_off(int p) { return (p / 4) * 3 * kGhPlLd + (p % 4) * kGhPlStep; }
 
-template <int D, bool TRANSPOSE, bool SPLIT = false, bool PRESPLIT = false>
+template <int D, bool TRANSPOSE, bool SPLIT = false, bool PRESPLIT = false, bool ROWSUM = false>
 __global__ __launch_bounds__(256, 2) void nnconv_mfma64_kernel(
     const float* __restrict__ x, int ldx, const float* __restrict__ ea, const float* __restrict__ w1,
     const float* __restrict__ b1, const int32_t* __restrict__ rowptr, const int32_t* __restrict__ col,
     const int32_t* __restrict__ eidx, const float* __restrict__ invdeg, const float* __restrict__ Wp,
     const float* __restrict__ bias, float* __restrict__ out, int64_t N, ActParams act,
-    const u32x4* __restrict__ Ws = nullptr, int64_t ws_planes = 0) {
+    const u32x4* __restrict__ Ws = nullptr, int64_t ws_planes = 0, uint16_t* __restrict__ codes = nullptr) {
     static_assert(!SPLIT || !TRANSPOSE, "split form: forward only");
     static_assert(!PRESPLIT || SPLIT, "the planes are the split form's");
+    static_assert(!ROWSUM || PRESPLIT, "row sums: the pre-split form's epilogue only");
     constexpr int K = 2 * D;
     constexpr int KM = (K + 1) * 64;
     constexpr int GM = KM / 16;
@@ -312,21 +313,38 @@
             }
             quad_share_draws<2, 2, 1>(mylo, myhi, zlo, zhi);
         }
+        float ys[ROWSUM ? 8 : 1];
+        uint32_t code = 0;
 #pragma unroll
         for (int r = 0; r < 8; ++r) {
             const int rr = kh * 8 + r;
             const int row = acc_row(rr, hi);
             const int64_t i = tile0 + row;
             float y = v[r];
+            bool kept = true;
             if (act.enabled) {
                 y = y > 0.f ? y : act.slope * y;
                 if (drop) {
                     const uint64_t z = ((uint64_t)zhi[r] << 32) | zlo[r];
                     const bool keep = ((uint32_t)(z >> (16 * (colg & 3))) & 0xFFFFu) >= act.thr16;
                     y = keep ? y * act.keep_scale : 0.f;
+                    if constexpr (ROWSUM) kept = keep;
                 }
             }
-            if (i < N) out[i * 64 + colg] = y;
+            if constexpr (ROWSUM) {
+                ys[r] = i < N ? y : 0.f;
+                if (i < N) code |= rowsum_code_bits(kept, v[r] > 0.f) << (2 * r);
+            } else {
+                if (i < N) out[i * 64 + colg] = y;
+            }
+        }
+        if constexpr (ROWSUM) {
+#pragma unroll
+            for (int u = 0; u < 2; ++u) {
+                const int64_t g4 = tile * 8 + 2 * (2 * kh + u) + hi;
+                if (4 * g4 < N) out[g4 * 64 + colg] = ((ys[4 * u] + ys[4 * u + 1]) + ys[4 * u + 2]) + ys[4 * u + 3];
+            }
+            codes[(tile * 4 + wave) * 64 + lane] = (uint16_t)code;
         }
     }
     if constexpr (!PRESPLIT) lds_barrier();
@@ -683,6 +701,31 @@
     return QOT_OK;
 }
 
+extern "C" int qot_nnconv_fused_split_rowsum(const float* x, int ld_x, const float* edge_attr, const float* w1,
+                                             const float* b1, const int32_t* rowptr, const int32_t* col,
+                                             const int32_t* edge_ids, const float* invdeg, const void* w_split,
+                                             int64_t split_stride, const float* bias, float* rowsum4, uint16_t* codes,
+                                             int64_t N, int H, int D, float act_slope, float act_p, uint64_t act_seed,
+                                             const int64_t* act_step, qot_stream_t stream) {
+    if (N < 0 || !rowptr) return QOT_ERR_BADARG;
+    if (H != 64 || D > 4) return QOT_ERR_UNSUPPORTED;
+    if (N == 0) return QOT_OK;
+    if (!x || !w1 || !b1 || !invdeg || !w_split || !rowsum4 || !codes || (ld_x & 3) || ((uintptr_t)w_split & 15) ||
+        (split_stride & 7) || split_stride < (int64_t)(2 * D + 2) * 4096)
+        return QOT_ERR_BADARG;
+    int grid = grid_for(N, 32);
+    if (grid > 2 * num_cus()) grid = 2 * num_cus();
+    const ActParams ap = make_act(1, act_slope, act_p, act_seed, act_step);
+    QOT_DISPATCH_D(D, {
+        if (kD <= 4)
+            nnconv_mfma64_kernel<(kD <= 4 ? kD : 4), false, true, true, true><<<grid, 256, 0, (hipStream_t)stream>>>(
+                x, ld_x, edge_attr, w1, b1, rowptr, col, edge_ids, invdeg, nullptr, bias, rowsum4, N, ap,
+                static_cast<const u32x4*>(w_split), split_stride / 8, codes);
+    });
+    QOT_LAUNCH_CHECK();
+    return QOT_OK;
+}
+
 int qot_nnconv_gradh64_launch(const float* grad_out, int ld_g, const float* x, int ld_x, const float* edge_attr, const float* w1,
                               const float* b1, const int32_t* rowptr, const int32_t* col, const int32_t* eid, const float* invdeg,
                               const float* b_perm, const void* b_split, int64_t split_stride, float* workspace, int64_t N, int D,
diff --git a/gnn_qot_estimation_amd/functional.py b/gnn_qot_estimation_amd/functional.py
--- a/gnn_qot_estimation_amd/functional.py
+++ b/gnn_qot_estimation_amd/functional.py
@@ -708,6 +708,11 @@
     return os.environ.get("QOT_NNCONV_F32_MFMA", "0") != "1"
 
 
+def head_rowsum_wanted(h: int, fours: bool) -> bool:
+    return (h == 64 and fours and nnconv_split_bf16() and os.environ.get("QOT_HEAD_FROM_ROWS") != "1"
+            and os.environ.get("QOT_NNCONV_FWD_SPLIT_AFTER_READ") != "1" and not os.environ.get("QOT_NO_HEAD_TRAIN"))
+
+
 def nnconv_split_index(k: int, device) -> torch.Tensor:
     key = ("splitidx", k, str(device))
     if key not in _PERM_CACHE:
@@ -793,6 +798,7 @@
         ctx.receivers = (w1, b1, w2, b2, wroot)
         if side is not None and act is not None:
             side["bias_param"] = bias
+        want_rows4 = side is not None and bool(side.pop("rowsum", None))
         x, edge_attr = _f32c(x), _f32c(edge_attr)
         w1, b1, w2, b2, wroot, bias = (_f32c(t) for t in (w1, b1, w2, b2, wroot, bias))
         N, hin = x.shape
@@ -811,15 +817,31 @@
         if D > 4:
             return NNConvFn._forward_wide_edge(ctx, x, edge_attr, w1, b1, w2, b2, wroot, bias, graph, act, side)
         wp, wp_adj, bp, split = packed if packed is not None else nnconv_pack(w2, b2, wroot, hin, K)
-        out = torch.empty(N, hout, dtype=torch.float32, device=x.device)
-        if split is not None:
+        rows4 = None
+        if want_rows4:
+            if (act is not None and split is not None and hin == 64
+                    and os.environ.get("QOT_NNCONV_FWD_SPLIT_AFTER_READ") != "1"):
+                n4 = ((N + 3) // 4) * hout
+                both = torch.empty(n4 + ((N + 31) // 32) * 128, dtype=torch.float32, device=x.device)
+                rows4, codes = both[:n4].view(-1, hout), both[n4:].view(torch.int16)
+                _lib.call("qot_nnconv_fused_split_rowsum", P(x), hin, P(edge_attr), P(w1), P(b1), P(graph.rowptr),
+                          P(graph.col), P(graph.eid), P(graph.invdeg), P(split), split.numel() // 3, P(bias), P(rows4),
+                          P(codes), N, hin, D, *_act_args(act)[1:])
+                side["rowsum"] = both
+                out = rows4.as_strided((N, hout), (0, 1))
+        if rows4 is None:
+            out = torch.empty(N, hout, dtype=torch.float32, device=x.device)
+        if rows4 is not None:
+            pass
+        elif split is not None:
             _lib.call("qot_nnconv_fused_split", P(x), hin, P(edge_attr), P(w1), P(b1), P(graph.rowptr), P(graph.col),
                       P(graph.eid), P(graph.invdeg), P(split), split.numel() // 3, P(bias), P(out), N, hin, D,
                       *_act_args(act))
         else:
             _lib.call("qot_nnconv_fused", P(x), hin, P(edge_attr), P(w1), P(b1), P(graph.rowptr), P(graph.col),
                       P(graph.eid), P(graph.invdeg), 0, P(wp), P(bias), P(out), N, hin, D, *_act_args(act))
-        ctx.save_for_backward(x, edge_attr, w1, b1, w2, b2, wroot, None, wp_adj, bp, out if act is not None else None,
+        ctx.save_for_backward(x, edge_attr, w1, b1, w2, b2, wroot, None, wp_adj, bp,
+                              out if (act is not None and rows4 is None) else None,
                               act[3] if act is not None else None, split)
         ctx.n_wcat = wp.numel()
         ctx.graph = graph
@@ -993,7 +1015,13 @@
     def forward(ctx, x, ptr32, w0, b0, w3, b3, B, act, in_act=None, side=None, loss=None):
         require_cuda(x, w0, b0, w3, b3)
         ctx.receivers = (w0, b0, w3, b3)
-        x, w0, b0, w3, b3 = (_f32c(t) for t in (x, w0, b0, w3, b3))
+        rowsum = side.pop("rowsum", None) if side is not None else None
+        if rowsum is not None and not (in_act is not None and loss is not None and len(loss) > 3 and loss[3]
+                                       and not os.environ.get("QOT_NO_HEAD_TRAIN")):
+            raise RuntimeError("the producer wrote row sums for the fused train read-out, which does not run")
+        w0, b0, w3, b3 = (_f32c(t) for t in (w0, b0, w3, b3))
+        if rowsum is None:
+            x = _f32c(x)
         N, H = x.shape
         O = w3.shape[0]
         slope, p, seed, step = act
@@ -1018,9 +1046,11 @@
                 ws = torch.empty(_lib.load().qot_head_bwd_workspace_floats(H, O), dtype=torch.float32, device=dev)
                 fa = (1, float(in_act[0]), float(in_act[1] if in_act[3] is not None else 0.0), int(in_act[2]), P(in_act[3])) \
                     if fold else (0, 0.0, 0.0, 0, None)
-                _lib.call("qot_head_train", P(x), P(ptr32), P(w0), P(b0), P(w3), P(b3), P(target), float(beta), P(out), P(gout),
-                          P(loss_rows), P(gx), P(ws), B, H, O, float(slope), float(p if step is not None else 0.0), int(seed),
-                          P(step), *fa)
+                if rowsum is not None:
+                    fa = (2,) + fa[1:]
+                _lib.call("qot_head_train", P(rowsum if rowsum is not None else x), P(ptr32), P(w0), P(b0), P(w3), P(b3),
+                          P(target), float(beta), P(out), P(gout), P(loss_rows), P(gx), P(ws), B, H, O, float(slope),
+                          float(p if step is not None else 0.0), int(seed), P(step), *fa)
                 ctx.train_fused = (gx, ws, gout, nb + (H if fold else 0))
                 ctx.cfg = (N, H, O, B, float(slope), float(p if step is not None else 0.0), int(seed))
                 ctx.fold = fold
diff --git a/gnn_qot_estimation_amd/graph.py b/gnn_qot_estimation_amd/graph.py
--- a/gnn_qot_estimation_amd/graph.py
+++ b/gnn_qot_estimation_amd/graph.py
@@ -245,6 +245,24 @@
     return res
 
 
+def graphs_in_fours(data, maps) -> bool:
+    if maps is not None:
+        return int(maps[3][1]) % 4 == 0
+    ptr, B = getattr(data, "ptr", None), getattr(data, "num_graphs", None)
+    if ptr is None or B is None or ptr.numel() != int(B) + 1:
+        return False
+    tag = (ptr.data_ptr(), ptr._version, tuple(ptr.shape))
+    c = _cache(data)
+    if c is not None and "ptr_fours" in c and c["ptr_fours"][0] == tag:
+        return c["ptr_fours"][1]
+    if ptr.is_cuda and torch.cuda.is_current_stream_capturing():
+        return False
+    ok = bool((ptr.detach().to("cpu") % 4 == 0).all())
+    if c is not None:
+        c["ptr_fours"] = (tag, ok)
+    return ok
+
+
 def cached_i32(data, name: str) -> torch.Tensor:
     t = getattr(data, name)
     tag = (t.data_ptr(), t._version, tuple(t.shape))
diff --git a/gnn_qot_estimation_amd/topological.py b/gnn_qot_estimation_amd/topological.py
--- a/gnn_qot_estimation_amd/topological.py
+++ b/gnn_qot_estimation_amd/topological.py
@@ -4,7 +4,7 @@
 from torch import nn
 
 from . import _lib, functional as QF, launch_group as LG
-from .graph import batch_index_for, batch_ptr_for, cached_i32, graph_index_for, table_maps_for
+from .graph import batch_index_for, batch_ptr_for, cached_i32, graph_index_for, graphs_in_fours, table_maps_for
 from .nn import NNConv, TransformerConv
 
 
@@ -164,6 +164,9 @@
         fused_head = width in (16, 32, 64, 128) and l3.out_features <= 8 and l0.out_features == width
         side = {} if (fused_head and torch.is_grad_enabled() and getattr(self, "_qot_fold_head", True)) else None
         last_act = None
+        if (side is not None and loss_spec is not None and not getattr(self, f"conv{self.num_layers}")._forward_hooks
+                and QF.head_rowsum_wanted(width, graphs_in_fours(data, maps))):
+            side["rowsum"] = True
         for layer in range(2, self.num_layers + 1):
             act_l = self._act(layer - 1, step)
             last = layer == self.num_layers
diff --git a/include/qot_gnn.h b/include/qot_gnn.h
--- a/include/qot_gnn.h
+++ b/include/qot_gnn.h
@@ -125,6 +125,12 @@
                            int64_t split_stride, const float* bias, float* out, int64_t N, int H, int D,
                            int act, float act_slope, float act_p, uint64_t act_seed, const int64_t* act_step,
                            qot_stream_t stream);
+int qot_nnconv_fused_split_rowsum(const float* x, int ld_x, const float* edge_attr, const float* w1,
+                                  const float* b1, const int32_t* rowptr, const int32_t* col,
+                                  const int32_t* edge_ids, const float* invdeg, const void* w_split,
+                                  int64_t split_stride, const float* bias, float* rowsum4, uint16_t* codes, int64_t N,
+                                  int H, int D, float act_slope, float act_p, uint64_t act_seed, const int64_t* act_step,
+                                  qot_stream_t stream);
 size_t qot_gemm_tn_workspace_floats(int KT);
 int qot_gemm_tn(const float* A, int lda, const float* G, int ldg, int64_t N, int KT, float* C,
                 float* workspace, qot_stream_t stream);
@@ -268,6 +274,11 @@
                    float* workspace, int64_t B, int H, int O, float slope, float p, uint64_t seed,
                    const int64_t* step_counter, int fold, float in_slope, float in_p, uint64_t in_seed,
                    const int64_t* in_step, qot_stream_t stream);
+int qot_head_train_rowsum(const float* rowsum4, const uint16_t* codes, const int32_t* ptr, const float* w0, const float* b0,
+                          const float* w3, const float* b3, const float* target, float beta, float* out, float* grad_out,
+                          float* loss_rows, float* grad_x, float* workspace, int64_t B, int H, int O, float slope, float p,
+                          uint64_t seed, const int64_t* step_counter, float in_slope, float in_p, uint64_t in_seed,
+                          const int64_t* in_step, qot_stream_t stream);
 size_t qot_head_bwd_workspace_floats(int H, int O);
 int qot_head_bwd_blocks(int64_t B);
 int qot_head_bwd(const float* grad_out, const float* pooled, const float* hidden, const int32_t* ptr,
```
